# fatchord/WaveRNN

Measured on AMD Instinct MI355X. Metric: audio samples/sec (real-time factor @22.05 kHz), MoL WaveRNN batched generate, higher is better.
Workload: dtype f32

## Files before the change

### include/wavernn_amd.h

```cpp
#ifndef WAVERNN_AMD_H
#define WAVERNN_AMD_H

#include <stddef.h>
#include <stdint.h>

#ifdef __cplusplus
extern "C" {
#endif

#define WRNN_ABI_VERSION 9

enum {
    WRNN_OK = 0,
    WRNN_ERR_ARG = -1,
    WRNN_ERR_NO_DEVICE = -2,
    WRNN_ERR_HIP = -3,
    WRNN_ERR_WORKSPACE = -4,
    WRNN_ERR_KERNEL = -5,
    WRNN_ERR_RESIDENCY = -6
};

enum { WRNN_MODE_RAW = 0, WRNN_MODE_MOL = 1 };

enum {
// ... 111 lines not shown
    int32_t struct_bytes;
    int32_t n_cus;
    int32_t mode, C;
    int32_t generic;
    int32_t gH, gF, gM, gA;
    int32_t sp_nbp;
    int32_t sp_max_blocks;
    int32_t sp_fc;
} wrnn_plan_traits;
int wrnn_debug_plan(const wrnn_plan_traits *traits, int32_t n_segments, int32_t T, int32_t n_frames,
                    const wrnn_options *opt, wrnn_run_info *out, size_t *workspace_bytes);

int wrnn_timer_create(int device, wrnn_timer **out);
void wrnn_timer_destroy(wrnn_timer *t);
float wrnn_timer_ms(wrnn_timer *t);
int wrnn_timer_launches(const wrnn_timer *t);

typedef struct wrnn_pre_weights {
    int32_t feat_dims;
    int32_t compute_dims;
    int32_t res_out_dims;
    int32_t res_blocks;
    int32_t pad;
    int32_t upsample_factors[3];
    const float *conv_in_w;
    const float *bn_in;
    const float *res_w;
    const float *res_bn;
    const float *conv_out_w;
    const float *conv_out_b;
    const float *up_w;
} wrnn_pre_weights;
typedef struct wrnn_pre wrnn_pre;

int wrnn_pre_create(const wrnn_pre_weights *w, int device, wrnn_pre **out);
void wrnn_pre_destroy(wrnn_pre *p);
int wrnn_pre_hop(const wrnn_pre *p);
size_t wrnn_pre_workspace_bytes(const wrnn_pre *p, int32_t n_frames);
int wrnn_pre_upsample(const wrnn_pre *p, const float *mel, int32_t n_frames, float *mels_up, float *aux,
                      void *workspace, size_t workspace_bytes, void *stream);
int wrnn_pre_upsample_rows(const wrnn_pre *p, const float *mel, int32_t n_frames, float *mel_rows, float *aux,
                           void *workspace, size_t workspace_bytes, void *stream);
typedef struct wrnn_pre_utt {
    const float *mel;
    int32_t n_frames;
    int32_t reserved;
    int64_t up_row;
    int64_t aux_row;
} wrnn_pre_utt;
size_t wrnn_pre_workspace_bytes_many(const wrnn_pre *p, const wrnn_pre_utt *utts, int32_t n_utt, int32_t rows_only);
int wrnn_pre_upsample_many(const wrnn_pre *p, const wrnn_pre_utt *utts, int32_t n_utt, int32_t rows_only, float *mels_up, float *aux,
                           void *workspace, size_t workspace_bytes, void *stream);
int wrnn_pre_debug_host_handle(const wrnn_pre_weights *w, wrnn_pre **out);
const char *wrnn_pre_last_error(void);

int wrnn_post_unfold(const float *segments, int32_t T, int32_t n_utt, const int32_t *first, const int32_t *folds,
                     const int64_t *out_off, const double *lut, int32_t n_classes, const double *fade_in,
                     const double *fade_out, int32_t overlap, const double *tail, int32_t tail_len, int32_t batched,
                     double *out, void *stream);
const char *wrnn_post_last_error(void);

typedef struct wrnn_taco_weights {
    uint32_t struct_bytes;
    int32_t n_mels, prenet1, prenet2, decoder_dims, encoder_width, lstm_dims, attn_filters, attn_kernel;
    const float *prenet_fc1_w, *prenet_fc1_b, *prenet_fc2_w, *prenet_fc2_b;
    const float *attn_rnn_w_ih, *attn_rnn_w_hh, *attn_rnn_b_ih, *attn_rnn_b_hh;
    const float *attn_W_w, *attn_W_b, *attn_conv_w, *attn_L_w, *attn_L_b, *attn_v_w;
    const float *rnn_input_w, *rnn_input_b;
    const float *rnn1_w_ih, *rnn1_w_hh, *rnn1_b_ih, *rnn1_b_hh;
    const float *rnn2_w_ih, *rnn2_w_hh, *rnn2_b_ih, *rnn2_b_hh;
    const float *mel_proj_w;
} wrnn_taco_weights;

typedef struct wrnn_taco_call {
    uint32_t struct_bytes;
    int32_t n;
    int32_t r, max_r;
    int32_t max_steps;
    float stop_threshold;
    const float *seq;
    const float *seq_proj;
    float *mel_out;
    float *scores_out;
    int32_t *steps_done;
    void *workspace;
    size_t workspace_bytes;
    void *stream;
    int32_t variant;
} wrnn_taco_call;

size_t wrnn_taco_workspace_bytes(void);
int wrnn_taco_decode(int device, const wrnn_taco_weights *w, const wrnn_taco_call *c);
int wrnn_taco_status(const void *workspace, unsigned *out4, void *stream);
const char *wrnn_taco_last_error(void);

#define WRNN_TACO_BATCH_MAX 8
#define WRNN_TACO_BATCH_NMAX 256
typedef struct wrnn_taco_batch_call {
    uint32_t struct_bytes;
    int32_t n_sent;
    int32_t r, max_r;
    float stop_threshold;
    const int32_t *n;
    const int32_t *max_steps;
    const float *const *seq, *const *seq_proj;
    float *const *mel_out;
// ... 92 lines not shown
```

### wavernn_amd/_lib.py

```python
import ctypes
import os
import subprocess

_HERE = os.path.dirname(os.path.abspath(__file__))
CSRC = os.path.join(_HERE, 'csrc')
SO_PATH = os.path.join(CSRC, 'libwavernn_amd.so')

WRNN_OK = 0
ERR_ARG = -1
ERR_NO_DEVICE = -2
ERR_RESIDENCY = -6
MODE_RAW, MODE_MOL = 0, 1
ABI_VERSION = 9
ALGO_AUTO, ALGO_STREAM, ALGO_LOOP, ALGO_SPARSE, ALGO_DUO, ALGO_CHAIN, ALGO_OCTO = 0, 1, 2, 5, 6, 7, 8
ALGOS = {'auto': ALGO_AUTO, 'stream': ALGO_STREAM, 'loop': ALGO_LOOP, 'sparse': ALGO_SPARSE, 'duo': ALGO_DUO, 'chain': ALGO_CHAIN, 'octo': ALGO_OCTO}

EXPORTS = ['wrnn_last_error', 'wrnn_abi_version', 'wrnn_device_cus', 'wrnn_pack_create', 'wrnn_pack_destroy',
           'wrnn_pack_weight_bytes', 'wrnn_pack_sparse_blocks', 'wrnn_pack_sparse_fc_blocks', 'wrnn_workspace_bytes', 'wrnn_workspace_bytes_segments', 'wrnn_generate',
           'wrnn_generate_segments', 'wrnn_noise_fill', 'wrnn_noise_fill_host', 'wrnn_plan_segments', 'wrnn_status', 'wrnn_timer_create', 'wrnn_timer_destroy', 'wrnn_timer_ms',
           'wrnn_timer_launches', 'wrnn_debug_read_exchange', 'wrnn_debug_plan', 'wrnn_selftest', 'wrnn_selftest_metric', 'wrnn_pre_create',
           'wrnn_pre_destroy', 'wrnn_pre_hop', 'wrnn_pre_workspace_bytes', 'wrnn_pre_upsample', 'wrnn_pre_upsample_rows', 'wrnn_pre_workspace_bytes_many',
           'wrnn_pre_upsample_many', 'wrnn_pre_debug_host_handle', 'wrnn_pre_last_error',
           'wrnn_post_unfold', 'wrnn_post_last_error', 'wrnn_taco_workspace_bytes', 'wrnn_taco_decode', 'wrnn_taco_status',
           'wrnn_taco_last_error', 'wrnn_bigru', 'wrnn_taco_front_create', 'wrnn_taco_front_destroy', 'wrnn_taco_front_workspace_bytes',
           'wrnn_taco_encode', 'wrnn_taco_postnet', 'wrnn_taco_batch_workspace_bytes', 'wrnn_taco_decode_batch',
           'wrnn_bigru_many', 'wrnn_taco_front_workspace_bytes_many', 'wrnn_taco_encode_many', 'wrnn_taco_postnet_many',
           'wrnn_taco_front_debug_host_handle']


class Weights(ctypes.Structure):
    _fields_ = [(n, ctypes.c_int32) for n in ('rnn_dims', 'fc_dims', 'feat_dims', 'aux_dims', 'n_classes', 'mode')] + \
               [(n, ctypes.c_void_p) for n in ('I_w', 'I_b', 'w_ih1', 'w_hh1', 'b_ih1', 'b_hh1', 'w_ih2', 'w_hh2',
                                               'b_ih2', 'b_hh2', 'fc1_w', 'fc1_b', 'fc2_w', 'fc2_b', 'fc3_w', 'fc3_b')]


class PreWeights(ctypes.Structure):
    _fields_ = [(n, ctypes.c_int32) for n in ('feat_dims', 'compute_dims', 'res_out_dims', 'res_blocks', 'pad')] + \
               [('upsample_factors', ctypes.c_int32 * 3)] + \
               [(n, ctypes.c_void_p) for n in ('conv_in_w', 'bn_in', 'res_w', 'res_bn', 'conv_out_w', 'conv_out_b', 'up_w')]


class PreUtt(ctypes.Structure):
    _fields_ = [('mel', ctypes.c_void_p), ('n_frames', ctypes.c_int32), ('reserved', ctypes.c_int32), ('up_row', ctypes.c_int64),
                ('aux_row', ctypes.c_int64)]


TACO_WEIGHT_FIELDS = ('prenet_fc1_w', 'prenet_fc1_b', 'prenet_fc2_w', 'prenet_fc2_b', 'attn_rnn_w_ih', 'attn_rnn_w_hh', 'attn_rnn_b_ih',
                      'attn_rnn_b_hh', 'attn_W_w', 'attn_W_b', 'attn_conv_w', 'attn_L_w', 'attn_L_b', 'attn_v_w', 'rnn_input_w', 'rnn_input_b',
                      'rnn1_w_ih', 'rnn1_w_hh', 'rnn1_b_ih', 'rnn1_b_hh', 'rnn2_w_ih', 'rnn2_w_hh', 'rnn2_b_ih', 'rnn2_b_hh', 'mel_proj_w')


class TacoWeights(ctypes.Structure):
    _fields_ = [('struct_bytes', ctypes.c_uint32)] + \
               [(n, ctypes.c_int32) for n in ('n_mels', 'prenet1', 'prenet2', 'decoder_dims', 'encoder_width', 'lstm_dims', 'attn_filters',
                                              'attn_kernel')] + \
               [(n, ctypes.c_void_p) for n in TACO_WEIGHT_FIELDS]


class TacoCall(ctypes.Structure):
    _fields_ = [('struct_bytes', ctypes.c_uint32), ('n', ctypes.c_int32), ('r', ctypes.c_int32), ('max_r', ctypes.c_int32),
                ('max_steps', ctypes.c_int32), ('stop_threshold', ctypes.c_float), ('seq', ctypes.c_void_p), ('seq_proj', ctypes.c_void_p),
                ('mel_out', ctypes.c_void_p), ('scores_out', ctypes.c_void_p), ('steps_done', ctypes.c_void_p),
                ('workspace', ctypes.c_void_p), ('workspace_bytes', ctypes.c_size_t), ('stream', ctypes.c_void_p), ('variant', ctypes.c_int32)]


TACO_BATCH_MAX = 8
TACO_BATCH_NMAX = 256


class TacoBatchCall(ctypes.Structure):
    _fields_ = [('struct_bytes', ctypes.c_uint32), ('n_sent', ctypes.c_int32), ('r', ctypes.c_int32), ('max_r', ctypes.c_int32),
                ('stop_threshold', ctypes.c_float), ('n', ctypes.POINTER(ctypes.c_int32)), ('max_steps', ctypes.POINTER(ctypes.c_int32)),
                ('seq', ctypes.POINTER(ctypes.c_void_p)), ('seq_proj', ctypes.POINTER(ctypes.c_void_p)),
                ('mel_out', ctypes.POINTER(ctypes.c_void_p)), ('scores_out', ctypes.POINTER(ctypes.c_void_p)),
                ('steps_done', ctypes.c_void_p), ('workspace', ctypes.c_void_p), ('workspace_bytes', ctypes.c_size_t), ('stream', ctypes.c_void_p)]
# ... 99 lines not shown
    import torch
    L = ctypes.CDLL(SO_PATH)
    L.wrnn_last_error.restype = ctypes.c_char_p
    L.wrnn_abi_version.restype = ctypes.c_int
    L.wrnn_device_cus.argtypes = [ctypes.c_int]
    L.wrnn_pack_create.argtypes = [ctypes.POINTER(Weights), ctypes.c_int, ctypes.POINTER(ctypes.c_void_p)]
    L.wrnn_pack_destroy.argtypes = [ctypes.c_void_p]
    L.wrnn_pack_destroy.restype = None
    L.wrnn_pack_weight_bytes.argtypes = [ctypes.c_void_p]
    L.wrnn_pack_weight_bytes.restype = ctypes.c_size_t
    L.wrnn_pack_sparse_blocks.argtypes = [ctypes.c_void_p]
    L.wrnn_pack_sparse_fc_blocks.argtypes = [ctypes.c_void_p]
    L.wrnn_workspace_bytes.argtypes = [ctypes.c_void_p, ctypes.POINTER(Geometry), ctypes.POINTER(Options)]
    L.wrnn_workspace_bytes.restype = ctypes.c_size_t
    L.wrnn_generate.argtypes = [ctypes.c_void_p, ctypes.POINTER(Geometry), ctypes.c_void_p, ctypes.c_void_p,
                                ctypes.c_void_p, ctypes.c_void_p, ctypes.c_void_p, ctypes.c_size_t, ctypes.POINTER(Options),
                                ctypes.c_void_p]
    L.wrnn_workspace_bytes_segments.argtypes = [ctypes.c_void_p, ctypes.c_int32, ctypes.c_int32, ctypes.c_int32,
                                                ctypes.POINTER(Options)]
    L.wrnn_workspace_bytes_segments.restype = ctypes.c_size_t
    L.wrnn_generate_segments.argtypes = [ctypes.c_void_p, ctypes.c_int32, ctypes.c_int32, ctypes.c_void_p, ctypes.c_void_p,
                                         ctypes.c_int32, ctypes.c_int32, ctypes.c_int32, ctypes.c_void_p, ctypes.c_void_p,
                                         ctypes.c_void_p, ctypes.c_void_p, ctypes.c_void_p, ctypes.c_size_t,
                                         ctypes.POINTER(Options), ctypes.c_void_p]
    L.wrnn_noise_fill.argtypes = [ctypes.c_int, ctypes.c_int32, ctypes.c_int32, ctypes.c_int32, ctypes.c_int32, ctypes.c_uint64, ctypes.c_void_p,
                                  ctypes.c_void_p, ctypes.c_int, ctypes.c_void_p]
    L.wrnn_noise_fill_host.argtypes = L.wrnn_noise_fill.argtypes[:8]
    L.wrnn_plan_segments.argtypes = [ctypes.c_void_p, ctypes.c_int32, ctypes.c_int32, ctypes.POINTER(Options), ctypes.POINTER(RunInfo)]
    L.wrnn_timer_create.argtypes = [ctypes.c_int, ctypes.POINTER(ctypes.c_void_p)]
    L.wrnn_timer_destroy.argtypes = [ctypes.c_void_p]
    L.wrnn_timer_destroy.restype = None
    L.wrnn_timer_ms.argtypes = [ctypes.c_void_p]
    L.wrnn_timer_ms.restype = ctypes.c_float
    L.wrnn_timer_launches.argtypes = [ctypes.c_void_p]
    L.wrnn_debug_read_exchange.argtypes = [ctypes.c_void_p, ctypes.c_void_p, ctypes.c_int32, ctypes.c_int32, ctypes.c_int32,
                                           ctypes.POINTER(Options), ctypes.c_int, ctypes.c_int, ctypes.c_int, ctypes.c_int,
                                           ctypes.c_void_p]
    L.wrnn_debug_plan.argtypes = [ctypes.POINTER(PlanTraits), ctypes.c_int32, ctypes.c_int32, ctypes.c_int32, ctypes.POINTER(Options),
                                  ctypes.POINTER(RunInfo), ctypes.POINTER(ctypes.c_size_t)]
    L.wrnn_pre_create.argtypes = [ctypes.POINTER(PreWeights), ctypes.c_int, ctypes.POINTER(ctypes.c_void_p)]
    L.wrnn_pre_destroy.argtypes = [ctypes.c_void_p]
    L.wrnn_pre_destroy.restype = None
    L.wrnn_pre_hop.argtypes = [ctypes.c_void_p]
    L.wrnn_pre_workspace_bytes.argtypes = [ctypes.c_void_p, ctypes.c_int32]
    L.wrnn_pre_workspace_bytes.restype = ctypes.c_size_t
    L.wrnn_pre_upsample.argtypes = [ctypes.c_void_p, ctypes.c_void_p, ctypes.c_int32, ctypes.c_void_p, ctypes.c_void_p,
                                    ctypes.c_void_p, ctypes.c_size_t, ctypes.c_void_p]
    L.wrnn_pre_upsample_rows.argtypes = L.wrnn_pre_upsample.argtypes
    L.wrnn_pre_workspace_bytes_many.argtypes = [ctypes.c_void_p, ctypes.POINTER(PreUtt), ctypes.c_int32, ctypes.c_int32]
    L.wrnn_pre_workspace_bytes_many.restype = ctypes.c_size_t
    L.wrnn_pre_upsample_many.argtypes = [ctypes.c_void_p, ctypes.POINTER(PreUtt), ctypes.c_int32, ctypes.c_int32, ctypes.c_void_p, ctypes.c_void_p,
                                         ctypes.c_void_p, ctypes.c_size_t, ctypes.c_void_p]
    L.wrnn_pre_debug_host_handle.argtypes = [ctypes.POINTER(PreWeights), ctypes.POINTER(ctypes.c_void_p)]
    L.wrnn_pre_last_error.restype = ctypes.c_char_p
    L.wrnn_post_unfold.argtypes = [ctypes.c_void_p, ctypes.c_int32, ctypes.c_int32, ctypes.c_void_p, ctypes.c_void_p, ctypes.c_void_p,
                                   ctypes.c_void_p, ctypes.c_int32, ctypes.c_void_p, ctypes.c_void_p, ctypes.c_int32,
                                   ctypes.c_void_p, ctypes.c_int32, ctypes.c_int32, ctypes.c_void_p, ctypes.c_void_p]
    L.wrnn_post_last_error.restype = ctypes.c_char_p
    L.wrnn_taco_workspace_bytes.restype = ctypes.c_size_t
    L.wrnn_taco_decode.argtypes = [ctypes.c_int, ctypes.POINTER(TacoWeights), ctypes.POINTER(TacoCall)]
    L.wrnn_taco_status.argtypes = [ctypes.c_void_p, ctypes.POINTER(ctypes.c_uint32 * 4), ctypes.c_void_p]
    L.wrnn_taco_last_error.restype = ctypes.c_char_p
    L.wrnn_taco_batch_workspace_bytes.argtypes = [ctypes.c_int32]
    L.wrnn_taco_batch_workspace_bytes.restype = ctypes.c_size_t
    L.wrnn_taco_decode_batch.argtypes = [ctypes.c_int, ctypes.POINTER(TacoWeights), ctypes.POINTER(TacoBatchCall)]
    L.wrnn_bigru.argtypes = [ctypes.c_int, ctypes.POINTER(BigruCall)]
    L.wrnn_taco_front_create.argtypes = [ctypes.POINTER(TacoFrontWeights), ctypes.c_int, ctypes.POINTER(ctypes.c_void_p)]
    L.wrnn_taco_front_destroy.argtypes = [ctypes.c_void_p]
    L.wrnn_taco_front_destroy.restype = None
    L.wrnn_taco_front_workspace_bytes.argtypes = [ctypes.c_void_p, ctypes.c_int32]
    L.wrnn_taco_front_workspace_bytes.restype = ctypes.c_size_t
    L.wrnn_taco_encode.argtypes = [ctypes.c_void_p, ctypes.c_void_p, ctypes.c_int32, ctypes.c_void_p, ctypes.c_void_p, ctypes.c_void_p,
                                   ctypes.c_void_p, ctypes.c_size_t, ctypes.c_void_p]
    L.wrnn_taco_postnet.argtypes = [ctypes.c_void_p, ctypes.c_void_p, ctypes.c_int32, ctypes.c_void_p, ctypes.c_void_p, ctypes.c_void_p,
                                    ctypes.c_size_t, ctypes.c_void_p]
    L.wrnn_bigru_many.argtypes = [ctypes.c_int, ctypes.POINTER(BigruManyCall)]
    L.wrnn_taco_front_workspace_bytes_many.argtypes = [ctypes.c_void_p, ctypes.POINTER(ctypes.c_int32), ctypes.c_int32]
    L.wrnn_taco_front_workspace_bytes_many.restype = ctypes.c_size_t
    L.wrnn_taco_encode_many.argtypes = [ctypes.c_void_p, ctypes.c_void_p, ctypes.POINTER(ctypes.c_int32), ctypes.c_int32, ctypes.c_void_p,
                                        ctypes.c_void_p, ctypes.c_void_p, ctypes.c_void_p, ctypes.c_size_t, ctypes.c_void_p]
    L.wrnn_taco_postnet_many.argtypes = [ctypes.c_void_p, ctypes.POINTER(ctypes.c_void_p), ctypes.POINTER(ctypes.c_int32), ctypes.c_int32,
                                         ctypes.c_void_p, ctypes.c_void_p, ctypes.c_void_p, ctypes.c_size_t, ctypes.c_void_p]
    L.wrnn_taco_front_debug_host_handle.argtypes = [ctypes.POINTER(TacoFrontWeights), ctypes.POINTER(ctypes.c_void_p)]
    L.wrnn_status.argtypes = [ctypes.c_void_p, ctypes.c_void_p]
    L.wrnn_selftest.argtypes = [ctypes.c_int, ctypes.c_int]
    L.wrnn_selftest_metric.restype = ctypes.c_float
    _lib = L
    return L


def check(rc, what):
    if rc != WRNN_OK:
        raise WrnnError(f'{what} failed (rc={rc}): {lib().wrnn_last_error().decode()}')


def noise_fill_host(mode, n_segments, n_classes, t_begin, t_end, seed, seg_id=None):
    import numpy as np
    mol = mode == 'MOL'
    out = np.empty((t_end - t_begin, 11 * n_segments) if mol else (t_end - t_begin, n_segments, n_classes), np.float32)
    ids = None if seg_id is None else np.ascontiguousarray(seg_id, dtype=np.uint64)
    if ids is not None and ids.shape != (n_segments,):
        raise ValueError('seg_id: one 64-bit id per segment')
    check(lib().wrnn_noise_fill_host(MODE_MOL if mol else MODE_RAW, n_segments, n_classes, t_begin, t_end, int(seed) & (2 ** 64 - 1),
                                     None if ids is None else ids.ctypes.data, out.ctypes.data), 'wrnn_noise_fill_host')
    return out
```

### wavernn_amd/batch.py

```python
import time
from dataclasses import dataclass
from typing import List, Optional, Sequence

import numpy as np
import torch

from . import fold as _fold


@dataclass
class Plan:
    target: int
    overlap: int
    T: int
    stride: int
    lengths: List[int]
    offsets: np.ndarray
    folds: np.ndarray
    first: np.ndarray
    seg_pos: np.ndarray
    seg_lim: np.ndarray
    seg_utt: np.ndarray

    @property
# ... 59 lines not shown
            else:
                origin = f'built-in defaults ({f} was measured on other kernel sources)'
        except (OSError, ValueError, KeyError):
            pass
        if path is not None:
            return table, origin
        _STEP_TABLE = (table, origin)
    return _STEP_TABLE


def estimate_step_us(n_segments: int, table: Optional[dict] = None) -> float:
    if n_segments <= 0:
        return 0.0
    table = table or step_table()[0]
    groups = -(-n_segments // 16)
    rounds = -(-groups // 32)
    depth = min(8, max(1, -(-(-(-groups // rounds)) // 4)))
    return rounds * table[depth]


def choose_ranks(n_segments: int, world: int, table: Optional[dict] = None) -> int:
    est = [estimate_step_us(-(-n_segments // r), table) for r in range(1, world + 1)]
    best = min(est)
    return 1 + next(i for i, e in enumerate(est) if e <= best * 1.01)


def pack_noise(mode: str, plan: Plan, per_utt, lo: int = 0, hi: Optional[int] = None, steps: Optional[int] = None):
    hi = plan.n_segments if hi is None else hi
    T = plan.T if steps is None else int(steps)
    n = hi - lo
    utts = [u for u in range(len(plan.lengths)) if plan.first[u] < hi and plan.first[u] + plan.folds[u] > lo]
    sample = per_utt[utts[0]]
    is_torch = isinstance(sample, torch.Tensor)
    cat = (lambda xs, d: torch.cat(xs, dim=d)) if is_torch else (lambda xs, d: np.concatenate(xs, axis=d))
    mix, logi, raw = [], [], []
    for u in utts:
        Bu, f0 = int(plan.folds[u]), int(plan.first[u])
        a, b = max(lo, f0) - f0, min(hi, f0 + Bu) - f0
        z = per_utt[u]
        if mode == 'MOL':
            z = z.reshape(T, 11 * Bu)
            mix.append(z[:, 10 * a:10 * b])
            logi.append(z[:, 10 * Bu + a:10 * Bu + b])
        else:
            raw.append(z.reshape(T, Bu, -1)[:, a:b])
    out = cat(mix + logi, 1) if mode == 'MOL' else cat(raw, 1)
    assert out.shape[0] == T and (out.shape[1] == 11 * n if mode == 'MOL' else out.shape[1] == n)
    return out.contiguous() if is_torch else np.ascontiguousarray(out)


def library_seg_ids(seed, folds, first_fold: int = 0) -> np.ndarray:
    hi = np.uint64((int(seed) & 0xffffffff) << 32)
    return hi | np.arange(first_fold, first_fold + int(folds), dtype=np.uint64)


def chunk_utterances(plan: Plan, lo: int, hi: int, max_segments: int):
    chunks, cur, cur_lo, cur_hi = [], [], None, None
    for u in range(len(plan.lengths)):
        a, b = max(lo, int(plan.first[u])), min(hi, int(plan.first[u] + plan.folds[u]))
        if a >= b:
            continue
        if cur and (b - cur_lo) > max_segments:
            chunks.append((cur, cur_lo, cur_hi))
            cur, cur_lo = [], None
        if cur_lo is None:
            cur_lo = a
        cur.append(u)
        cur_hi = b
    if cur:
        chunks.append((cur, cur_lo, cur_hi))
    return chunks


def generate_corpus(model, mels: Sequence, target: int, overlap: int, mu_law: bool, seeds: Optional[Sequence[int]] = None,
                    group=None, loop_fn=None, return_segments=False, noise_source='cpu', finish='all', check=True,
                    max_segments_per_launch: int = 4096, shard=None, ranks: Optional[int] = None, timings: Optional[dict] = None):
    import torch.distributed as dist
    from .rng import draw_steps
    if noise_source in ('cpu', 'library') and seeds is None:
        raise ValueError(f"noise_source={noise_source!r} needs `seeds` (one per utterance); "
                         "pass noise_source='device' to draw from the device generator instead")
    if noise_source not in ('cpu', 'device', 'library'):
        raise ValueError(f'unknown noise source {noise_source!r}')
    world = dist.get_world_size(group) if group is not None else 1
    rank = dist.get_rank(group) if group is not None else 0
    if shard is not None:
        if group is not None:
            raise ValueError('shard=(rank, world) emulates a rank without a process group')
        rank, world = int(shard[0]), int(shard[1])
        finish = 'own'
    device = next(model.parameters()).device
    mode = model.mode
    mu_law = mu_law if mode == 'RAW' else False
    hop = model.hop_length
    was_training = model.training
    model.eval()
    mels = [torch.as_tensor(m) for m in mels]
    mels = [m.unsqueeze(0) if m.dim() == 2 else m for m in mels]
    frames = [int(m.size(-1)) for m in mels]
    plan = plan_utterances([n * hop for n in frames], target, overlap)
    bounds = shard_bounds(plan.n_segments, world, ranks)
    lo, hi = bounds[rank]
    n_max = max(h - l for l, h in bounds)

    out_local = torch.zeros(n_max, plan.T, dtype=torch.float32, device=device)
    native_pre = loop_fn is None and getattr(model, 'pre_algo', 'torch') == 'native' and device.type == 'cuda'
# ... 48 lines not shown
                    return mels_up, aux
                ups, auxs = zip(*[model.conditioning(mels[u])[:2] for u in utts])
                return torch.cat(ups).contiguous(), torch.cat(auxs).contiguous()
            rows = eng is not None and native_pre and model.mel_rows_ok(eng, n_seg, T)
            mels_up, aux = conditioning(rows)
            rebase = np.array([local_off[int(u)] - int(plan.offsets[int(u)]) for u in plan.seg_utt[clo:chi]], dtype=np.int64)
            seg_pos = (plan.seg_pos[clo:chi].astype(np.int64) + rebase).astype(np.int32)
            seg_lim = (plan.seg_lim[clo:chi].astype(np.int64) + rebase).astype(np.int32)
            out_view = out_local[clo - lo:chi - lo]
            gens, pool = {}, None
            if noise_source == 'cpu':
                if len(utts) > 1 and mode == 'RAW':
                    import os
                    from concurrent.futures import ThreadPoolExecutor
                    pool = ThreadPoolExecutor(max(1, min(len(utts), (os.cpu_count() or 2) // (2 * max(1, int(os.environ.get('LOCAL_WORLD_SIZE', '1')))))))
                from .rng import burn_ctor_draws
                for u in utts:
                    gens[u] = torch.Generator(device='cpu').manual_seed(int(seeds[u]))
                    burn_ctor_draws(model.rnn_dims, model.aux_dims, 'cpu', gens[u])

            lib_ids = None
            if noise_source == 'library':
                lib_ids = np.concatenate([library_seg_ids(seeds[u], min(chi, int(plan.first[u] + plan.folds[u])) - max(clo, int(plan.first[u])),
                                                          max(clo, int(plan.first[u])) - int(plan.first[u])) for u in utts])
                assert lib_ids.shape == (n_seg,)
            lib_kw = dict(noise_seed=int(getattr(model, 'noise_key', 0)), noise_seg_id=lib_ids) if lib_ids is not None else {}

            def draw(steps_):
                if noise_source == 'library':
                    if loop_fn is None:
                        return None
                    from ._lib import noise_fill_host
                    return torch.from_numpy(noise_fill_host(mode, n_seg, model.n_classes, 0, steps_, lib_kw['noise_seed'], lib_ids)).to(device)
                if noise_source != 'cpu':
                    return draw_steps(mode, n_seg, steps_, model.n_classes, device, 'device')
                def one(u):
                    noise[u] = draw_steps(mode, int(plan.folds[u]), steps_, model.n_classes, 'cpu', 'cpu', generator=gens[u])
                if pool is None:
                    for u in utts:
                        one(u)
                else:
                    list(pool.map(one, utts))
                return pack_noise(mode, plan, noise, clo, chi, steps=steps_).to(device)

            if loop_fn is not None:
                out_view[:] = loop_fn(mels_up, aux, seg_pos, seg_lim, T, draw(T), hop)
                if pool is not None:
                    pool.shutdown()
                continue
            from ._lib import ResidencyError
            from .engine import RESUMABLE_KERNELS
            steps = T
            groups = model.loop_sparse_groups(eng, n_seg, T) if hasattr(model, 'loop_sparse_groups') else 0
            if noise_source != 'library' and eng.plan(n_seg, T, algo=model.loop_algo)['kernel'] in RESUMABLE_KERNELS:
                per_step = n_seg * (11 if mode == 'MOL' else model.n_classes) * 4
                steps = max(1, min(T, getattr(model, 'noise_chunk_bytes', 2 << 30) // per_step))
                steps = -(-T // (-(-T // steps)))
            try:
                for t0 in range(0, T, steps):
                    t1 = min(T, t0 + steps)
                    eng.run_segments(mels_up, aux, seg_pos, seg_lim, T, draw(t1 - t0), hop, algo=model.loop_algo, check=check, out=out_view,
                                     t_range=None if (t0 == 0 and t1 == T) else (t0, t1), sparse_groups=groups, tuning=slab_tuning, **lib_kw)
            except ResidencyError as e:
                import warnings
                warnings.warn(f'wavernn_amd: {e}; redoing the chunk unsliced on the next kernel')
                if rows:
                    mels_up, aux = conditioning(False)
                for u in gens:
                    gens[u].manual_seed(int(seeds[u]))
                    burn_ctor_draws(model.rnn_dims, model.aux_dims, 'cpu', gens[u])
                eng.run_segments(mels_up, aux, seg_pos, seg_lim, T, draw(T), hop, algo=model.loop_algo, check=check, out=out_view, sparse_groups=groups, tuning=slab_tuning, **lib_kw)
            finally:
                if pool is not None:
                    pool.shutdown()
    n_utt = len(frames)
    work, gathered = None, None
    if group is not None:
        gathered = [torch.empty_like(out_local) for _ in range(world)]
        work = dist.all_gather(gathered, out_local, group=group, async_op=True)
        if timings is not None:
            timings['gather_bytes'] = timings.get('gather_bytes', 0) + (world - 1) * out_local.numel() * out_local.element_size()
            timings['world_seen'] = dist.get_world_size(group)

    def gathered_segments():
        nonlocal work
        if group is None:
            if shard is not None:
                raise ValueError('an emulated shard has only its own block of segments')
            return out_local[:plan.n_segments]
        if work is not None:
            t_w = time.perf_counter()
            work.wait()
            work = None
            if timings is not None:
                timings['gather_wait_ms'] = timings.get('gather_wait_ms', 0.0) + (time.perf_counter() - t_w) * 1e3
        return torch.cat([gathered[r][:h - l] for r, (l, h) in enumerate(bounds)])

    if was_training:
        model.train()
    if return_segments:
        return gathered_segments().cpu().numpy().astype(np.float64), plan
    outs = [None] * n_utt

    def unfold(segs, first_of, us):
        if not us:
            return
        if native_post:
            from .post import unfold_on_device
            wav, sl = unfold_on_device(segs, *unfold_args(us, first_of), tables=early.get(first_of))
            if getattr(model, 'pinned_output', True):
                host = torch.empty(wav.shape, dtype=wav.dtype, pin_memory=True)
                host.copy_(wav, non_blocking=True)
                torch.cuda.current_stream(wav.device).synchronize()
                wav = host.numpy()
            else:
                wav = wav.cpu().numpy()
            for (a, b), u in zip(sl, us):
                outs[u] = wav[a:b]
            return
        host = segs.cpu().numpy().astype(np.float64)
        for u in us:
            y = host[first_of(u):first_of(u) + int(plan.folds[u])].copy()
            if mu_law:
                y = _fold.decode_mu_law(y, model.n_classes, False)
# ... 18 lines not shown
```

### wavernn_amd/csrc/wrnn_abi.hip

```cpp
#include <hip/hip_runtime.h>
#include <stdarg.h>
#include <stdio.h>
#include <stdlib.h>
#include <string.h>
#include <math.h>
#include <string>
#include <vector>

#include "../../include/wavernn_amd.h"
#include "wrnn_device.h"

namespace wrnn {
hipError_t launch_cond(const CondArgs &a, int n_cus, bool valu, hipStream_t stream);
hipError_t launch_cond_frames(const CondArgs &a, hipStream_t stream);
hipError_t launch_cond_frames_slab(const CondArgs &a, hipStream_t stream);
hipError_t launch_slab_prep(const CondArgs &a, const float *nz_in, float *nz_out, long nz_n, unsigned *xcc, int n_cus, hipStream_t stream);
hipError_t launch_cond_frag(const CondArgs &a, int n_cus, hipStream_t stream);
hipError_t launch_noise_mol(const float *in, float *out, long n, int B, int n_cus, hipStream_t stream);
hipError_t launch_noise_fill(bool mol, int B, int C, int t0, int t1, uint64_t seed, const uint64_t *seg_id, float *out, int n_cus, hipStream_t stream);
void noise_fill_host(bool mol, int B, int C, int t0, int t1, uint64_t seed, const uint64_t *seg_id, float *out);
hipError_t launch_stream(const LoopArgs &args, int mode, hipStream_t stream);
hipError_t launch_loop(const LoopArgs &args, int ncl, int mode, hipStream_t stream);
int loop_max_depth(int mode);
size_t loop_state_floats(int G);
hipError_t launch_generic(const GenArgs &args, int mode, hipStream_t stream);
bool generic_dims_ok(int H, int F, int M, int A, int C, int mode);
hipError_t launch_duo(const LoopArgs &args, int ncl, int mode, hipStream_t stream);
int duo_max_depth();
size_t duo_xbuf_bytes(int G);
size_t duo_xbuf_bytes_max();
hipError_t launch_sparse(const LoopArgs &args, int nbp, int mode, hipStream_t stream);
int sparse_clusters(int n_cus);
int sparse_max_slots();
size_t sparse_state_floats(int slots);
size_t sparse_xbuf_bytes(int slots);
hipError_t launch_put_floats(float *dst, const float *src, int n, hipStream_t stream);
hipError_t launch_chain(const LoopArgs &args, int mode, hipStream_t stream);
hipError_t launch_octo(const LoopArgs &args, int ncl, int mode, hipStream_t stream);
int octo_max_depth();
int chain_clusters(int n_cus);
int chain_max_depth();
size_t chain_state_floats(int G);
size_t chain_xbuf_bytes(int G);
int selftest_mfma(char *msg, size_t n);
int selftest_allgather(int n_cus, char *msg, size_t n, float *us_per_round);
int selftest_tanh(char *msg, size_t n);
int selftest_xor(char *msg, size_t n);
}

using namespace wrnn;

static thread_local char g_err[512] = "";
static void set_err(const char *fmt, ...)
// ... 310 lines not shown
extern "C" float wrnn_timer_ms(wrnn_timer *t)
{
    if (!t || t->used < 2) return -1.f;
    float total = 0.f;
    for (int i = 0; i + 1 < t->used; i += 2) {
        if (hipEventSynchronize(t->ev[i + 1]) != hipSuccess) return -1.f;
        float ms = 0.f;
        if (hipEventElapsedTime(&ms, t->ev[i], t->ev[i + 1]) != hipSuccess) return -1.f;
        total += ms;
    }
    return total;
}

namespace {
int timer_mark(wrnn_timer *t, hipStream_t stream)
{
    if (!t) return WRNN_OK;
    if (t->used == (int)t->ev.size()) {
        hipEvent_t e;
        HIPCHK(hipEventCreate(&e));
        t->ev.push_back(e);
    }
    HIPCHK(hipEventRecord(t->ev[t->used], stream));
    t->used += 1;
    return WRNN_OK;
}

struct ProgressCtx {
    void (*fn)(int32_t, int32_t, int32_t, void *);
    void *user;
    int32_t done, T, n;
};
void progress_trampoline(void *p)
{
    ProgressCtx *c = static_cast<ProgressCtx *>(p);
    c->fn(c->done, c->T, c->n, c->user);
    delete c;
}
int enqueue_progress(const wrnn_options *o, int done, int T, int n, hipStream_t stream)
{
    if (!o->progress) return WRNN_OK;
    ProgressCtx *c = new ProgressCtx{o->progress, o->progress_user, done, T, n};
    hipError_t e = hipLaunchHostFunc(stream, progress_trampoline, c);
    if (e != hipSuccess) {
        delete c;
        set_err("hipLaunchHostFunc failed: %s", hipGetErrorString(e));
        return WRNN_ERR_HIP;
    }
    return WRNN_OK;
}

enum Kind { K_STREAM, K_GENERIC, K_LOOP, K_DUO, K_OCTO, K_CHAIN, K_SPARSE, N_KINDS };
constexpr int DUO_TAB_FPS = 8;
constexpr bool DUO_AUTO = true;
constexpr int CHAIN_AUTO_GROUPS = 8;
constexpr bool OCTO_AUTO = false;

struct KindDesc {
    const char *name;
    int units_per_wg;
    int kind_tag;
    bool persistent;
    bool slabbed;
    bool mel_stage;
    int (*clusters)(int n_cus);
    int (*max_depth)(int mode);
    size_t (*state_floats)(int G);
    size_t (*xbuf_bytes)(int G);
    size_t (*xbuf_fill)(int G);
    hipError_t (*launch)(const LoopArgs &a, int ncl, int nbp, int mode, hipStream_t s);
};
size_t loop_xbuf_bytes(int) { return XBUF_FLOATS * sizeof(float); }
const KindDesc KINDS[N_KINDS] = {
     {"wrnn_stream_kernel", 0, 0, false, false, false},
     {"wrnn_generic_kernel", 16, 0, false, false, false},
     {"wrnn_loop_kernel", 16, 1, true, false, false, clusters_of_64, loop_max_depth, loop_state_floats, loop_xbuf_bytes, loop_xbuf_bytes,
                     [](const LoopArgs &a, int ncl, int, int mode, hipStream_t s) { return launch_loop(a, ncl, mode, s); }},
     {"wrnn_duo_kernel", 16, 2, true, true, true, clusters_of_64, [](int) { return duo_max_depth(); }, loop_state_floats,
                     [](int) { return duo_xbuf_bytes_max(); }, duo_xbuf_bytes,
                     [](const LoopArgs &a, int ncl, int, int mode, hipStream_t s) { return launch_duo(a, ncl, mode, s); }},
     {"wrnn_octo_kernel", 16, 5, true, true, true, clusters_of_64, [](int) { return octo_max_depth(); }, loop_state_floats,
                     [](int) { return duo_xbuf_bytes_max(); }, duo_xbuf_bytes,
                     [](const LoopArgs &a, int ncl, int, int mode, hipStream_t s) { return launch_octo(a, ncl, mode, s); }},
     {"wrnn_chain_kernel", 16, 4, true, true, true, chain_clusters, [](int) { return chain_max_depth(); }, chain_state_floats,
                     chain_xbuf_bytes, chain_xbuf_bytes,
                     [](const LoopArgs &a, int, int, int mode, hipStream_t s) { return launch_chain(a, mode, s); }},
     {"wrnn_sparse_kernel", 64, 3, true, true, true, sparse_clusters, [](int) { return 1; }, sparse_state_floats,
                     sparse_xbuf_bytes, sparse_xbuf_bytes,
                     [](const LoopArgs &a, int, int nbp, int mode, hipStream_t s) { return launch_sparse(a, nbp, mode, s); }},
};

struct Plan {
    Kind kind;
    int ncl, G, rounds, per_round, slab, ngr_max;
    int tab_fps;
    int t0, t1;
};

struct WsLayout {
    size_t status, xcc, segs, melc, c2f, c3f, c4f;
    size_t cI, npre;
    size_t nlib;
    size_t xbuf, state, cIf;
    size_t total;
};
size_t al(size_t x) { return (x + 255) / 256 * 256; }

template <class S> S norm_struct(const S *in)
{
    S s;
    memset(&s, 0, sizeof s);
    if (in) memcpy(&s, in, in->struct_bytes > 0 && (size_t)in->struct_bytes < sizeof s ? (size_t)in->struct_bytes : sizeof s);
    s.struct_bytes = (int32_t)sizeof s;
    return s;
}
wrnn_options whole_call(const wrnn_options *opt)
{
    wrnn_options o = norm_struct(opt);
    o.t_begin = 0; o.t_end = 0;
    return o;
}

void plan_split(Plan *pl, int B, int ncl, int gmax, int depth)
{
    const int groups = (B + SEG - 1) / SEG;
    int g = depth;
    if (g < 1 || g > gmax) {
        const int rounds = (groups + ncl * gmax - 1) / (ncl * gmax);
        g = (groups + ncl * rounds - 1) / (ncl * rounds);
        if (g < 1) g = 1;
        if (g > gmax) g = gmax;
    }
    pl->ncl = ncl; pl->G = g;
    pl->rounds = (groups + ncl * g - 1) / (ncl * g);
    pl->per_round = (B + pl->rounds - 1) / pl->rounds;
    pl->ngr_max = (pl->per_round + SEG - 1) / SEG;
    if (pl->ngr_max > ncl * g) { pl->rounds += 1; pl->per_round = (B + pl->rounds - 1) / pl->rounds; pl->ngr_max = (pl->per_round + SEG - 1) / SEG; }
}

constexpr size_t NOISE_LIB_SLAB_BYTES = (size_t)2 << 30;
int default_slab(const Plan &pl, int mode, int C, bool noise_lib)
{
    const int most = KINDS[pl.kind].slabbed ? 4096 : 1024;
    int slab = most;
    if (!KINDS[pl.kind].slabbed) slab = (int)((96u << 20) / ((size_t)pl.ngr_max * SEG * H * sizeof(float)));
    else if (mode == WRNN_MODE_MOL) slab = (int)((32u << 20) / ((size_t)pl.per_round * 11 * sizeof(float) * pl.rounds));
    else if (noise_lib) {
        const size_t fit = NOISE_LIB_SLAB_BYTES / ((size_t)pl.per_round * pl.rounds * C * sizeof(float));
        slab = fit < (size_t)most ? (int)fit : most;
    }
    return slab < 16 ? 16 : slab > most ? most : slab;
}

int make_plan(const wrnn_plan_traits *p, int B, int T, const wrnn_options *o, Plan *pl)
{
    const bool shape_ok = (p->mode == WRNN_MODE_MOL) || (p->C == H);
    pl->t0 = o->t_begin; pl->t1 = o->t_end;
    if (pl->t0 == 0 && pl->t1 == 0) pl->t1 = T;
    if (pl->t0 < 0 || pl->t1 > T || pl->t0 >= pl->t1) { set_err("bad step range [%d, %d) of T=%d", pl->t0, pl->t1, T); return WRNN_ERR_ARG; }
    const bool partial = pl->t0 != 0 || pl->t1 != T;
    const int algo = o->algo;
    if (algo != WRNN_ALGO_AUTO && algo != WRNN_ALGO_STREAM && algo != WRNN_ALGO_LOOP && algo != WRNN_ALGO_SPARSE && algo != WRNN_ALGO_DUO && algo != WRNN_ALGO_CHAIN &&
        algo != WRNN_ALGO_OCTO) {
        set_err("unknown algo %d", algo);
        return WRNN_ERR_ARG;
    }
    if (o->sparse_groups < 0 || o->sparse_groups > sparse_max_slots()) {
        set_err("wrnn_options.sparse_groups = %d: 0 or 1 (one group per cluster) or 2", o->sparse_groups);
        return WRNN_ERR_ARG;
    }
    if (o->noise_lib != 0 && o->noise_lib != 1) {
        set_err("wrnn_options.noise_lib = %d: 0 (the caller's `noise`) or 1 (the library draws it)", o->noise_lib);
        return WRNN_ERR_ARG;
    }
    const bool two_groups = o->sparse_groups == 2;
    const int groups = (B + SEG - 1) / SEG;
    pl->kind = K_STREAM; pl->ncl = 0; pl->G = 0; pl->rounds = 1; pl->per_round = B; pl->slab = T; pl->ngr_max = groups;
    if (p->generic) {
        if (algo != WRNN_ALGO_AUTO && algo != WRNN_ALGO_STREAM) {
            set_err("this pack has non-shipped dims (rnn %d, fc %d, feat %d, aux %d): only the generic kernel (algo auto / stream) runs it", p->gH, p->gF, p->gM, p->gA);
            return WRNN_ERR_ARG;
        }
        if (partial) { set_err("a partial step range needs a persistent loop kernel"); return WRNN_ERR_ARG; }
        if (two_groups) { set_err("wrnn_options.sparse_groups = 2: only wrnn_sparse_kernel runs two groups per cluster (this call runs on wrnn_generic_kernel)"); return WRNN_ERR_ARG; }
        pl->kind = K_GENERIC;
        return WRNN_OK;
    }
    const int ccl = KINDS[K_CHAIN].clusters(p->n_cus), scl = KINDS[K_SPARSE].clusters(p->n_cus), lcl = KINDS[K_LOOP].clusters(p->n_cus);
    const bool chain_hw = shape_ok && ccl >= 1;
    if (algo == WRNN_ALGO_CHAIN && !chain_hw) {
        set_err("wrnn_chain_kernel needs MOL or RAW with 512 classes, and >= 256 CUs (C = %d, device: %d CUs)", p->C, p->n_cus);
        return !shape_ok ? WRNN_ERR_ARG : WRNN_ERR_RESIDENCY;
    }
    if (algo == WRNN_ALGO_SPARSE && (!p->sp_nbp || scl < 1)) {
        set_err("block-sparse kernel needs MOL or RAW with 512 classes, >= 256 CUs and GRU matrices with <= 64 surviving 16x1 blocks per block row "
                "(this pack: mode %s, %d classes, up to %d blocks; device: %d CUs)", p->mode == WRNN_MODE_MOL ? "MOL" : "RAW", p->C, p->sp_max_blocks, p->n_cus);
        return (!p->sp_nbp) ? WRNN_ERR_ARG : WRNN_ERR_RESIDENCY;
    }
    if (algo == WRNN_ALGO_OCTO && (p->mode != WRNN_MODE_MOL || KINDS[K_OCTO].clusters(p->n_cus) != MAXCL)) {
        set_err("wrnn_octo_kernel needs MOL and >= 256 CUs (mode %d, device has %d CUs)", p->mode, p->n_cus);
        return p->mode != WRNN_MODE_MOL ? WRNN_ERR_ARG : WRNN_ERR_RESIDENCY;
    }
    if (algo == WRNN_ALGO_DUO && (!shape_ok || KINDS[K_DUO].clusters(p->n_cus) < 1)) {
        set_err("the two-workgroups-per-CU loop kernel needs MOL or RAW with 512 classes, and >= 64 CUs (C = %d, device has %d CUs)", p->C, p->n_cus);
        return !shape_ok ? WRNN_ERR_ARG : WRNN_ERR_RESIDENCY;
    }
    if (algo == WRNN_ALGO_LOOP && !(shape_ok && lcl >= 1)) {
        set_err("the loop kernel needs >= 64 CUs and (MOL or RAW with 512 classes); device has %d CUs, C=%d", p->n_cus, p->C);
        return WRNN_ERR_RESIDENCY;
    }
    const bool sparse_auto = p->sp_nbp && p->mode == WRNN_MODE_MOL;
    Kind kind = K_STREAM;
    int ncl = 0;
    if (algo == WRNN_ALGO_CHAIN || (algo == WRNN_ALGO_AUTO && chain_hw && groups <= CHAIN_AUTO_GROUPS && !sparse_auto)) {
        kind = K_CHAIN; ncl = ccl;
    } else if (algo == WRNN_ALGO_SPARSE || (algo == WRNN_ALGO_AUTO && sparse_auto && scl >= 1)) {
        kind = K_SPARSE; ncl = scl;
    } else if (algo != WRNN_ALGO_STREAM && shape_ok && lcl >= 1) {
        ncl = lcl;
        if (o->clusters == 1 || o->clusters == 2 || o->clusters == 4) ncl = o->clusters < ncl ? o->clusters : ncl;
        else if (groups < ncl && !(DUO_AUTO && algo != WRNN_ALGO_LOOP && ncl == MAXCL)) {
            int c2 = 1; while (c2 < groups) c2 *= 2; if (c2 < ncl) ncl = c2;
        }
        kind = K_LOOP;
        if (algo == WRNN_ALGO_DUO || (algo == WRNN_ALGO_AUTO && DUO_AUTO && ncl == MAXCL)) kind = K_DUO;
        if (algo == WRNN_ALGO_OCTO || (kind == K_DUO && algo == WRNN_ALGO_AUTO && OCTO_AUTO && p->mode == WRNN_MODE_MOL && !o->clusters)) kind = K_OCTO;
    }
    const KindDesc &k = KINDS[kind];
    pl->kind = kind;
    if (two_groups) {
        if (kind != K_SPARSE) {
            set_err("wrnn_options.sparse_groups = 2: only wrnn_sparse_kernel runs two groups per cluster (this call runs on %s)", k.name);
            return WRNN_ERR_ARG;
        }
        if (p->mode != WRNN_MODE_MOL) { set_err("wrnn_options.sparse_groups = 2: wrnn_sparse_kernel's 9-bit RAW form is built with one group per cluster only"); return WRNN_ERR_ARG; }
        if (!p->sp_fc || (o->tuning & 2048)) {
            set_err("wrnn_options.sparse_groups = 2: needs a pack whose Linear layers are block-sparse too (wrnn_pack_sparse_fc_blocks() > 0) and their gathered fc "
                    "stages: the dense fc tiles leave no registers for a second group");
            return WRNN_ERR_ARG;
        }
        if (o->phase_clocks && !(o->tuning & 64)) { set_err("wrnn_options.sparse_groups = 2: the phase-clock build of wrnn_sparse_kernel has one group per cluster only"); return WRNN_ERR_ARG; }
    }
    if (k.persistent) {
        if (two_groups) plan_split(pl, B, ncl, sparse_max_slots(), sparse_max_slots());
        else plan_split(pl, B, ncl, k.max_depth(p->mode), o->depth);
        pl->slab = o->slab_steps >= 1 ? o->slab_steps : default_slab(*pl, p->mode, p->C, o->noise_lib != 0);
        if (pl->slab > T) pl->slab = T;
        pl->tab_fps = DUO_TAB_FPS;
    } else if (partial) {
        set_err("a partial step range [%d, %d) needs a persistent loop kernel", pl->t0, pl->t1);
        return WRNN_ERR_ARG;
    }
    if (k.slabbed && ((size_t)B * pl->tab_fps + 1) * 3 * H * sizeof(float) >= 0x7FFFF000ull) {
        set_err("%d segments in one call: the per-slab aux tables exceed a 2 GB buffer resource; split the call (generate_corpus caps a launch at 4096 segments)", B);
        return WRNN_ERR_ARG;
    }
    return WRNN_OK;
}

WsLayout ws_layout(const wrnn_plan_traits *p, const Plan &pl, int B, int T, int n_frames, bool noise_lib)
{
    const size_t noise_row = (size_t)B * (p->mode == WRNN_MODE_MOL ? 11 : p->C) * sizeof(float);
    const KindDesc &k = KINDS[pl.kind];
    WsLayout l;
    memset(&l, 0, sizeof l);
    size_t o = 0;
    l.status = o; o = al(o + STATUS_WORDS * sizeof(unsigned));
    l.xcc = o;    o = al(o + XCC_WORDS * sizeof(unsigned));
    l.segs = o;   o = al(o + (size_t)3 * B * sizeof(int));
    l.melc = o;   o = al(o + (size_t)3 * LAST_SCALE * sizeof(float));
    if (pl.kind == K_GENERIC) {
        l.nlib = o; if (noise_lib) o = al(o + (size_t)T * noise_row);
        l.total = o;
        return l;
    }
    const size_t tab_rows = k.slabbed ? (size_t)B * pl.tab_fps + 1 : (size_t)n_frames + 1;
    l.c2f = o;    o = al(o + tab_rows * 3 * H * sizeof(float));
    l.c3f = o;    o = al(o + tab_rows * H * sizeof(float));
    l.c4f = o;    o = al(o + tab_rows * H * sizeof(float));
    if (k.persistent) {
        l.xbuf = o;  o = al(o + k.xbuf_bytes(pl.G));
        l.state = o; o = al(o + (size_t)pl.rounds * k.state_floats(pl.G) * sizeof(float));
        l.cIf = o;   if (!k.slabbed) o = al(o + (size_t)pl.slab * pl.ngr_max * SEG * H * sizeof(float));
        l.npre = o;  if (p->mode == WRNN_MODE_MOL) o = al(o + (size_t)pl.slab * 11 * B * sizeof(float));
    } else {
        l.cI = o;    o = al(o + (size_t)T * B * H * sizeof(float));
        l.npre = o;
    }
    l.nlib = o;   if (noise_lib) o = al(o + (size_t)(k.persistent ? pl.slab : T) * noise_row);
    l.total = o;
    return l;
}
void hop_magic(int hop, unsigned *magic, int *shift)
{
    *magic = 0u; *shift = 0;
    if (hop < 2) return;
    int s = 0;
    while ((1ll << s) < hop) ++s;
    const unsigned long long m = ((1ull << (31 + s)) + (unsigned long long)hop - 1ull) / (unsigned long long)hop;
    if (m >> 32) return;
    const int sh = s - 1;
    for (long long q = 0; q * hop < (1ll << 31); q += 997) {
        for (long long p = q * hop - 1; p <= q * hop + 1; ++p) {
            if (p < 0 || p >= (1ll << 31)) continue;
            if ((long long)(((unsigned long long)p * m) >> (32 + sh)) != p / hop) return;
        }
    }
    *magic = (unsigned)m; *shift = sh;
}

int check_geometry(const wrnn_geometry *g)
{
    if (!g) { set_err("NULL geometry"); return WRNN_ERR_ARG; }
    if (g->B < 1 || g->T < 1 || g->L < 1 || g->hop < 1 || g->n_frames < 1 || g->stride < 0) {
        set_err("bad geometry B=%d T=%d stride=%d L=%d hop=%d n_frames=%d", g->B, g->T, g->stride, g->L, g->hop, g->n_frames);
        return WRNN_ERR_ARG;
    }
    if ((long)g->n_frames * g->hop < g->L) { set_err("n_frames*hop < L"); return WRNN_ERR_ARG; }
    if ((double)g->B * g->stride + g->T > 2.0e9) { set_err("geometry overflows int32"); return WRNN_ERR_ARG; }
    return WRNN_OK;
}
int check_segments(int B, int T, const int32_t *seg_pos, const int32_t *seg_lim, int L, int hop, int n_frames)
{
    if (B < 1 || T < 1 || L < 1 || hop < 1 || n_frames < 1 || !seg_pos || !seg_lim) {
        set_err("bad segment table B=%d T=%d L=%d hop=%d n_frames=%d", B, T, L, hop, n_frames);
        return WRNN_ERR_ARG;
    }
    if ((long)n_frames * hop < L) { set_err("n_frames*hop < L"); return WRNN_ERR_ARG; }
    for (int b = 0; b < B; ++b) {
        if (seg_pos[b] < 0 || seg_lim[b] < 0 || seg_lim[b] > L || (double)seg_pos[b] + T > 2.0e9) {
            set_err("segment %d: pos=%d lim=%d outside [0,%d]", b, seg_pos[b], seg_lim[b], L);
            return WRNN_ERR_ARG;
        }
    }
    return WRNN_OK;
}
int plan_report(const wrnn_plan_traits *tr, int B, int T, int n_frames, const wrnn_options &o, wrnn_run_info *out, size_t *ws_bytes)
{
    Plan pl;
    const int rc = make_plan(tr, B, T, &o, &pl);
    if (rc != WRNN_OK) return rc;
    if (out) {
        memset(out, 0, sizeof *out);
        out->kernel = KINDS[pl.kind].name; out->units_per_wg = KINDS[pl.kind].units_per_wg;
        out->clusters = pl.ncl; out->depth = pl.G; out->rounds = pl.rounds; out->slab_steps = pl.slab;
    }
    if (ws_bytes) *ws_bytes = ws_layout(tr, pl, B, T, n_frames, o.noise_lib != 0).total;
    return WRNN_OK;
}
}

extern "C" size_t wrnn_workspace_bytes_segments(const wrnn_pack *p, int32_t n_segments, int32_t T, int32_t n_frames,
                                                const wrnn_options *opt)
{
    if (!p || n_segments < 1 || T < 1 || n_frames < 1) return 0;
    size_t bytes = 0;
    (void)plan_report(&p->tr, n_segments, T, n_frames, whole_call(opt), nullptr, &bytes);
    return bytes;
}

extern "C" int wrnn_plan_segments(const wrnn_pack *p, int32_t n_segments, int32_t T, const wrnn_options *opt, wrnn_run_info *out)
{
    if (!p || !out || n_segments < 1 || T < 1) { set_err("bad argument"); return WRNN_ERR_ARG; }
    return plan_report(&p->tr, n_segments, T, 1, whole_call(opt), out, nullptr);
}

extern "C" size_t wrnn_workspace_bytes(const wrnn_pack *p, const wrnn_geometry *g, const wrnn_options *opt)
{
    if (!p || check_geometry(g) != WRNN_OK) return 0;
    return wrnn_workspace_bytes_segments(p, g->B, g->T, g->n_frames, opt);
}

extern "C" int wrnn_generate_segments(const wrnn_pack *p, int32_t B, int32_t T, const int32_t *seg_pos,
                                      const int32_t *seg_lim, int32_t L, int32_t hop, int32_t n_frames,
                                      const float *mels_up, const float *aux, const float *noise, float *out,
                                      void *workspace, size_t workspace_bytes, const wrnn_options *opt, void *stream_)
{
    const wrnn_options opts = norm_struct(opt), *o = &opts;
    const bool lib_noise = o->noise_lib == 1;
    if (lib_noise && noise) {
        set_err("wrnn_options.noise_lib = 1: the library draws the noise itself -- `noise` must be NULL (the tensor passed would not be read)");
        return WRNN_ERR_ARG;
    }
    if (!p || !mels_up || !aux || (!noise && !lib_noise) || !out || !workspace) { set_err("NULL argument"); return WRNN_ERR_ARG; }
    int rc = check_segments(B, T, seg_pos, seg_lim, L, hop, n_frames);
    if (rc != WRNN_OK) return rc;
    Plan pl;
    if ((rc = make_plan(&p->tr, B, T, o, &pl)) != WRNN_OK) return rc;
    const KindDesc &k = KINDS[pl.kind];
    const WsLayout l = ws_layout(&p->tr, pl, B, T, n_frames, lib_noise);
    if (workspace_bytes < l.total) { set_err("workspace %zu < required %zu", workspace_bytes, l.total); return WRNN_ERR_WORKSPACE; }
    if (((uintptr_t)workspace & 255) != 0) { set_err("workspace must be 256-byte aligned"); return WRNN_ERR_ARG; }
    hipStream_t stream = (hipStream_t)stream_;
    DeviceGuard dg(p->device);
    HIPCHK(dg.err);
    char *ws = (char *)workspace;
    const bool mol_mode = p->tr.mode == WRNN_MODE_MOL;
    wrnn_timer *timer = o->timer;
    if (timer && pl.t0 == 0) timer->used = 0;

    if (pl.t0 == 0) HIPCHK(hipMemsetAsync(ws + l.status, 0, STATUS_WORDS * sizeof(unsigned), stream));
    HIPCHK(hipMemcpyAsync(ws + l.segs, seg_pos, (size_t)B * sizeof(int), hipMemcpyHostToDevice, stream));
    HIPCHK(hipMemcpyAsync(ws + l.segs + (size_t)B * sizeof(int), seg_lim, (size_t)B * sizeof(int), hipMemcpyHostToDevice, stream));
    const int *d_pos = (const int *)(ws + l.segs), *d_lim = d_pos + B;
    if (o->mel_stage) {
        if (!k.mel_stage) { set_err("wrnn_options.mel_stage: only wrnn_duo_kernel / wrnn_sparse_kernel / wrnn_chain_kernel form the last up-sampling stage (this call runs on another kernel)"); return WRNN_ERR_ARG; }
        if (o->mel_stage != 1 || o->mel_scale != LAST_SCALE || !o->mel_taps || !o->seg_moff || o->mel_rows < 3) {
            set_err("wrnn_options.mel_stage=%d: needs mel_scale == %d (got %d), mel_taps, seg_moff, mel_rows >= 3", o->mel_stage, LAST_SCALE, o->mel_scale);
            return WRNN_ERR_ARG;
        }
        for (int b = 0; b < B; ++b) {
            const long last = (seg_lim[b] < (long)seg_pos[b] + T ? seg_lim[b] : (long)seg_pos[b] + T) - 1;
            if (last < seg_pos[b]) continue;
            const long j0 = (long)seg_pos[b] + o->seg_moff[b], j1 = last + o->seg_moff[b];
            if (o->seg_moff[b] < 0 || j0 / LAST_SCALE < 1 || j1 / LAST_SCALE + 1 >= o->mel_rows) {
                set_err("segment %d: positions %ld..%ld of the last up-sampling stage reach outside its %d input rows", b, j0, j1, o->mel_rows);
                return WRNN_ERR_ARG;
            }
        }
        float coef[3 * LAST_SCALE];
        for (int ph = 0; ph < LAST_SCALE; ++ph) {
            double c0 = 0, c1 = 0, c2 = 0;
            for (int j = 0; j <= 2 * LAST_SCALE; ++j) {
                const double w = o->mel_taps[j];
                if (j < LAST_SCALE - ph) c0 += w; else if (j < 2 * LAST_SCALE - ph) c1 += w; else c2 += w;
            }
            coef[3 * ph] = (float)c0; coef[3 * ph + 1] = (float)c1; coef[3 * ph + 2] = (float)c2;
        }
        HIPCHK(hipMemcpyAsync(ws + l.segs + (size_t)2 * B * sizeof(int), o->seg_moff, (size_t)B * sizeof(int), hipMemcpyHostToDevice, stream));
        HIPCHK(launch_put_floats((float *)(ws + l.melc), coef, 3 * LAST_SCALE, stream));
    }
    if (pl.kind == K_GENERIC) {
        GenArgs g;
        memset(&g, 0, sizeof g);
        g.I_T = p->g_I_T; g.I_b = p->I_b; g.w_ih1T = p->w_ih1T; g.w_hh1T = p->w_hh1T; g.b_ih1 = p->b_ih1; g.b_hh1 = p->b_hh1;
        g.w_ih2T = p->g_w_ih2T; g.w_hh2T = p->w_hh2T; g.b_ih2 = p->b_ih2; g.b_hh2 = p->b_hh2;
        g.fc1T = p->g_fc1T; g.fc1_b = p->fc1_b; g.fc2T = p->g_fc2T; g.fc2_b = p->fc2_b; g.fc3T = p->fc3T; g.fc3_b = p->fc3_b;
        g.mels_up = mels_up; g.aux = aux; g.noise = noise; g.force_x = o->force_x; g.out = out; g.dbg_logits = o->logits;
        g.seg_pos = d_pos; g.seg_lim = d_lim;
        if (lib_noise) {
            HIPCHK(launch_noise_fill(mol_mode, B, p->tr.C, 0, T, o->noise_seed, o->noise_seg_id, (float *)(ws + l.nlib), p->tr.n_cus, stream));
            g.noise = (const float *)(ws + l.nlib);
        }
        g.H = p->tr.gH; g.F = p->tr.gF; g.M = p->tr.gM; g.A = p->tr.gA; g.C = p->tr.C; g.B = B; g.T = T; g.hop = hop;
        if ((rc = timer_mark(timer, stream)) != WRNN_OK) return rc;
        HIPCHK(launch_generic(g, p->tr.mode, stream));
        if ((rc = timer_mark(timer, stream)) != WRNN_OK) return rc;
        wrnn_run_info gi;
        memset(&gi, 0, sizeof gi);
        gi.kernel = k.name; gi.rounds = 1; gi.slab_steps = T; gi.launches = 1;
        if (o->info) *o->info = gi;
        return enqueue_progress(o, T, T, B, stream);
    }

    CondArgs c;
    memset(&c, 0, sizeof c);
    c.mels_up = mels_up; c.aux = aux; c.I_cT = p->I_cT; c.I_b = p->I_b; c.c2_wT = p->c2_wT; c.b_ih2 = p->b_ih2;
    c.c3_wT = p->c3_wT; c.fc1_b = p->fc1_b; c.c4_wT = p->c4_wT; c.fc2_b = p->fc2_b;
    c.c2f = (float *)(ws + l.c2f); c.c3f = (float *)(ws + l.c3f); c.c4f = (float *)(ws + l.c4f);
    c.seg_pos = d_pos; c.seg_lim = d_lim;
    c.B = B; c.T = T; c.hop = hop; c.NF = n_frames;
    if (k.slabbed) {
        const long eff = (long)(pl.tab_fps - 2) * hop + 1;
        if (pl.slab > eff) pl.slab = (int)eff;
    } else HIPCHK(launch_cond_frames(c, stream));

    LoopArgs a;
    memset(&a, 0, sizeof a);
    a.I_w0 = p->I_w0; a.w_ih1 = p->w_ih1; a.w_hh1 = p->w_hh1; a.b_ih1 = p->b_ih1; a.b_hh1 = p->b_hh1;
    a.w_ih2 = p->w_ih2; a.w_hh2 = p->w_hh2; a.b_hh2 = p->b_hh2; a.fc1_w = p->fc1_w; a.fc2_w = p->fc2_w;
    a.fc3_w = p->fc3_w; a.fc3_b = p->fc3_b; a.fc3f = p->fc3f; a.u1 = p->u1;
    a.w_ih1T = p->w_ih1T; a.w_hh1T = p->w_hh1T; a.w_ih2T = p->w_ih2T; a.w_hh2T = p->w_hh2T;
    a.fc1T = p->fc1T; a.fc2T = p->fc2T; a.fc3T = p->fc3T;
    a.c2f = c.c2f; a.c3f = c.c3f; a.c4f = c.c4f;
    a.noise = noise; a.force_x = o->force_x; a.out = out; a.dbg_logits = o->logits;
    a.status = (unsigned *)(ws + l.status);
    a.prof = (u64 *)o->phase_clocks;
    a.tuning = o->tuning;
    a.seg_pos = d_pos; a.seg_lim = d_lim;
    a.Btot = B; a.T = T; a.hop = hop; a.NF = n_frames; a.C = p->tr.C;
    a.NG = (B + SEG - 1) / SEG;
    a.Nall = B;
    a.xcc_tab = (unsigned *)(ws + l.xcc);
    a.mels_up = mels_up; a.aux_fr = aux; a.I_cT = p->I_cT; a.I_b = p->I_b;
    a.mel_stage = o->mel_stage; a.seg_moff = d_pos + 2 * B; a.mel_coef = (const float *)(ws + l.melc);
    hop_magic(hop, &a.hop_magic, &a.hop_shift);

    wrnn_run_info info;
    memset(&info, 0, sizeof info);
    info.kernel = k.name; info.units_per_wg = k.units_per_wg;
    info.clusters = pl.ncl; info.depth = pl.G; info.rounds = pl.rounds; info.slab_steps = pl.slab;

    if (k.persistent) {
        a.sp_vals = p->sp_vals; a.sp_cols = p->sp_cols;
        a.sp_fc_vals = (o->tuning & 2048) ? nullptr : p->sp_fc_vals; a.sp_fc_cols = p->sp_fc_cols;
        const bool mol = p->tr.mode == WRNN_MODE_MOL;
        a.xbuf = (float *)(ws + l.xbuf);
        a.cIf = (const float *)(ws + l.cIf);
        a.G = pl.G;
        c.cI = (float *)(ws + l.cIf);
        for (int s0 = pl.t0; s0 < pl.t1; s0 += pl.slab) {
            const int s1 = s0 + pl.slab < pl.t1 ? s0 + pl.slab : pl.t1;
            if (lib_noise) HIPCHK(launch_noise_fill(mol, B, p->tr.C, s0, s1, o->noise_seed, o->noise_seg_id, (float *)(ws + l.nlib), p->tr.n_cus, stream));
            const bool prep_fused = k.slabbed && !(o->tuning & 8192);
            const float *mol_rows = nullptr;
            if (mol) {
                const float *const rows = lib_noise ? (const float *)(ws + l.nlib) : noise + (size_t)(s0 - pl.t0) * 11 * B;
                if (prep_fused) mol_rows = rows;
                else HIPCHK(launch_noise_mol(rows, (float *)(ws + l.npre), (long)(s1 - s0) * 11 * B, B, p->tr.n_cus, stream));
                a.noise_pre = (const float *)(ws + l.npre);
                a.noise_t0 = s0;
            } else if (lib_noise) {
                a.noise = (const float *)(ws + l.nlib);
                a.noise_t0 = s0;
            } else {
                a.noise_t0 = pl.t0;
            }
            if (k.slabbed) {
                c.t0 = s0; c.B = B; c.FPS = pl.tab_fps;
                if (prep_fused) HIPCHK(launch_slab_prep(c, mol_rows, (float *)(ws + l.npre), (long)(s1 - s0) * 11 * B, (unsigned *)(ws + l.xcc), p->tr.n_cus, stream));
                else HIPCHK(launch_cond_frames_slab(c, stream));
                a.tab_fps = pl.tab_fps; a.tab_t0 = s0;
            }
            bool xcc_clear = prep_fused;
            for (int r = 0; r < pl.rounds; ++r) {
                const int rb0 = (int)(((long)r * B) / pl.rounds), rb1 = (int)(((long)(r + 1) * B) / pl.rounds);
                const int nr = rb1 - rb0;
                if (nr < 1) continue;
                const int ngr = (nr + SEG - 1) / SEG;
                c.t0 = s0; c.t1 = s1; c.rb0 = rb0; c.B = nr; c.NG = ngr;
                if (!k.slabbed) HIPCHK(launch_cond_frag(c, p->tr.n_cus, stream));
                if (!k.slabbed || s0 == 0 || pl.rounds > 1 || (o->tuning & 4)) HIPCHK(hipMemsetAsync(ws + l.xbuf, 0xFF, k.xbuf_fill(pl.G), stream));
                if (k.slabbed && !xcc_clear) HIPCHK(hipMemsetAsync(ws + l.xcc, 0, XCC_WORDS * sizeof(unsigned), stream));
                xcc_clear = false;
                a.state = (float *)(ws + l.state) + (size_t)r * k.state_floats(pl.G);
                a.t0 = s0; a.t1 = s1; a.cI_t0 = s0; a.rb0 = rb0; a.Btot = nr; a.NG = ngr; a.resume = s0 > 0 ? 1 : 0;
                a.kind_tag = k.kind_tag;
                if ((rc = timer_mark(timer, stream)) != WRNN_OK) return rc;
                hipError_t e = k.launch(a, pl.ncl, p->tr.sp_nbp, p->tr.mode, stream);
                if (e != hipSuccess) {
                    (void)hipGetLastError();
                    set_err("%s cooperative launch failed: %s", info.kernel, hipGetErrorString(e));
                    return e == hipErrorCooperativeLaunchTooLarge ? WRNN_ERR_RESIDENCY : WRNN_ERR_HIP;
                }
                if ((rc = timer_mark(timer, stream)) != WRNN_OK) return rc;
                info.launches += 1;
            }
            if ((rc = enqueue_progress(o, s1, T, B, stream)) != WRNN_OK) return rc;
        }
    } else {
        c.cI = (float *)(ws + l.cI);
        a.cI = c.cI;
        HIPCHK(launch_cond(c, p->tr.n_cus, o->cond_valu != 0, stream));
        if (lib_noise) {
            HIPCHK(launch_noise_fill(mol_mode, B, p->tr.C, 0, T, o->noise_seed, o->noise_seg_id, (float *)(ws + l.nlib), p->tr.n_cus, stream));
            a.noise = (const float *)(ws + l.nlib);
        }
        a.b0 = 0;
        a.nb = B;
        if ((rc = timer_mark(timer, stream)) != WRNN_OK) return rc;
        HIPCHK(launch_stream(a, p->tr.mode, stream));
        if ((rc = timer_mark(timer, stream)) != WRNN_OK) return rc;
        info.launches = 1;
        if ((rc = enqueue_progress(o, T, T, B, stream)) != WRNN_OK) return rc;
    }
    if (o->info) *o->info = info;
    return WRNN_OK;
}

extern "C" int wrnn_generate(const wrnn_pack *p, const wrnn_geometry *g, const float *mels_up, const float *aux,
                             const float *noise, float *out, void *workspace, size_t workspace_bytes, const wrnn_options *opt,
                             void *stream_)
{
    int rc = check_geometry(g);
    if (rc != WRNN_OK) return rc;
// ... 108 lines not shown
```

### wavernn_amd/csrc/wrnn_chain.hip

```cpp
#include <type_traits>

#include "wrnn_ring.h"

namespace wrnn {

constexpr int CHCL = 4;
constexpr int CHWG = 64;
constexpr int CHMAXG = 4;
constexpr int CHPART = 2 * NW * 3 * 256;
constexpr int CHSTATE_SLOT = NT * 4 + SEG;
static_assert(CHCL * CHWG <= XCC_WORDS, "placement table");
static_assert(CHCL * CHMAXG <= LMAXG * MAXCL, "one exchange-buffer region per (slot, cluster)");
static_assert(SEG * LDC <= 2 * XT, "RAW logits fit the fc3 region");

struct ChLds {
    int off_seg, off_geo, off_st, off_part, off_misc, off_prof, off_b3, off_y2t, off_f3, total;
};
__host__ __device__ inline ChLds ch_lds(int G)
{
    ChLds l;
    int o = 0;
    l.off_seg = o;  o += G * 64;
    l.off_geo = o;  o += 2 * CHMAXG;
    l.off_st = o;   o += G * 8 * NT;
    l.off_part = o; o += CHPART;
    l.off_misc = o; o += 64;
    l.off_prof = o; o += 64;
    l.off_b3 = o;   o += 32;
    l.off_y2t = o;  o += 256;
    o = (o + 3) & ~3;
    l.off_f3 = o;   o += 2 * XT;
    l.total = o;
    return l;
}

typedef unsigned ch_u32x2 __attribute__((ext_vector_type(2)));
#define CHX(k)                                                                 \
    do {                                                                       \
        if (PROF && tid == 0) {                                                \
            const u64 now_ = __builtin_amdgcn_s_memtime();                     \
            PROFL[k] += now_ - plast;                                          \
            plast = now_;                                                      \
        }                                                                      \
    } while (0)

template <int MODE, bool LA, bool PROF>
__device__ __forceinline__ void ch_role(const LoopArgs &a, float *smem, const int cl, const int ncl, const int J, const bool loc_a, const bool loc_b)
{
    const int G = a.G;
    const ChLds L = ch_lds(G);
    float *PART = smem + L.off_part, *fc3b = smem + L.off_b3, *F3 = smem + L.off_f3, *ST = smem + L.off_st, *Y2T = smem + L.off_y2t;
    int *SEGT = reinterpret_cast<int *>(smem + L.off_seg), *GEO = reinterpret_cast<int *>(smem + L.off_geo);
    u64 *PROFL = reinterpret_cast<u64 *>(smem + L.off_prof);
    u64 plast = 0;
    const int tid = threadIdx.x, lane = tid & 63, w = __builtin_amdgcn_readfirstlane(tid >> 6);
    const int fi = lane & 15, kq = lane >> 4;
    const int kbase_lane = KCH * w + 4 * kq;
    const int pu = 4 * w + (tid & 3), pj = (tid >> 2) & 15;
    const int prow = LU * J + pu;
    const int T0 = a.t0, T1 = a.t1;
    unsigned *const status = a.status;
    const int hop = a.hop, resume = a.resume, Tall = a.T, Nall = a.Nall, noise_t0 = a.noise_t0, C = a.C;
    const unsigned magic = a.hop_magic;
    const int mshift = a.hop_shift;
    const int zrow = a.Nall * a.tab_fps;
    float *const outp = a.out, *const dbgl = a.dbg_logits;
    const float *const forcex = a.force_x, *const noise_pre = a.noise_pre, *const noise_raw = a.noise;
    const float *const mels_up = a.mels_up, *const aux_fr = a.aux_fr, *const mel_coef = a.mel_coef;
    const int mel_stage = a.mel_stage;
    const int NR = a.Btot, NGR = a.NG;
    constexpr bool HAS_FC1 = !LA;
    constexpr bool MOL = MODE == 1;
    float *const state_wg = a.state + ((size_t)(cl * CHWG + (LA ? 0 : 32) + J) * G) * CHSTATE_SLOT;

    float A_ih[3][AF], A_hh[3][AF], A_fc1[AF], A_fc2[AF];
#pragma unroll
    for (int g = 0; g < 3; ++g) {
        load_afrag(A_ih[g], LA ? a.w_ih1 : a.w_ih2, LA ? H : H + AUX, g * H + LU * J + fi, true, kbase_lane);
        load_afrag(A_hh[g], LA ? a.w_hh1 : a.w_hh2, H, g * H + LU * J + fi, true, kbase_lane);
    }
    if constexpr (HAS_FC1) load_afrag(A_fc1, a.fc1_w, H + AUX, LU * J + fi, true, kbase_lane);
    if constexpr (!LA) load_afrag(A_fc2, a.fc2_w, H + AUX, LU * J + fi, true, kbase_lane);
    float A_f3[AF];
    float A_f3m[2][AF];
    if constexpr (LA && MOL) {
        if (a.tuning & 32) {
#pragma unroll
            for (int q = 0; q < 2; ++q)
#pragma unroll
                for (int k = 0; k < AF; ++k) A_f3m[q][k] = 0.f;
        } else {
#pragma unroll
            for (int q = 0; q < 2; ++q)
#pragma unroll
                for (int r = 0; r < 8; ++r) {
                    const float4 v = *reinterpret_cast<const float4 *>(a.fc3f + q * XT + frag_off(w, 0, lane) + 256 * r);
                    A_f3m[q][4 * r + 0] = v.x; A_f3m[q][4 * r + 1] = v.y; A_f3m[q][4 * r + 2] = v.z; A_f3m[q][4 * r + 3] = v.w;
                }
        }
    }
    bool fold3 = false;
    float A3[2][4];
    if constexpr (!LA && MOL) {
#pragma unroll
        for (int q = 0; q < 2; ++q)
#pragma unroll
            for (int i = 0; i < 4; ++i) A3[q][i] = (16 * q + fi < C) ? a.fc3_w[(size_t)(16 * q + fi) * H + LU * J + 4 * i + kq] : 0.f;
    }
    float b3 = 0.f;
    if constexpr (LA && !MOL) {
        load_afrag(A_f3, a.fc3_w, H, LU * J + fi, true, kbase_lane);
        b3 = a.fc3_b[prow];
    }
    float cb_r = 0.f, cb_z = 0.f, cb_n = 0.f, ux_r = 0.f, ux_z = 0.f, ux_n = 0.f, w0o = 0.f;
    if constexpr (LA) {
        cb_r = a.b_ih1[prow]; cb_z = a.b_ih1[H + prow]; cb_n = a.b_ih1[2 * H + prow];
        ux_r = a.u1[prow]; ux_z = a.u1[H + prow]; ux_n = a.u1[2 * H + prow];
        w0o = a.I_w0[prow];
    }
    const float *bhp = LA ? a.b_hh1 : a.b_hh2;
    const float bh_r = bhp[prow], bh_z = bhp[H + prow], bh_n = bhp[2 * H + prow];
    CondTile ct;
    if constexpr (LA) cond_tile_init(ct, a.I_cT, a.I_b, J, lane);
    for (int q = tid; q < L.off_f3; q += NT) smem[q] = 0.f;
    __syncthreads();
    int nact = 0;
    for (int i = 0; i < G; ++i) {
        const int g = cl + ncl * i;
        if (g >= NGR) break;
        nact = i + 1;
        const int b0 = (int)(((long)g * NR) / NGR), nb = (int)(((long)(g + 1) * NR) / NGR) - b0;
        if (tid == 0) { GEO[2 * i] = a.rb0 + b0; GEO[2 * i + 1] = nb; }
        if (tid < SEG) {
            const int sc = a.rb0 + b0 + (tid < nb ? tid : nb - 1);
            const int pos = a.seg_pos[sc];
            SEGT[i * 64 + tid] = pos;
            SEGT[i * 64 + SEG + tid] = a.seg_lim[sc];
            SEGT[i * 64 + 2 * SEG + tid] = sc * a.tab_fps - (pos + a.tab_t0) / a.hop;
            SEGT[i * 64 + 3 * SEG + tid] = a.mel_stage ? a.seg_moff[sc] : 0;
        }
        float4 sv = make_float4(0.f, bh_r, bh_z, bh_n);
        if (resume) sv = *reinterpret_cast<const float4 *>(state_wg + (size_t)i * CHSTATE_SLOT + tid * 4);
        ST[(i * 8 + 0) * NT + tid] = sv.x; ST[(i * 8 + 1) * NT + tid] = sv.y; ST[(i * 8 + 2) * NT + tid] = sv.z; ST[(i * 8 + 3) * NT + tid] = sv.w;
    }
    fold3 = MOL && nact == 1 && (a.tuning & 16) == 0;
    const bool sampler = LA && J < (MOL ? nact : 4 * nact);
    const bool f3_lds = (a.tuning & 32) != 0;
    if (MOL && sampler) {
        for (int q = tid; q < 2 * XT / 4; q += NT) reinterpret_cast<float4 *>(F3)[q] = reinterpret_cast<const float4 *>(a.fc3f)[q];
        if (tid < 32) fc3b[tid] = tid < 30 ? a.fc3_b[tid] : 0.f;
    }
    float *const LGT = F3;
    __syncthreads();

    const __amdgpu_buffer_rsrc_t xrs = make_rsrc(a.xbuf, (unsigned)(DXBUF_FLOATS * 4));
    const __amdgpu_buffer_rsrc_t crs = make_rsrc(a.c2f, 0x7FFFF000u);
    const __amdgpu_buffer_rsrc_t nrs = make_rsrc(noise_pre, 0x7FFFF000u);
    const __amdgpu_buffer_rsrc_t f1rs = make_rsrc(a.c3f, 0x7FFFF000u), f2rs = make_rsrc(a.c4f, 0x7FFFF000u);
    const int voff_frag = frag_off(w, 0, lane) * 4;
    const int voff_own = (((J * 64) + 16 * w + pj) * 4 + (tid & 3)) * 4;
    const bool loc_x2 = loc_b, loc_y1 = loc_b;

    bool dead = false;
    int pp = 0;
    int t = T0;
    auto cbase_of = [&](int i) { return (i * CHCL + cl) * DSLOTB; };
    auto nb_of = [&](int i) { return GEO[2 * i + 1]; };

    auto stage = [&](auto NTC, auto AGC, const float (&A0)[AF], const float (&A1)[AF], const float (&A2)[AF], int so, int nb, unsigned code, int ts, int px_wait,
                     float &s0, float &s1, float &s2, unsigned &ownw, bool want_own) {
        constexpr int NTL = decltype(NTC)::value;
        constexpr bool AG = decltype(AGC)::value != 0;
        const bool live = fi < nb, plive = pj < nb;
        u32x4 x[8];
#pragma unroll
        for (int r = 0; r < 8; ++r) x[r] = __builtin_amdgcn_raw_buffer_load_b128(xrs, voff_frag + r * 1024, so, 16 );
        if (want_own) ownw = __builtin_amdgcn_raw_buffer_load_b32(xrs, voff_own, so, 16 );
        if (__builtin_expect(!frag_there(x, live), 0))
            wait_for([&] { return frag_there(x, live); },
                     [&] {
#pragma unroll
                         for (int r = 0; r < 8; ++r) x[r] = __builtin_amdgcn_raw_buffer_load_b128(xrs, voff_frag + r * 1024, so, 16 );
                         if (want_own) ownw = __builtin_amdgcn_raw_buffer_load_b32(xrs, voff_own, so, 16 );
                     },
                     status, dead, code, ts);
        if (want_own && __builtin_expect(__any(plive && ownw == SENT), 0))
            wait_for([&] { return !__any(plive && ownw == SENT); }, [&] { ownw = __builtin_amdgcn_raw_buffer_load_b32(xrs, voff_own, so, 16 ); },
                     status, dead, code | 0x80u, ts);
        CHX(px_wait);
        float b[32];
        frag_to_b(x, b);
// ... 454 lines not shown
```

### wavernn_amd/csrc/wrnn_cond.hip

```cpp
#include <stdlib.h>
#include <string.h>

#include "wrnn_device.h"

namespace wrnn {


constexpr int CR = 8;

__global__ __launch_bounds__(H) void wrnn_cond_sample_kernel(const CondArgs a)
{
    __shared__ __attribute__((aligned(16))) float in[CR][KCOND];
    const int r = threadIdx.x;
    float wreg[KCOND];
#pragma unroll
    for (int k = 0; k < KCOND; ++k) wreg[k] = a.I_cT[k * H + r];
    const float bias = a.I_b[r];
    const long rows = (long)a.T * a.B;
    for (long base = (long)blockIdx.x * CR; base < rows; base += (long)gridDim.x * CR) {
        __syncthreads();
        for (int q = r; q < CR * KCOND; q += H) {
            const int rr = q / KCOND, k = q % KCOND;
            const long row = base + rr;
            float val = 0.f;
// ... 185 lines not shown
    }
    if (r < 4 * AUX) ax[r] = (f < a.NF) ? a.aux[(size_t)f * 4 * AUX + r] : 0.f;
    __syncthreads();
    float g0 = 0.f, g1 = 0.f, g2 = 0.f, y3 = 0.f, y4 = 0.f;
#pragma unroll 8
    for (int k = 0; k < AUX; ++k) {
        g0 = fmaf(a.c2_wT[k * 3 * H + r], ax[AUX + k], g0);
        g1 = fmaf(a.c2_wT[k * 3 * H + H + r], ax[AUX + k], g1);
        g2 = fmaf(a.c2_wT[k * 3 * H + 2 * H + r], ax[AUX + k], g2);
        y3 = fmaf(a.c3_wT[k * H + r], ax[2 * AUX + k], y3);
        y4 = fmaf(a.c4_wT[k * H + r], ax[3 * AUX + k], y4);
    }
    a.c2f[(size_t)row * 3 * H + r] = g0 + a.b_ih2[r];
    a.c2f[(size_t)row * 3 * H + H + r] = g1 + a.b_ih2[H + r];
    a.c2f[(size_t)row * 3 * H + 2 * H + r] = g2 + a.b_ih2[2 * H + r];
    a.c3f[(size_t)row * H + r] = y3 + a.fc1_b[r];
    a.c4f[(size_t)row * H + r] = y4 + a.fc2_b[r];
}

__device__ __forceinline__ void noise_mol_body(const float *__restrict__ in, float *__restrict__ out, long n, int B, long i0, long stride)
{
    for (long i = i0; i < n; i += stride) {
        const float u = in[i];
        const int col = (int)(i % (11L * B));
        out[i] = (col < 10 * B) ? logf(-logf(u)) : (logf(u) - logf(1.0f - u));
    }
}
__global__ __launch_bounds__(256) void wrnn_noise_mol_kernel(const float *__restrict__ in, float *__restrict__ out, long n, int B)
{
    noise_mol_body(in, out, n, B, (long)blockIdx.x * blockDim.x + threadIdx.x, (long)gridDim.x * blockDim.x);
}

constexpr int SPR = 8;
struct SlabPrepArgs {
    CondArgs c;
    const float *nz_in;
    float *nz_out;
    long nz_n;
    unsigned *xcc;
    int cond_blocks, nz_blocks;
};
__global__ __launch_bounds__(H) void wrnn_slab_prep_kernel(const SlabPrepArgs s)
{
    const int r = threadIdx.x;
    if ((int)blockIdx.x >= s.cond_blocks) {
        const int nb = (int)blockIdx.x - s.cond_blocks;
        if (nb == 0)
            for (int i = r; i < XCC_WORDS; i += H) s.xcc[i] = 0u;
        noise_mol_body(s.nz_in, s.nz_out, s.nz_n, s.c.B, (long)nb * H + r, (long)s.nz_blocks * H);
        return;
    }
    const CondArgs &a = s.c;
    __shared__ float ax[SPR][4 * AUX];
    const int nrows = a.B * a.FPS + 1, row0 = (int)blockIdx.x * SPR;
    for (int q = r; q < SPR * 4 * AUX; q += H) {
        const int i = q / (4 * AUX), e = q % (4 * AUX), row = row0 + i;
        int f = a.NF;
        if (row < a.B * a.FPS) {
            const int b = row / a.FPS, j = row % a.FPS;
            f = (a.seg_pos[b] + a.t0) / a.hop + j;
        }
        ax[i][e] = (f < a.NF) ? a.aux[(size_t)f * 4 * AUX + e] : 0.f;
    }
    __syncthreads();
    float g0[SPR], g1[SPR], g2[SPR], y3[SPR], y4[SPR];
#pragma unroll
    for (int i = 0; i < SPR; ++i) { g0[i] = 0.f; g1[i] = 0.f; g2[i] = 0.f; y3[i] = 0.f; y4[i] = 0.f; }
#pragma unroll 4
    for (int k = 0; k < AUX; ++k) {
        const float w0 = a.c2_wT[k * 3 * H + r], w1 = a.c2_wT[k * 3 * H + H + r], w2 = a.c2_wT[k * 3 * H + 2 * H + r];
        const float w3 = a.c3_wT[k * H + r], w4 = a.c4_wT[k * H + r];
#pragma unroll
        for (int i = 0; i < SPR; ++i) {
            g0[i] = fmaf(w0, ax[i][AUX + k], g0[i]);
            g1[i] = fmaf(w1, ax[i][AUX + k], g1[i]);
            g2[i] = fmaf(w2, ax[i][AUX + k], g2[i]);
            y3[i] = fmaf(w3, ax[i][2 * AUX + k], y3[i]);
            y4[i] = fmaf(w4, ax[i][3 * AUX + k], y4[i]);
        }
    }
    const float b0 = a.b_ih2[r], b1 = a.b_ih2[H + r], b2 = a.b_ih2[2 * H + r], b3 = a.fc1_b[r], b4 = a.fc2_b[r];
#pragma unroll
    for (int i = 0; i < SPR; ++i) {
        const int row = row0 + i;
        if (row < nrows) {
            a.c2f[(size_t)row * 3 * H + r] = g0[i] + b0;
            a.c2f[(size_t)row * 3 * H + H + r] = g1[i] + b1;
            a.c2f[(size_t)row * 3 * H + 2 * H + r] = g2[i] + b2;
            a.c3f[(size_t)row * H + r] = y3[i] + b3;
            a.c4f[(size_t)row * H + r] = y4[i] + b4;
        }
    }
}

hipError_t launch_slab_prep(const CondArgs &a, const float *nz_in, float *nz_out, long nz_n, unsigned *xcc, int n_cus, hipStream_t stream)
{
    SlabPrepArgs s;
    s.c = a; s.nz_in = nz_in; s.nz_out = nz_out; s.nz_n = nz_in ? nz_n : 0; s.xcc = xcc;
    s.cond_blocks = (a.B * a.FPS + 1 + SPR - 1) / SPR;
    long nb = (s.nz_n + H - 1) / H;
    if (nb > (long)n_cus * 4) nb = (long)n_cus * 4;
    if (nb < 1) nb = 1;
    s.nz_blocks = (int)nb;
    hipLaunchKernelGGL(wrnn_slab_prep_kernel, dim3((unsigned)(s.cond_blocks + s.nz_blocks)), dim3(H), 0, stream, s);
    return hipGetLastError();
}

hipError_t launch_noise_mol(const float *in, float *out, long n, int B, int n_cus, hipStream_t stream)
{
    long blocks = (n + 255) / 256;
    if (blocks > (long)n_cus * 8) blocks = (long)n_cus * 8;
    if (blocks < 1) blocks = 1;
    hipLaunchKernelGGL(wrnn_noise_mol_kernel, dim3((unsigned)blocks), dim3(256), 0, stream, in, out, n, B);
    return hipGetLastError();
}

hipError_t launch_cond_frames(const CondArgs &a, hipStream_t stream)
{
    hipLaunchKernelGGL(wrnn_cond_frame_kernel, dim3(a.NF + 1), dim3(H), 0, stream, a);
    return hipGetLastError();
}

hipError_t launch_cond_frames_slab(const CondArgs &a, hipStream_t stream)
{
    hipLaunchKernelGGL(wrnn_cond_frame_slab_kernel, dim3(a.B * a.FPS + 1), dim3(H), 0, stream, a);
    return hipGetLastError();
}

struct PutFloats { float v[64]; };
__global__ void wrnn_put_floats_kernel(float *dst, PutFloats src, int n)
{
    if ((int)threadIdx.x < n) dst[threadIdx.x] = src.v[threadIdx.x];
}
hipError_t launch_put_floats(float *dst, const float *src, int n, hipStream_t stream)
{
    if (n < 1 || n > 64) return hipErrorInvalidValue;
    PutFloats p;
    for (int i = 0; i < 64; ++i) p.v[i] = i < n ? src[i] : 0.f;
    hipLaunchKernelGGL(wrnn_put_floats_kernel, dim3(1), dim3(64), 0, stream, dst, p, n);
    return hipGetLastError();
}

hipError_t launch_cond_frag(const CondArgs &a, int n_cus, hipStream_t stream)
{
    long blocks = (long)(a.t1 - a.t0) * a.NG;
    if (blocks > n_cus) blocks = n_cus;
    if (blocks < 1) blocks = 1;
    hipLaunchKernelGGL(wrnn_cond_frag_kernel, dim3((unsigned)blocks), dim3(256), 0, stream, a);
    return hipGetLastError();
}

hipError_t launch_cond(const CondArgs &a, int n_cus, bool valu, hipStream_t stream)
// ... 19 lines not shown
```

### wavernn_amd/csrc/wrnn_device.h

```cpp
#pragma once
#include <hip/hip_runtime.h>
#include <stdint.h>

namespace wrnn {

struct DeviceGuard {
    int prev = -1;
    hipError_t err;
    explicit DeviceGuard(int device)
    {
        if (hipGetDevice(&prev) != hipSuccess) prev = -1;
        err = (prev == device) ? hipSuccess : hipSetDevice(device);
    }
    ~DeviceGuard() { if (prev >= 0) (void)hipSetDevice(prev); }
    DeviceGuard(const DeviceGuard &) = delete;
    DeviceGuard &operator=(const DeviceGuard &) = delete;
};

typedef float f32x4 __attribute__((ext_vector_type(4)));
typedef unsigned long long u64;

constexpr int H = 512;
constexpr int MEL = 80;
constexpr int AUX = 32;
// ... 14 lines not shown
{
    int ncl = n_cus / 64;
    if (ncl > MAXCL) ncl = MAXCL;
    while (ncl > 1 && (8 % ncl) != 0) --ncl;
    return ncl;
}

struct LoopArgs {
    const float *I_w0;
    const float *w_ih1, *w_hh1;
    const float *b_ih1, *b_hh1;
    const float *w_ih2;
    const float *w_hh2;
    const float *b_hh2;
    const float *fc1_w, *fc2_w;
    const float *fc3_w, *fc3_b;
    const float *w_ih1T, *w_hh1T, *w_ih2T, *w_hh2T;
    const float *fc1T, *fc2T;
    const float *fc3T;
    const float *cI;
    const float *c2f, *c3f, *c4f;
    const float *noise;
    const float *noise_pre;
    const float *sp_vals;
    const int *sp_cols;
    const float *sp_fc_vals;
    const int *sp_fc_cols;
    const float *force_x;
    float *out;
    float *dbg_logits;
    unsigned *status;
    u64 *prof;
    const int *seg_pos, *seg_lim;
    int Btot, b0, nb, T, hop, NF, C;
    int NG;
    float *xbuf;
    float *state;
    const float *cIf;
    int t0, t1, cI_t0, noise_t0;
    int tuning;
    int rb0, Nall, G, resume;
    const float *fc3f;
    const float *u1;
    unsigned hop_magic;
    int hop_shift;
    const float *mels_up, *aux_fr;
    const float *I_cT, *I_b;
    int mel_stage;
    const int *seg_moff;
    const float *mel_coef;
    int tab_fps, tab_t0;
    unsigned *xcc_tab;
    int kind_tag;
};

__device__ __forceinline__ void check_kind(const LoopArgs &a)
{
    if (blockIdx.x == 0 && threadIdx.x == 0) {
        if (!a.resume) a.status[8] = (unsigned)a.kind_tag;
        else if (a.status[8] != (unsigned)a.kind_tag) {
            if (atomicCAS(a.status + 1, 0u, 0x7F0u | (unsigned)a.kind_tag) == 0u) { a.status[2] = a.status[8]; a.status[3] = (unsigned)a.t0; a.status[4] = 0u; }
            __hip_atomic_store(a.status, 1u, __ATOMIC_RELAXED, __HIP_MEMORY_SCOPE_AGENT);
        }
    }
}


struct GenArgs {
    const float *I_T, *I_b;
    const float *w_ih1T, *w_hh1T, *b_ih1, *b_hh1;
    const float *w_ih2T, *w_hh2T, *b_ih2, *b_hh2;
    const float *fc1T, *fc1_b;
    const float *fc2T, *fc2_b;
    const float *fc3T, *fc3_b;
    const float *mels_up, *aux;
    const float *noise;
    const float *force_x;
    float *out, *dbg_logits;
    const int *seg_pos, *seg_lim;
    int H, F, M, A, C, B, T, hop;
};

struct CondArgs {
    const float *mels_up;
    const float *aux;
    const float *I_cT;
    const float *I_b;
    const float *c2_wT;
    const float *b_ih2;
    const float *c3_wT, *fc1_b;
    const float *c4_wT, *fc2_b;
    float *cI, *c2f, *c3f, *c4f;
    const int *seg_pos, *seg_lim;
    int B, T, hop, NF;
    int t0, t1, rb0, NG;
    int FPS;
};

__device__ __forceinline__ float sigmoid_f(float x) { return 1.0f / (1.0f + expf(-x)); }

__device__ __forceinline__ float gru_update(float gi_r, float gi_z, float gi_n, float gh_r, float gh_z,
                                            float gh_n, float h)
{
    const float r = sigmoid_f(gh_r + gi_r);
    const float z = sigmoid_f(gh_z + gi_z);
    const float n = tanhf(gi_n + gh_n * r);
// ... 241 lines not shown
```

### wavernn_amd/csrc/wrnn_duo.hip

```cpp
#include <type_traits>

#include "wrnn_ring.h"

namespace wrnn {

#ifndef DUO_XR_FIRST
#define DUO_XR_FIRST 1
#endif

#ifndef DUO_ABLATE
#define DUO_ABLATE 0
#endif
#ifndef DUO_EI_DEPTH
#define DUO_EI_DEPTH 4
#endif

constexpr int DNWGC = 4 * LNJ;
#ifndef DUO_GH_SHIFT
#define DUO_GH_SHIFT 1
#endif
constexpr int DLOGS = 36;
constexpr int DPART = 2 * NW * 3 * 256;
static_assert(O_HOWN == 768 && O_XS == 1024 && O_SP == 1040, "saved state layout");

// ... 25 lines not shown
            PROFL[k] += now_ - plast;                                          \
            plast = now_;                                                      \
            if (trp && t >= tr_t0 && t < tr_t0 + 3 && ntr < 510)               \
                trp[1 + ntr++] = (now_ << 16) | (u64)(((tri & 15) << 8) | ((k) & 255));   \
        }                                                                      \
    } while (0)
#define TRACE_DECL                                                                                                   \
    u64 *const trp = (PROF && (a.tuning & 16384) && a.prof) ? a.prof + 256 * 32 + (size_t)blockIdx.x * 512 : nullptr; \
    int ntr = 0, tri = 0;                                                                                            \
    const int tr_t0 = a.t0 + (a.t1 - a.t0) / 2;

typedef __attribute__((address_space(3))) void lds_void;
__device__ __forceinline__ void prefetch8(__amdgpu_buffer_rsrc_t rs, float *dst, int voff, int soff)
{
    lds_void *d0 = (lds_void *)dst, *d1 = (lds_void *)(dst + 1024);
    __builtin_amdgcn_raw_ptr_buffer_load_lds(rs, d0, 16, voff, soff, 0, 16 );
    __builtin_amdgcn_raw_ptr_buffer_load_lds(rs, d0, 16, voff, soff, 1024, 16);
    __builtin_amdgcn_raw_ptr_buffer_load_lds(rs, d0, 16, voff, soff, 2048, 16);
    __builtin_amdgcn_raw_ptr_buffer_load_lds(rs, d0, 16, voff, soff, 3072, 16);
    __builtin_amdgcn_raw_ptr_buffer_load_lds(rs, d1, 16, voff + 4096, soff, 0, 16);
    __builtin_amdgcn_raw_ptr_buffer_load_lds(rs, d1, 16, voff + 4096, soff, 1024, 16);
    __builtin_amdgcn_raw_ptr_buffer_load_lds(rs, d1, 16, voff + 4096, soff, 2048, 16);
    __builtin_amdgcn_raw_ptr_buffer_load_lds(rs, d1, 16, voff + 4096, soff, 3072, 16);
}

struct DuoGeo {
    int nact;
    u64 nbpack;
};

template <int MODE, bool LA, bool LP, bool EI, bool PROF>
__device__ __forceinline__ void duo_ih(const LoopArgs &a, float *smem, const int cl, const int J, const int ncl, const bool loc_h, const bool loc_y)
{
    const int G = a.G;
    const DuoLds L = duo_lds(G);
    float *HS = smem + L.off_h, *XS = smem + L.off_xs, *PART = smem + L.off_part;
    int *SEGT = reinterpret_cast<int *>(smem + L.off_seg);
    int *GEO = reinterpret_cast<int *>(smem + L.off_misc);
    u64 *PROFL = reinterpret_cast<u64 *>(smem + L.off_prof);
    u64 plast = 0;
    TRACE_DECL
    const int tid = threadIdx.x, lane = tid & 63, w = __builtin_amdgcn_readfirstlane(tid >> 6);
    const int fi = lane & 15, kq = lane >> 4;
    const int kbase_lane = KCH * w + 4 * kq;
    const int pu = 4 * w + (tid & 3), pj = (tid >> 2) & 15;
    const int prow = LU * J + pu;
    const int T0 = a.t0, T1 = a.t1;
    const int NR = a.Btot, NGR = a.NG;
    unsigned *const status = a.status;
    float *const state = a.state;
    u64 *const profp = a.prof;
    const float *const bhhp = LA ? a.b_hh1 : a.b_hh2;
    const int resume = a.resume, hop = a.hop;
    const int zrow = a.Nall * a.tab_fps;
    constexpr int L_H = LA ? 0 : 1, L_XR = LA ? 5 : 6, L_Y = LA ? 2 : 3, L_GH = LA ? 8 : 12;
    constexpr int L_P0 = LA ? 4 : 5, L_P2 = LA ? 6 : 2;

    float A_ih[3][AF], A_fc[AF];
#pragma unroll
    for (int g = 0; g < 3; ++g) load_afrag(A_ih[g], LA ? a.w_ih1 : a.w_ih2, LA ? H : H + AUX, g * H + LU * J + fi, true, kbase_lane);
    load_afrag(A_fc, LA ? a.fc1_w : a.fc2_w, H + AUX, LU * J + fi, true, kbase_lane);
    float cb_r = 0.f, cb_z = 0.f, cb_n = 0.f, ux_r = 0.f, ux_z = 0.f, ux_n = 0.f, w0o = 0.f;
    if constexpr (LA) {
        cb_r = a.b_ih1[prow]; cb_z = a.b_ih1[H + prow]; cb_n = a.b_ih1[2 * H + prow];
        ux_r = a.u1[prow]; ux_z = a.u1[H + prow]; ux_n = a.u1[2 * H + prow];
        w0o = a.I_w0[prow];
    }

    for (int q = tid; q < L.total; q += NT) smem[q] = 0.f;
    __syncthreads();
    DuoGeo geo;
    geo.nact = 0; geo.nbpack = 0;
    const size_t state_wg = ((size_t)(cl * LNWGC + 2 * J + (LA ? 0 : 1)) * G) * LGRP;
    for (int i = 0; i < G; ++i) {
        const int g = cl + ncl * i;
        if (g >= NGR) break;
        geo.nact = i + 1;
        const int b0 = (int)(((long)g * NR) / NGR), nb = (int)(((long)(g + 1) * NR) / NGR) - b0;
        if (tid == 0) { GEO[2 * i] = a.rb0 + b0; GEO[2 * i + 1] = nb; }
        geo.nbpack |= (u64)(unsigned)nb << (8 * i);
        if (a.resume) {
            const float *sg = a.state + state_wg + (size_t)i * LGRP;
            HS[i * 256 + tid] = sg[O_HOWN + tid];
            if (tid < SEG) XS[i * 16 + tid] = sg[O_XS + tid];
            if (tid < 2 * SEG) SEGT[i * 48 + tid] = reinterpret_cast<const int *>(sg + O_SP)[tid];
        } else if (tid < SEG) {
            const int sc = a.rb0 + b0 + (tid < nb ? tid : nb - 1);
            SEGT[i * 48 + tid] = a.seg_pos[sc];
            SEGT[i * 48 + SEG + tid] = a.seg_lim[sc];
        }
    }
    __syncthreads();
    for (int i = 0; i < geo.nact; ++i) {
        if (tid < SEG) {
            const int nb = (int)((geo.nbpack >> (8 * i)) & 255u);
            const int sc = GEO[2 * i] + (tid < nb ? tid : nb - 1);
            SEGT[i * 48 + 2 * SEG + tid] = sc * a.tab_fps - (SEGT[i * 48 + tid] + a.tab_t0) / a.hop;
        }
    }
    __syncthreads();
    const int nact = geo.nact;
    const u64 nbpack = geo.nbpack;

    const __amdgpu_buffer_rsrc_t xrs = make_rsrc(a.xbuf, (unsigned)(DXBUF_FLOATS * 4));
    const __amdgpu_buffer_rsrc_t crs = make_rsrc(a.c2f, 0x7FFFF000u);
    const __amdgpu_buffer_rsrc_t frs = make_rsrc(LA ? a.c3f : a.c4f, 0x7FFFF000u);
    const int voff_frag = frag_off(w, 0, lane) * 4;
    const int voff_own = (((J * 64) + 16 * w + pj) * 4 + (tid & 3)) * 4;
    const int voff_gh = (256 * (J & 7) + tid) * 16;
    const int cbase = cl * DSLOTB;
    const unsigned magic = a.hop_magic;
    const int mshift = a.hop_shift;

    const int locbits = (loc_h ? 1 : 0) | (loc_y ? 2 : 0);
    const bool late_xo = (a.tuning & 128) == 0, reprobe = (a.tuning & 8) == 0;
    const bool full_chk = !PROF && (a.tuning & 4096) != 0;
    bool dead = false;
    int pp = 0;
    int t = T0;
    int cur = 0;

    struct Carry {
        float c0, c1, c2;
        u32x4 gw;
        unsigned xo, xt;
        int i, pp, t;
    };
    Carry cy;
    cy.c0 = cy.c1 = cy.c2 = 0.f; cy.gw = u32x4{0u, 0u, 0u, 0u}; cy.xo = cy.xt = 0u; cy.i = 0; cy.pp = 0; cy.t = T0;

    auto slot_nb = [&](int i) -> int { return (int)((nbpack >> (8 * i)) & 255u); };

    auto back_gates = [&](const Carry &c) {
        const int bi = c.i, bt = c.t;
        const float *PB = DPARTOF(c.pp);
        const int nb = slot_nb(bi);
        const int sb = cbase + bi * (MAXCL * DSLOTB) + (bt & (DRING - 1)) * XTB;
        const bool live = pj < nb;
        lds_barrier();
        PHX(cur + 1);
        const float pr = get_partial<3>(PB, 0, pu, pj), pz = get_partial<3>(PB, 1, pu, pj), pn = get_partial<3>(PB, 2, pu, pj);
        const float hprev = HS[bi * 256 + tid];
        float ghr, ghz, ghn;
        u32x4 g = c.gw;
        if (bt > T0) {
            const unsigned tag = (unsigned)bt + 1u;
            if (__builtin_expect(__any(live && g.w != tag), 0))
                wait_for([&] { return !__any(live && g.w != tag); },
                         [&] { g = __builtin_amdgcn_raw_buffer_load_b128(xrs, voff_gh, cbase + bi * (MAXCL * DSLOTB) + (L_GH + (J >> 3)) * DLAYERB + (bt & (DGHRING - 1)) * XTB, 16 ); },
                         status, dead, 0x500u | (LA ? 0u : 8u) | 6u, bt);
// ... 793 lines not shown
```

### wavernn_amd/csrc/wrnn_octo.hip

```cpp
#include <type_traits>

#include "wrnn_ring.h"

namespace wrnn {

constexpr int ONT = 512;
constexpr int ONPX = 3;
constexpr int OLOGS = 36;
constexpr int OPXB = NW * 3 * 256 + 256;
constexpr int OXO = NW * 3 * 256;

struct OctoLds {
    int off_op, off_px, off_fcw, off_h, off_gh, off_cv, off_seg, off_xs, off_py, off_log, off_misc, off_cnt, off_prof, total;
};
__host__ __device__ constexpr OctoLds octo_lds(int G)
{
    OctoLds l{};
    int o = 0;
    l.off_op = o;   o += NW * 2048;
    l.off_px = o;   o += ONPX * OPXB;
    l.off_fcw = o;  o += XT;
    l.off_h = o;    o += G * 256;
    l.off_gh = o;   o += G * 768;
    l.off_cv = o;   o += G * 5 * 256;
// ... 180 lines not shown
            else mfma3s(A_hh[0], A_hh[1], A_hh[2], b, o0, o1, o2);
            put_partial<3>(P, w, 0, lane, o0);
            put_partial<3>(P, w, 1, lane, o1);
            put_partial<3>(P, w, 2, lane, o2);
        }
        ocnt_set(CNT + w, kblk + 1u, lane);
        if (PROF) { asm volatile("s_waitcnt lgkmcnt(0)" ::: "memory"); if (lane == 0 && w == 0) pacc[5] += 1; }
        OPHM(kind == 2 ? 4 : 3);
        ++kblk;
        pxi = (pxi + 1 == ONPX) ? 0 : pxi + 1;
    };
    using K0 = std::integral_constant<int, 0>;
    using K1 = std::integral_constant<int, 1>;
    using K2 = std::integral_constant<int, 2>;
    for (; t < T1; ++t) {
#pragma unroll 1
        for (int i = 0; i < nact; ++i) block(K0{}, i);
#pragma unroll 1
        for (int i = 0; i < nact; ++i) {
            block(K1{}, i);
            block(K2{}, i);
        }
    }
    if (PROF && w == 0 && lane == 0 && a.prof)
        for (int k = 0; k < 7; ++k) a.prof[(size_t)(blockIdx.x & 255) * 32 + k] += pacc[k];
}

template <bool LA, bool PROF>
__device__ __forceinline__ void octo_service(const LoopArgs &a, float *smem, const int cl, const int J, const int ncl, const int w, const int lane,
                                             const bool loc_h)
{
    const int G = a.G;
    const OctoLds L = octo_lds(G);
    float *const PX = smem + L.off_px, *const HS = smem + L.off_h, *const GH = smem + L.off_gh, *const XS = smem + L.off_xs;
    float *const PY = smem + L.off_py, *const LOG = smem + L.off_log;
    int *const SEGT = reinterpret_cast<int *>(smem + L.off_seg);
    int *const GEO = reinterpret_cast<int *>(smem + L.off_misc);
    unsigned *const CNT = reinterpret_cast<unsigned *>(smem + L.off_cnt);
    const int tid = w * 64 + lane;
    const int fi = lane & 15, kq = lane >> 4;
    const int kbase_lane = KCH * w + 4 * kq;
    const int pu = 4 * w + (tid & 3), pj = (tid >> 2) & 15;
    const int prow = LU * J + pu;
    const int T0 = a.t0, T1 = a.t1, C = a.C;
    const int NR = a.Btot, Nall = a.Nall, NGR = a.NG;
    unsigned *const status = a.status;
    float *const state = a.state;
    float *const outp = a.out, *const dbgl = a.dbg_logits;
    const float *const forcex = a.force_x, *const noise_pre = a.noise_pre;
    const int Tall = a.T, noise_t0 = a.noise_t0;
    const float *const mels_up = a.mels_up, *const aux_fr = a.aux_fr, *const mel_coef = a.mel_coef;
    const int mel_stage = a.mel_stage;
    const int resume = a.resume, hop = a.hop;
    const int zrow = a.Nall * a.tab_fps;
    const unsigned magic = a.hop_magic;
    const int mshift = a.hop_shift;
    const int tun = a.tuning;
    constexpr int L_H = LA ? 0 : 1, L_XR = LA ? 5 : 6, L_Y = LA ? 2 : 3, L_IN = LA ? 4 : 5;

    const float *bhh = LA ? a.b_hh1 : a.b_hh2;
    const float bh_r = bhh[prow], bh_z = bhh[H + prow], bh_n = bhh[2 * H + prow];
    float cb_r = 0.f, cb_z = 0.f, cb_n = 0.f, ux_r = 0.f, ux_z = 0.f, ux_n = 0.f, w0o = 0.f;
    CondTile ct;
    if constexpr (LA) {
        cb_r = a.b_ih1[prow]; cb_z = a.b_ih1[H + prow]; cb_n = a.b_ih1[2 * H + prow];
        ux_r = a.u1[prow]; ux_z = a.u1[H + prow]; ux_n = a.u1[2 * H + prow];
        w0o = a.I_w0[prow];
        cond_tile_init(ct, a.I_cT, a.I_b, J, lane);
    }

    int nact = 0;
    u64 nbpack = 0;
    for (int i = 0; i < G; ++i) {
        const int g = cl + ncl * i;
        if (g >= NGR) break;
        nact = i + 1;
        const int b0 = (int)(((long)g * NR) / NGR), nb = (int)(((long)(g + 1) * NR) / NGR) - b0;
        nbpack |= (u64)(unsigned)nb << (8 * i);
    }
    auto slot_nb = [&](int i) -> int { return (int)((nbpack >> (8 * i)) & 255u); };
    const size_t state_wg = ((size_t)(cl * LNWGC + 2 * J + (LA ? 0 : 1)) * G) * LGRP;

    const bool sampler = !LA && J < nact;
    float A3[2][AF];
    float b3a = 0.f, b3b = 0.f;
    if constexpr (!LA) {
        load_afrag(A3[0], a.fc3_w, H, fi, sampler, kbase_lane);
        load_afrag(A3[1], a.fc3_w, H, 16 + fi, sampler && 16 + fi < 30, kbase_lane);
        if (sampler) {
            b3a = a.fc3_b[pu];
            b3b = (16 + pu < 30) ? a.fc3_b[16 + pu] : 0.f;
        }
    }

    const __amdgpu_buffer_rsrc_t xrs = make_rsrc(a.xbuf, (unsigned)(DXBUF_FLOATS * 4));
    const __amdgpu_buffer_rsrc_t crs = make_rsrc(a.c2f, 0x7FFFF000u);
    const __amdgpu_buffer_rsrc_t frs = make_rsrc(LA ? a.c3f : a.c4f, 0x7FFFF000u);
    const int voff_frag = frag_off(w, 0, lane) * 4;
    const int voff_own = (((J * 64) + 16 * w + pj) * 4 + (tid & 3)) * 4;
    const int cbase = cl * DSLOTB;

    bool dead = false;
    u64 *const pacc = reinterpret_cast<u64 *>(smem + L.off_prof) + 8;
    u64 plast = PROF ? __builtin_amdgcn_s_memtime() : 0;
    unsigned kblk = 0, ksync = 0;
    int pxi = 0;
    int t = T0;
// ... 322 lines not shown
        const int ok_a = (tid < LNJ) ? (v != 0u && (int)v == TAB[0]) : 1;
        const int ok_b = (tid >= LNJ && tid < LNWGC) ? (v != 0u && (int)v == TAB[LNJ]) : 1;
        loc_a = __syncthreads_and(ok_a) != 0;
        loc_b = __syncthreads_and(ok_b) != 0;
        if (a.tuning & 256) { loc_a = false; loc_b = false; }
        __syncthreads();
    }
    for (int q = tid; q < L.total; q += ONT) smem[q] = 0.f;
    __syncthreads();
    {
        const float *Wfc = layer == 0 ? a.fc1_w : a.fc2_w;
        float *FCW = smem + L.off_fcw;
        for (int q = tid; q < XT / 4; q += ONT) {
            const int lq = q & 63, r = (q >> 6) & 7, wq = q >> 9;
            reinterpret_cast<float4 *>(FCW)[q] = *reinterpret_cast<const float4 *>(Wfc + (size_t)(LU * J + (lq & 15)) * (H + AUX) + KCH * wq + 16 * r + 4 * (lq >> 4));
        }
        float *HS = smem + L.off_h, *GH = smem + L.off_gh, *XS = smem + L.off_xs;
        int *SEGT = reinterpret_cast<int *>(smem + L.off_seg);
        int *GEO = reinterpret_cast<int *>(smem + L.off_misc);
        const size_t state_wg = ((size_t)(cl * LNWGC + 2 * J + layer) * G) * LGRP;
        const float *bhh = layer == 0 ? a.b_hh1 : a.b_hh2;
        const int NR = a.Btot, NGR = a.NG;
        for (int i = 0; i < G; ++i) {
            const int g = cl + ncl * i;
            if (g >= NGR) break;
            const int b0 = (int)(((long)g * NR) / NGR), nb = (int)(((long)(g + 1) * NR) / NGR) - b0;
            if (tid == 0) { GEO[2 * i] = a.rb0 + b0; GEO[2 * i + 1] = nb; }
            if (tid < 256) {
                const int pu = 4 * (tid >> 6) + (tid & 3);
                const int prow = LU * J + pu;
                if (a.resume) {
                    const float *sg = a.state + state_wg + (size_t)i * LGRP;
                    HS[i * 256 + tid] = sg[O_HOWN + tid];
                    GH[i * 768 + tid] = sg[tid]; GH[i * 768 + 256 + tid] = sg[256 + tid]; GH[i * 768 + 512 + tid] = sg[512 + tid];
                    if (tid < SEG) XS[i * 16 + tid] = sg[O_XS + tid];
                    if (tid < 2 * SEG) SEGT[i * 64 + tid] = reinterpret_cast<const int *>(sg + O_SP)[tid];
                } else {
                    GH[i * 768 + tid] = bhh[prow]; GH[i * 768 + 256 + tid] = bhh[H + prow]; GH[i * 768 + 512 + tid] = bhh[2 * H + prow];
                    if (tid < SEG) {
                        const int sc = a.rb0 + b0 + (tid < nb ? tid : nb - 1);
                        SEGT[i * 64 + tid] = a.seg_pos[sc];
                        SEGT[i * 64 + SEG + tid] = a.seg_lim[sc];
                    }
                }
            }
        }
        __syncthreads();
        for (int i = 0; i < G; ++i) {
            const int g = cl + ncl * i;
            if (g >= NGR) break;
            const int b0 = (int)(((long)g * NR) / NGR), nb = (int)(((long)(g + 1) * NR) / NGR) - b0;
            if (tid < SEG) {
                const int sc = a.rb0 + b0 + (tid < nb ? tid : nb - 1);
                SEGT[i * 64 + 2 * SEG + tid] = sc * a.tab_fps - (SEGT[i * 64 + tid] + a.tab_t0) / a.hop;
                SEGT[i * 64 + 3 * SEG + tid] = a.mel_stage ? a.seg_moff[sc] : 0;
            }
        }
        __syncthreads();
    }
#ifndef OCTO_ROLES
#define OCTO_ROLES 15
#endif
    const int w = w8 & 3;
    if (w8 < 4) {
        if (layer == 0) { if constexpr ((OCTO_ROLES & 1) != 0) octo_matrix<true, PROF>(a, smem, cl, J, ncl, w, lane); }
        else { if constexpr ((OCTO_ROLES & 2) != 0) octo_matrix<false, PROF>(a, smem, cl, J, ncl, w, lane); }
    } else {
        if (layer == 0) { if constexpr ((OCTO_ROLES & 4) != 0) octo_service<true, PROF>(a, smem, cl, J, ncl, w, lane, loc_a); }
        else { if constexpr ((OCTO_ROLES & 8) != 0) octo_service<false, PROF>(a, smem, cl, J, ncl, w, lane, loc_b); }
    }
}

size_t octo_lds_bytes(int G) { return (size_t)octo_lds(G).total * sizeof(float); }
constexpr int OMAXG = 4;
static_assert(sizeof(float) * (size_t)octo_lds(OMAXG).total <= 160 * 1024, "LDS carve");
int octo_max_depth() { return OMAXG; }

hipError_t launch_octo(const LoopArgs &args, int ncl, int mode, hipStream_t stream)
{
    if (ncl < 1 || args.G < 1 || args.G > OMAXG || mode != 1 || !args.u1 || !args.xcc_tab) return hipErrorInvalidValue;
    const size_t lds = octo_lds_bytes(args.G);
    const void *fn = args.prof ? (const void *)wrnn_octo_kernel<true> : (const void *)wrnn_octo_kernel<false>;
    hipError_t e = hipFuncSetAttribute(fn, hipFuncAttributeMaxDynamicSharedMemorySize, (int)lds);
    if (e != hipSuccess) return e;
    LoopArgs a = args;
    void *params[] = {(void *)&a};
    return hipLaunchCooperativeKernel(fn, dim3(ncl * LNWGC), dim3(ONT), params, (unsigned)lds, stream);
}

}
```

### wavernn_amd/csrc/wrnn_pre.hip

```cpp
#include <math.h>
#include <stdio.h>
#include <string.h>
#include <vector>

#include "wrnn_device.h"
#include "../../include/wavernn_amd.h"

namespace wrnn {

constexpr int PC = 128;
constexpr int PFEAT = MEL;
constexpr int PK = 5;
constexpr int PPAD = 2;
constexpr int PKIN = PFEAT * PK;
constexpr int PLDI = 516;
constexpr int PLDX = 132;
constexpr int PNF = 16;

struct PreArgs {
    const float *mel;
    const float *conv_in_w;
    const float *bn_in;
    const float *res_w;
    const float *res_bn;
// ... 177 lines not shown
        float acc = 0.f;
        for (int k = 0; k < C; ++k) acc = fmaf(a.conv_out_w[(size_t)r * C + k], XA[j * C + k], acc);
        if (j0 + j < N) a.aux[(size_t)(j0 + j) * R + r] = acc + a.conv_out_b[r];
    }
}

template <bool FIRST, bool LAST, int S, int F>
__device__ __forceinline__ void upstage_body(const float *__restrict__ in, float *__restrict__ out, const float *__restrict__ taps, int n_in, int s_rt,
                                             int pad, int indent, int feat_rt, long blk, long nblk)
{
    const int s = S > 0 ? S : s_rt;
    const int feat = F > 0 ? F : feat_rt;
    const long n_out = (long)n_in * s;
    const long total = LAST ? (n_out - 2L * indent) * feat : n_out * feat;
    const int ld_in = FIRST ? n_in - 2 * pad : n_in;
    for (long idx = blk * blockDim.x + threadIdx.x; idx < total; idx += nblk * blockDim.x) {
        int c;
        long q;
        if (LAST) { c = (int)(idx % feat); q = idx / feat + indent; }
        else { c = (int)(idx / n_out); q = idx % n_out; }
        float acc = 0.f;
#pragma unroll
        for (int j = 0; j <= 2 * s; ++j) {
            const long u = q + j - s;
            float v = 0.f;
            if (u >= 0 && u < n_out) {
                int f = (int)(u / s);
                if (FIRST) { f -= pad; v = (f >= 0 && f < ld_in) ? in[(size_t)c * ld_in + f] : 0.f; }
                else v = in[(size_t)c * ld_in + f];
            }
            acc = fmaf(taps[j], v, acc);
        }
        if (LAST) out[(size_t)(q - indent) * feat + c] = acc;
        else out[(size_t)c * n_out + q] = acc;
    }
}
template <bool FIRST, bool LAST, int S, int F = PFEAT>
__global__ __launch_bounds__(256) void wrnn_upstage_kernel(const float *__restrict__ in, float *__restrict__ out,
                                                           const float *__restrict__ taps, int n_in, int s_rt, int pad, int indent, int feat_rt = PFEAT)
{
    upstage_body<FIRST, LAST, S, F>(in, out, taps, n_in, s_rt, pad, indent, feat_rt, blockIdx.x, gridDim.x);
}
template <bool FIRST, bool LAST, int S>
__global__ __launch_bounds__(256) void wrnn_upstage_many_kernel(const PreUttDev *__restrict__ utt, int n_utt, const float *__restrict__ taps)
{
    constexpr int stage = FIRST ? 1 : 2;
    const int u = pre_find_utt(utt, n_utt, stage, blockIdx.x);
    const int nf = utt[u].n + 2 * PPAD, n_in = FIRST ? nf : nf * 5;
    const float *in = FIRST ? utt[u].mel : utt[u].s1;
    float *out = FIRST ? utt[u].s1 : (LAST ? utt[u].up : utt[u].s2);
    upstage_body<FIRST, LAST, S, PFEAT>(in, out, taps, n_in, S, PPAD, 0, PFEAT, blockIdx.x - utt[u].blk[stage], utt[u + 1].blk[stage] - utt[u].blk[stage]);
}

template <int S>
__device__ __forceinline__ void upstage_last_body(const float *__restrict__ in, float *__restrict__ out, const float *__restrict__ taps, int n_in, int s_rt,
                                                  int indent, long blk, long nblk)
{
    constexpr int TQ = 64;
    __shared__ float tile[TQ][PFEAT + 1];
    const int s = S > 0 ? S : s_rt;
    const long n_out = (long)n_in * s, nq = n_out - 2L * indent;
    for (long q0 = blk * TQ; q0 < nq; q0 += nblk * TQ) {
        for (int e = threadIdx.x; e < TQ * PFEAT; e += 256) {
            const int c = e / TQ, ql = e % TQ;
            const long q = q0 + ql + indent;
            float acc = 0.f;
            if (q0 + ql < nq) {
#pragma unroll
                for (int j = 0; j <= 2 * s; ++j) {
                    const long u = q + j - s;
                    float v = 0.f;
                    if (u >= 0 && u < n_out) v = in[(size_t)c * n_in + (int)(u / s)];
                    acc = fmaf(taps[j], v, acc);
                }
            }
            tile[ql][c] = acc;
        }
        __syncthreads();
        for (int e = threadIdx.x; e < TQ * PFEAT; e += 256) {
            const int ql = e / PFEAT, c = e % PFEAT;
            if (q0 + ql < nq) out[(size_t)(q0 + ql) * PFEAT + c] = tile[ql][c];
        }
        __syncthreads();
    }
}
template <int S>
__global__ __launch_bounds__(256) void wrnn_upstage_last_kernel(const float *__restrict__ in, float *__restrict__ out,
                                                                const float *__restrict__ taps, int n_in, int s_rt, int indent)
{
    upstage_last_body<S>(in, out, taps, n_in, s_rt, indent, blockIdx.x, gridDim.x);
}
template <int S>
__global__ __launch_bounds__(256) void wrnn_upstage_last_many_kernel(const PreUttDev *__restrict__ utt, int n_utt, const float *__restrict__ taps, int indent)
{
    const int u = pre_find_utt(utt, n_utt, 3, blockIdx.x);
    upstage_last_body<S>(utt[u].s2, utt[u].up, taps, (utt[u].n + 2 * PPAD) * 25, S, indent, blockIdx.x - utt[u].blk[3], utt[u + 1].blk[3] - utt[u].blk[3]);
}

}

using namespace wrnn;

static thread_local char g_pre_err[384] = "";
extern "C" const char *wrnn_pre_last_error(void) { return g_pre_err; }
#define PRE_FAIL(code, ...)                                  \
    do {                                                     \
        snprintf(g_pre_err, sizeof g_pre_err, __VA_ARGS__);  \
        return code;                                         \
    } while (0)
#define PRE_HIP(expr)                                                                                   \
    do {                                                                                                \
        hipError_t e_ = (expr);                                                                         \
        if (e_ != hipSuccess) PRE_FAIL(WRNN_ERR_HIP, "%s failed: %s", #expr, hipGetErrorString(e_));    \
    } while (0)

struct wrnn_pre {
    int device, blocks, scales[3], total_scale;
    int feat, C, R, pad;
    int gf;
    float *dev;
    const float *conv_in_w, *bn_in, *res_w, *res_bn, *conv_out_w, *conv_out_b, *taps[3];
};

static size_t generic_lds_bytes(int feat, int C, int pad, int gf) { return ((size_t)feat * (gf + 2 * pad) + 2 * (size_t)gf * C) * sizeof(float); }

static int pre_check_dims(const wrnn_pre_weights *w, int *gf_out)
{
    if (w->feat_dims < 1 || w->feat_dims > 4096 || w->compute_dims < 1 || w->compute_dims > 4096 || w->res_out_dims < 1 || w->res_out_dims > 4096 ||
        w->pad < 0 || w->pad > 64 || w->res_blocks < 0 || w->res_blocks > 64)
        PRE_FAIL(WRNN_ERR_ARG, "bad UpsampleNetwork dims: feat_dims %d, compute_dims %d, res_out_dims %d, pad %d, res_blocks %d", w->feat_dims,
                 w->compute_dims, w->res_out_dims, w->pad, w->res_blocks);
    for (int i = 0; i < 3; ++i)
        if (w->upsample_factors[i] < 1 || w->upsample_factors[i] > 64) PRE_FAIL(WRNN_ERR_ARG, "bad upsample factor %d", w->upsample_factors[i]);
    const int FE = w->feat_dims, C = w->compute_dims, R = w->res_out_dims, PD = w->pad;
    const bool shipped_dims = FE == PFEAT && C == PC && R == PC && PD == PPAD;
    int gf = 0;
    if (!shipped_dims) {
        for (gf = 16; gf >= 1 && generic_lds_bytes(FE, C, PD, gf) > 65536; gf >>= 1) {}
        if (gf < 1) PRE_FAIL(WRNN_ERR_ARG, "UpsampleNetwork too wide for the pre-loop kernel (feat_dims %d, compute_dims %d, pad %d)", FE, C, PD);
    }
    *gf_out = gf;
    return WRNN_OK;
}

static void pre_set_dims(wrnn_pre *p, const wrnn_pre_weights *w, int device, int gf)
{
    p->device = device; p->blocks = w->res_blocks; p->total_scale = 1;
    p->feat = w->feat_dims; p->C = w->compute_dims; p->R = w->res_out_dims; p->pad = w->pad; p->gf = gf;
    for (int i = 0; i < 3; ++i) { p->scales[i] = w->upsample_factors[i]; p->total_scale *= w->upsample_factors[i]; }
}

extern "C" int wrnn_pre_debug_host_handle(const wrnn_pre_weights *w, wrnn_pre **out)
{
    if (!w || !out) PRE_FAIL(WRNN_ERR_ARG, "NULL argument");
    int gf = 0;
    const int rc = pre_check_dims(w, &gf);
    if (rc != WRNN_OK) return rc;
    wrnn_pre *p = new wrnn_pre();
    pre_set_dims(p, w, -1, gf);
    *out = p;
    return WRNN_OK;
}

extern "C" int wrnn_pre_create(const wrnn_pre_weights *w, int device, wrnn_pre **out)
{
    if (!w || !out) PRE_FAIL(WRNN_ERR_ARG, "NULL argument");
    int gf = 0;
    const int rc_dims = pre_check_dims(w, &gf);
    if (rc_dims != WRNN_OK) return rc_dims;
    if (!w->conv_in_w || !w->bn_in || (w->res_blocks && (!w->res_w || !w->res_bn)) || !w->conv_out_w || !w->conv_out_b || !w->up_w)
        PRE_FAIL(WRNN_ERR_ARG, "NULL weight pointer");
    const int FE = w->feat_dims, C = w->compute_dims, R = w->res_out_dims, PD = w->pad, KT = 2 * PD + 1;
    int n = 0;
    if (hipGetDeviceCount(&n) != hipSuccess || n <= 0 || device >= n) PRE_FAIL(WRNN_ERR_NO_DEVICE, "no HIP device %d (count %d)", device, n);
    DeviceGuard dg(device);
    PRE_HIP(dg.err);
    const int B = w->res_blocks;
    const double eps = 1e-5;
    std::vector<float> h;
    auto put = [&](const float *src, size_t cnt) { size_t o = (h.size() + 63) / 64 * 64; h.resize(o + cnt); if (src) memcpy(h.data() + o, src, cnt * 4); return o; };
    auto fold = [&](const float *bn, size_t o) {
        for (int c = 0; c < C; ++c) {
            const float s = bn[c] / sqrtf(bn[3 * C + c] + (float)eps);
            h[o + c] = s;
            h[o + C + c] = bn[C + c] - bn[2 * C + c] * s;
        }
    };
    const size_t o_cin = put(w->conv_in_w, (size_t)C * FE * KT);
    const size_t o_bnin = put(nullptr, 2 * (size_t)C);
    fold(w->bn_in, o_bnin);
    const size_t o_resw = put(w->res_w, (size_t)B * 2 * C * C);
    const size_t o_resbn = put(nullptr, (size_t)B * 2 * 2 * C);
    for (int i = 0; i < 2 * B; ++i) fold(w->res_bn + (size_t)i * 4 * C, o_resbn + (size_t)i * 2 * C);
    const size_t o_cow = put(w->conv_out_w, (size_t)R * C), o_cob = put(w->conv_out_b, R);
    size_t o_t[3], toff = 0;
    for (int i = 0; i < 3; ++i) { o_t[i] = put(w->up_w + toff, 2 * w->upsample_factors[i] + 1); toff += 2 * w->upsample_factors[i] + 1; }
    put(nullptr, 64);
    wrnn_pre *p = new wrnn_pre();
    pre_set_dims(p, w, device, gf);
    hipError_t e = hipMalloc((void **)&p->dev, h.size() * 4);
    if (e != hipSuccess) { delete p; PRE_FAIL(WRNN_ERR_HIP, "hipMalloc failed: %s", hipGetErrorString(e)); }
    e = hipMemcpy(p->dev, h.data(), h.size() * 4, hipMemcpyHostToDevice);
    if (e != hipSuccess) { (void)hipFree(p->dev); delete p; PRE_FAIL(WRNN_ERR_HIP, "hipMemcpy failed: %s", hipGetErrorString(e)); }
    p->conv_in_w = p->dev + o_cin; p->bn_in = p->dev + o_bnin; p->res_w = p->dev + o_resw; p->res_bn = p->dev + o_resbn;
    p->conv_out_w = p->dev + o_cow; p->conv_out_b = p->dev + o_cob;
    for (int i = 0; i < 3; ++i) p->taps[i] = p->dev + o_t[i];
    *out = p;
    return WRNN_OK;
}

extern "C" void wrnn_pre_destroy(wrnn_pre *p)
{
    if (!p) return;
    if (p->dev) (void)hipFree(p->dev);
    delete p;
}

extern "C" int wrnn_pre_hop(const wrnn_pre *p) { return p ? p->total_scale : 0; }

extern "C" size_t wrnn_pre_workspace_bytes(const wrnn_pre *p, int32_t n_frames)
{
    if (!p || n_frames < 1) return 0;
    const size_t nf = (size_t)n_frames + 2 * p->pad;
    return (nf * p->scales[0] + nf * p->scales[0] * p->scales[1]) * p->feat * sizeof(float) + 512;
}

static int pre_run(const wrnn_pre *p, const float *mel, int32_t n_frames, float *mels_up, float *aux,
                   void *workspace, size_t workspace_bytes, void *stream_, bool rows_only)
{
    if (!p || !mel || !mels_up || !aux || !workspace) PRE_FAIL(WRNN_ERR_ARG, "NULL argument");
    if (n_frames < 1 || (double)n_frames * p->total_scale > 2.0e9) PRE_FAIL(WRNN_ERR_ARG, "bad n_frames %d", n_frames);
    if (workspace_bytes < wrnn_pre_workspace_bytes(p, n_frames)) PRE_FAIL(WRNN_ERR_WORKSPACE, "workspace too small");
    if (((uintptr_t)workspace & 255) != 0) PRE_FAIL(WRNN_ERR_ARG, "workspace must be 256-byte aligned");
    if (p->device < 0) PRE_FAIL(WRNN_ERR_NO_DEVICE, "a dims-only handle (wrnn_pre_debug_host_handle) launches nothing");
    hipStream_t stream = (hipStream_t)stream_;
    DeviceGuard dg(p->device);
    PRE_HIP(dg.err);
    PreArgs a;
    a.mel = mel; a.conv_in_w = p->conv_in_w; a.bn_in = p->bn_in; a.res_w = p->res_w; a.res_bn = p->res_bn;
    a.conv_out_w = p->conv_out_w; a.conv_out_b = p->conv_out_b; a.aux = aux; a.N = n_frames; a.blocks = p->blocks;
    const int FE = p->feat, PD = p->pad;
    if (p->gf == 0) hipLaunchKernelGGL(wrnn_resnet_kernel, dim3((n_frames + PNF - 1) / PNF), dim3(256), 0, stream, a);
    else {
        GenPreArgs g;
        g.p = a; g.feat = FE; g.C = p->C; g.R = p->R; g.pad = PD; g.gf = p->gf;
        hipLaunchKernelGGL(wrnn_resnet_generic_kernel, dim3((n_frames + p->gf - 1) / p->gf), dim3(256), generic_lds_bytes(FE, p->C, PD, p->gf), stream, g);
    }
    const int nf = n_frames + 2 * PD;
    float *s1 = (float *)workspace;
    float *s2 = s1 + (size_t)nf * p->scales[0] * FE;
    auto grid = [](long total) { long b = (total + 255) / 256; return (unsigned)(b > 65535 ? 65535 : (b < 1 ? 1 : b)); };
    const bool feat80 = FE == PFEAT;
    const bool shipped = feat80 && PD == PPAD && p->scales[0] == 5 && p->scales[1] == 5 && p->scales[2] == 11;
    const unsigned g1 = grid((long)nf * p->scales[0] * FE), g2 = grid((long)nf * p->scales[0] * p->scales[1] * FE);
    const unsigned g3 = grid((long)n_frames * p->total_scale * 4);
    const int n2 = nf * p->scales[0], n3 = n2 * p->scales[1], indent = PD * p->total_scale;
    if (rows_only) {
        if (shipped) {
            hipLaunchKernelGGL((wrnn_upstage_kernel<true, false, 5>), dim3(g1), dim3(256), 0, stream, mel, s1, p->taps[0], nf, 5, PD, 0, PFEAT);
            hipLaunchKernelGGL((wrnn_upstage_kernel<false, true, 5>), dim3(g2), dim3(256), 0, stream, s1, mels_up, p->taps[1], n2, 5, 0, 0, PFEAT);
        } else {
            hipLaunchKernelGGL((wrnn_upstage_kernel<true, false, 0, 0>), dim3(g1), dim3(256), 0, stream, mel, s1, p->taps[0], nf, p->scales[0], PD, 0, FE);
            hipLaunchKernelGGL((wrnn_upstage_kernel<false, true, 0, 0>), dim3(g2), dim3(256), 0, stream, s1, mels_up, p->taps[1], n2, p->scales[1], 0, 0, FE);
        }
    } else if (shipped) {
        hipLaunchKernelGGL((wrnn_upstage_kernel<true, false, 5>), dim3(g1), dim3(256), 0, stream, mel, s1, p->taps[0], nf, 5, PD, 0, PFEAT);
        hipLaunchKernelGGL((wrnn_upstage_kernel<false, false, 5>), dim3(g2), dim3(256), 0, stream, s1, s2, p->taps[1], n2, 5, 0, 0, PFEAT);
        hipLaunchKernelGGL((wrnn_upstage_last_kernel<11>), dim3(g3), dim3(256), 0, stream, s2, mels_up, p->taps[2], n3, 11, indent);
    } else {
        hipLaunchKernelGGL((wrnn_upstage_kernel<true, false, 0, 0>), dim3(g1), dim3(256), 0, stream, mel, s1, p->taps[0], nf, p->scales[0], PD, 0, FE);
        hipLaunchKernelGGL((wrnn_upstage_kernel<false, false, 0, 0>), dim3(g2), dim3(256), 0, stream, s1, s2, p->taps[1], n2, p->scales[1], 0, 0, FE);
        if (feat80) hipLaunchKernelGGL((wrnn_upstage_last_kernel<0>), dim3(g3), dim3(256), 0, stream, s2, mels_up, p->taps[2], n3, p->scales[2], indent);
        else hipLaunchKernelGGL((wrnn_upstage_kernel<false, true, 0, 0>), dim3(grid((long)n_frames * p->total_scale * FE)), dim3(256), 0, stream, s2, mels_up, p->taps[2], n3, p->scales[2], 0, indent, FE);
    }
    PRE_HIP(hipGetLastError());
    return WRNN_OK;
}

extern "C" int wrnn_pre_upsample(const wrnn_pre *p, const float *mel, int32_t n_frames, float *mels_up, float *aux,
                                 void *workspace, size_t workspace_bytes, void *stream)
{
    return pre_run(p, mel, n_frames, mels_up, aux, workspace, workspace_bytes, stream, false);
}

extern "C" int wrnn_pre_upsample_rows(const wrnn_pre *p, const float *mel, int32_t n_frames, float *mel_rows, float *aux,
                                      void *workspace, size_t workspace_bytes, void *stream)
{
    return pre_run(p, mel, n_frames, mel_rows, aux, workspace, workspace_bytes, stream, true);
}

static size_t al256(size_t x) { return (x + 255) & ~(size_t)255; }
static bool pre_many_batched(const wrnn_pre *p) { return p->gf == 0 && p->scales[0] == 5 && p->scales[1] == 5 && p->scales[2] == 11; }
static size_t pre_many_slice(const wrnn_pre *p, int32_t n_frames, bool rows_only, size_t *s2_off)
{
    if (!pre_many_batched(p)) return al256(wrnn_pre_workspace_bytes(p, n_frames));
    const size_t nf = (size_t)n_frames + 2 * p->pad, s1 = al256(nf * p->scales[0] * p->feat * sizeof(float));
    if (s2_off) *s2_off = s1;
    return s1 + (rows_only ? 0 : al256(nf * p->scales[0] * p->scales[1] * p->feat * sizeof(float)));
}

extern "C" size_t wrnn_pre_workspace_bytes_many(const wrnn_pre *p, const wrnn_pre_utt *utts, int32_t n_utt, int32_t rows_only)
{
    if (!p || !utts || n_utt < 1) return 0;
    size_t total = al256((size_t)(n_utt + 1) * sizeof(PreUttDev));
    for (int u = 0; u < n_utt; ++u) {
        if (utts[u].n_frames < 1) return 0;
        total += pre_many_slice(p, utts[u].n_frames, rows_only != 0, nullptr);
    }
    return total;
}

extern "C" int wrnn_pre_upsample_many(const wrnn_pre *p, const wrnn_pre_utt *utts, int32_t n_utt, int32_t rows_only, float *mels_up, float *aux,
                                      void *workspace, size_t workspace_bytes, void *stream_)
{
    if (!p || !mels_up || !aux || !workspace) PRE_FAIL(WRNN_ERR_ARG, "NULL argument");
    if (!utts) PRE_FAIL(WRNN_ERR_ARG, "NULL utterance table");
    if (n_utt < 1 || n_utt > 65536) PRE_FAIL(WRNN_ERR_ARG, "bad utterance count %d (1 .. 65536 per call)", n_utt);
    for (int u = 0; u < n_utt; ++u) {
        if (utts[u].n_frames < 1 || (double)utts[u].n_frames * p->total_scale > 2.0e9) PRE_FAIL(WRNN_ERR_ARG, "utterance %d: bad n_frames %d", u, utts[u].n_frames);
        if (!utts[u].mel || utts[u].up_row < 0 || utts[u].aux_row < 0) PRE_FAIL(WRNN_ERR_ARG, "utterance %d: NULL mel or negative output offset", u);
    }
    const size_t need = wrnn_pre_workspace_bytes_many(p, utts, n_utt, rows_only);
    if (workspace_bytes < need) PRE_FAIL(WRNN_ERR_ARG, "workspace too small: %zu bytes, wrnn_pre_workspace_bytes_many says %zu", workspace_bytes, need);
    if (((uintptr_t)workspace & 255) != 0) PRE_FAIL(WRNN_ERR_ARG, "workspace must be 256-byte aligned");
    if (p->device < 0) PRE_FAIL(WRNN_ERR_NO_DEVICE, "a dims-only handle (wrnn_pre_debug_host_handle) launches nothing");
    const bool rows = rows_only != 0;
    char *ws = (char *)workspace;
    size_t off = al256((size_t)(n_utt + 1) * sizeof(PreUttDev));
    if (!pre_many_batched(p)) {
        for (int u = 0; u < n_utt; ++u) {
            const size_t slice = pre_many_slice(p, utts[u].n_frames, rows, nullptr);
            const int rc = pre_run(p, utts[u].mel, utts[u].n_frames, mels_up + (size_t)utts[u].up_row * p->feat, aux + (size_t)utts[u].aux_row * p->R,
                                   ws + off, slice, stream_, rows);
            if (rc != WRNN_OK) return rc;
            off += slice;
        }
        return WRNN_OK;
    }
    hipStream_t stream = (hipStream_t)stream_;
    DeviceGuard dg(p->device);
    PRE_HIP(dg.err);
    auto grid = [](long total) { long b = (total + 255) / 256; return (long)(b > 65535 ? 65535 : (b < 1 ? 1 : b)); };
    std::vector<PreUttDev> tab((size_t)n_utt + 1);
    long blk[4] = {0, 0, 0, 0};
    for (int u = 0; u < n_utt; ++u) {
        const int n = utts[u].n_frames;
        const long nf = (long)n + 2 * PPAD;
        size_t s2_off = 0;
        const size_t slice = pre_many_slice(p, n, rows, &s2_off);
        PreUttDev &d = tab[u];
        d.mel = utts[u].mel; d.up = mels_up + (size_t)utts[u].up_row * PFEAT; d.aux = aux + (size_t)utts[u].aux_row * PC;
        d.s1 = (float *)(ws + off); d.s2 = rows ? nullptr : (float *)(ws + off + s2_off);
        d.n = n; d.pad_ = 0;
        for (int s = 0; s < 4; ++s) d.blk[s] = (int)blk[s];
        blk[0] += (n + PNF - 1) / PNF;
        blk[1] += grid(nf * 5 * PFEAT);
        blk[2] += grid(nf * 25 * PFEAT);
        blk[3] += rows ? 0 : grid((long)n * p->total_scale * 4);
        for (int s = 0; s < 4; ++s)
            if (blk[s] > 0x7fffffffL) PRE_FAIL(WRNN_ERR_ARG, "too many frames for one call (stage grid of %ld workgroups); split the table", blk[s]);
        off += slice;
    }
    memset(&tab[n_utt], 0, sizeof(PreUttDev));
    for (int s = 0; s < 4; ++s) tab[n_utt].blk[s] = (int)blk[s];
    PreUttDev *d_tab = (PreUttDev *)ws;
    PRE_HIP(hipMemcpyAsync(d_tab, tab.data(), tab.size() * sizeof(PreUttDev), hipMemcpyHostToDevice, stream));
    PreManyArgs m;
    memset(&m, 0, sizeof m);
    m.w.conv_in_w = p->conv_in_w; m.w.bn_in = p->bn_in; m.w.res_w = p->res_w; m.w.res_bn = p->res_bn;
    m.w.conv_out_w = p->conv_out_w; m.w.conv_out_b = p->conv_out_b; m.w.blocks = p->blocks;
    m.utt = d_tab; m.n_utt = n_utt;
    hipLaunchKernelGGL(wrnn_resnet_many_kernel, dim3((unsigned)blk[0]), dim3(256), 0, stream, m);
    hipLaunchKernelGGL((wrnn_upstage_many_kernel<true, false, 5>), dim3((unsigned)blk[1]), dim3(256), 0, stream, d_tab, n_utt, p->taps[0]);
    if (rows) {
        hipLaunchKernelGGL((wrnn_upstage_many_kernel<false, true, 5>), dim3((unsigned)blk[2]), dim3(256), 0, stream, d_tab, n_utt, p->taps[1]);
    } else {
        hipLaunchKernelGGL((wrnn_upstage_many_kernel<false, false, 5>), dim3((unsigned)blk[2]), dim3(256), 0, stream, d_tab, n_utt, p->taps[1]);
        hipLaunchKernelGGL((wrnn_upstage_last_many_kernel<11>), dim3((unsigned)blk[3]), dim3(256), 0, stream, d_tab, n_utt, p->taps[2], PPAD * p->total_scale);
    }
    PRE_HIP(hipGetLastError());
    return WRNN_OK;
}
```

### wavernn_amd/csrc/wrnn_sparse.hip

```cpp
#include <type_traits>

#include "wrnn_ring.h"
#include "wrnn_raw.h"

namespace wrnn {

constexpr int SPCLUSTERS = 16;
constexpr int SPWG = 16;
constexpr int SPPART = 2 * NW * 2 * 256;
constexpr int SPSTATE_WG = NT * 16 + SEG;
constexpr int SPSTATE_CL = SPWG * SPSTATE_WG;
static_assert(SPCLUSTERS <= LMAXG * MAXCL, "one exchange-buffer region per cluster");
static_assert(SPCLUSTERS * SPWG <= XCC_WORDS, "placement table");

struct SpLds {
    int off_seg, off_part, off_log, off_misc, off_prof, off_ct1, off_f3, off_lgt, off_seg1, total;
};
__host__ __device__ inline SpLds sp_lds(bool raw = false, int slots = 1)
{
    SpLds l;
    int o = 0;
    l.off_seg = o;  o += 64;
    l.off_part = o; o += SPPART;
    l.off_log = o;  o += 32;
// ... 96 lines not shown

__device__ __forceinline__ unsigned max4(const u32x4 &q) { return max(max(q.x, q.y), max(q.z, q.w)); }
typedef unsigned u32x2 __attribute__((ext_vector_type(2)));
#define SPX(k)                                                                 \
    do {                                                                       \
        if (PROF && tid == 0) {                                                \
            const u64 now_ = __builtin_amdgcn_s_memtime();                     \
            PROFL[k] += now_ - plast;                                          \
            plast = now_;                                                      \
        }                                                                      \
    } while (0)

__device__ __forceinline__ void mfma2(const float (&a0)[AF], const float (&a1)[AF], const float (&b)[32], f32x4 &o0, f32x4 &o1)
{
    f32x4 c00 = mfma_ag0(a0[0], b[0]), c10 = mfma_ag0(a1[0], b[0]), c01 = mfma_ag0(a0[4], b[4]), c11 = mfma_ag0(a1[4], b[4]);
#pragma unroll
    for (int r = 0; r < 8; r += 2) {
#pragma unroll
        for (int e = 0; e < 4; ++e) {
            if (r + e > 0) {
                mfma_ag(c00, a0[4 * r + e], b[4 * r + e]);
                mfma_ag(c10, a1[4 * r + e], b[4 * r + e]);
                mfma_ag(c01, a0[4 * r + 4 + e], b[4 * r + 4 + e]);
                mfma_ag(c11, a1[4 * r + 4 + e], b[4 * r + 4 + e]);
            }
        }
    }
    asm volatile("s_nop 15\n\ts_nop 7" : "+v"(c00), "+v"(c10), "+v"(c01), "+v"(c11));
    o0 = c00 + c01;
    o1 = c10 + c11;
}

template <int NBP, bool FCS, int MODE, bool LA, bool PROF, int NS>
__device__ __forceinline__ void sp_role(const LoopArgs &a, float *smem, const int rg, const int gid, const int ub, const int wgi, const bool loc)
{
    constexpr int MPW = NBP / 4;
    constexpr bool MOL = MODE == 1;
    static_assert(NS == 1 || (NS == 2 && MOL && FCS && !PROF), "two groups per cluster: MOL with gathered fc stages");
    const SpLds L = sp_lds(!MOL, NS);
    float *PART = smem + L.off_part, *fc3b = smem + L.off_log, *F3 = smem + L.off_f3, *LGT = smem + L.off_lgt;
    u64 *PROFL = reinterpret_cast<u64 *>(smem + L.off_prof);
    u64 plast = 0;
    const int tid = threadIdx.x, lane = tid & 63, w = __builtin_amdgcn_readfirstlane(tid >> 6);
    const int fi = lane & 15, kq = lane >> 4;
    const int rb = 4 * ub + w;
    const int u0 = LU * rb + 4 * kq;
    const int kbase_lane = KCH * w + 4 * kq;
    const int pu = 4 * w + (tid & 3), pj = (tid >> 2) & 15;
    const int T0 = a.t0, T1 = a.t1;
    unsigned *const status = a.status;
    const int hop = a.hop, resume = a.resume, Tall = a.T, Nall = a.Nall, noise_t0 = a.noise_t0, C = a.C;
    const unsigned magic = a.hop_magic;
    const int mshift = a.hop_shift;
    const int zrow = a.Nall * a.tab_fps;
    float *const outp = a.out, *const dbgl = a.dbg_logits;
    const float *const forcex = a.force_x, *const noise_pre = a.noise_pre, *const noise_raw = a.noise;
    const float *const mels_up = a.mels_up, *const aux_fr = a.aux_fr, *const mel_coef = a.mel_coef;
    const int mel_stage = a.mel_stage;
    const int NR = a.Btot, NGR = a.NG;
    constexpr int L_H = LA ? 0 : 1, L_XR = LA ? 5 : 6, L_IN = LA ? 4 : 5;
    SpSlot sl[NS];
#pragma unroll
    for (int s = 0; s < NS; ++s) {
        const int g = gid + SPCLUSTERS * s;
        const bool there = NS == 1 || g < NGR;
        const int b0 = there ? (int)(((long)g * NR) / NGR) : 0;
        sl[s].nb = there ? (int)(((long)(g + 1) * NR) / NGR) - b0 : 0;
        sl[s].b0g = a.rb0 + b0;
        sl[s].cbase = (rg + SPCLUSTERS * s) * DSLOTB;
        sl[s].state_wg = a.state + (size_t)g * SPSTATE_CL + (size_t)wgi * SPSTATE_WG;
        sl[s].SEGT = reinterpret_cast<int *>(smem + (s == 0 ? L.off_seg : L.off_seg1));
    }
    const bool sampler = !LA && (ub == 0 || (!MOL && ub >= 5));
    const int sidx = ub == 0 ? 0 : ub - 4;

    GateTiles<MPW> gi, gh;
    gate_tiles_init(gi, a.sp_vals, a.sp_cols, LA ? 0 : 2, rb, lane);
    gate_tiles_init(gh, a.sp_vals, a.sp_cols, LA ? 1 : 3, rb, lane);
    float A_fc1[2][AF], A_fc2[2][AF];
    FcTile<MPW> ft;
    if constexpr (FCS) fc_tile_init(ft, a.sp_fc_vals, a.sp_fc_cols, w >> 1, 2 * wgi + (w & 1), lane);
    else {
#pragma unroll
        for (int q = 0; q < 2; ++q) {
            load_afrag(A_fc1[q], a.fc1_w, H + AUX, 2 * LU * wgi + LU * q + fi, true, kbase_lane);
            load_afrag(A_fc2[q], a.fc2_w, H + AUX, 2 * LU * wgi + LU * q + fi, true, kbase_lane);
        }
    }
    const bool fold3 = MOL && FCS && (a.tuning & 16) == 0;
    float A3[2][4];
    if constexpr (FCS && MOL) {
#pragma unroll
        for (int q = 0; q < 2; ++q)
#pragma unroll
            for (int e = 0; e < 4; ++e) A3[q][e] = (16 * q + fi < C) ? a.fc3_w[(size_t)(16 * q + fi) * H + LU * (2 * wgi + (w & 1)) + 4 * kq + e] : 0.f;
    }
    for (int q = tid; q < L.off_f3; q += NT) smem[q] = 0.f;
    if constexpr (MOL) {
        if (sampler) {
            for (int q = tid; q < 2 * XT / 4; q += NT) reinterpret_cast<float4 *>(F3)[q] = reinterpret_cast<const float4 *>(a.fc3f)[q];
        }
    } else {
        for (int q = tid; q < 2 * XT / 4; q += NT) {
            const int l6 = q & 63, r = (q >> 6) & 7, wv = (q >> 9) & 3, tile = q >> 11;
            const float *src = a.fc3_w + (size_t)(32 * wgi + 16 * tile + (l6 & 15)) * H + 128 * wv + 16 * r + 4 * (l6 >> 4);
            reinterpret_cast<float4 *>(F3)[q] = make_float4(src[0], src[1], src[2], src[3]);
        }
    }
    float b3r[2] = {0.f, 0.f};
    if constexpr (!MOL) { b3r[0] = a.fc3_b[32 * wgi + pu]; b3r[1] = a.fc3_b[32 * wgi + 16 + pu]; }
    float cb[3][4], ux[3][4], w0o[4], bh[3][4];
#pragma unroll
    for (int g = 0; g < 3; ++g)
#pragma unroll
        for (int e = 0; e < 4; ++e) {
            cb[g][e] = LA ? a.b_ih1[g * H + u0 + e] : 0.f;
            ux[g][e] = LA ? a.u1[g * H + u0 + e] : 0.f;
            bh[g][e] = (LA ? a.b_hh1 : a.b_hh2)[g * H + u0 + e];
        }
#pragma unroll
    for (int e = 0; e < 4; ++e) w0o[e] = LA ? a.I_w0[u0 + e] : 0.f;
    const float b3a = sampler ? a.fc3_b[pu] : 0.f, b3b = (sampler && 16 + pu < 30) ? a.fc3_b[16 + pu] : 0.f;
    const bool cond_wg = !LA && ub >= 1;
    const bool cond2 = cond_wg && ub <= 4 && w == 0;
    const int cblk0 = cond_wg ? 4 * (ub - 1) + w : 0, cblk1 = cond2 ? 27 + ub : 0;
    float *CT0 = smem + L.off_ct1 + w * 64 * (CK + 4), *CT1 = smem + L.off_ct1 + 4 * 64 * (CK + 4);
    __syncthreads();
    if (MOL && sampler && tid >= 32 && tid < 64) fc3b[tid - 32] = tid - 32 < 30 ? a.fc3_b[tid - 32] : 0.f;
    if (cond_wg) {
        CondTile c1;
        cond_tile_init(c1, a.I_cT, a.I_b, cblk0, lane);
#pragma unroll
        for (int kk = 0; kk < CK; ++kk) CT0[kk * 64 + lane] = c1.w[kk];
#pragma unroll
        for (int i = 0; i < 4; ++i) CT0[(CK + i) * 64 + lane] = c1.bias[i];
        if (cond2) {
            cond_tile_init(c1, a.I_cT, a.I_b, cblk1, lane);
#pragma unroll
            for (int kk = 0; kk < CK; ++kk) CT1[kk * 64 + lane] = c1.w[kk];
#pragma unroll
            for (int i = 0; i < 4; ++i) CT1[(CK + i) * 64 + lane] = c1.bias[i];
        }
    }
#pragma unroll
    for (int s = 0; s < NS; ++s) {
        SP_SLOT(sl[s]);
        if (tid < SEG && (NS == 1 || nb > 0)) {
            const int sc = b0g + (tid < nb ? tid : nb - 1);
            const int pos = a.seg_pos[sc];
            SEGT[tid] = pos;
            SEGT[SEG + tid] = a.seg_lim[sc];
            SEGT[2 * SEG + tid] = sc * a.tab_fps - (pos + a.tab_t0) / a.hop;
            SEGT[3 * SEG + tid] = a.mel_stage ? a.seg_moff[sc] : 0;
        }
    }
    __syncthreads();

    const __amdgpu_buffer_rsrc_t xrs = make_rsrc(a.xbuf, (unsigned)(DXBUF_FLOATS * 4));
    const __amdgpu_buffer_rsrc_t crs = make_rsrc(a.c2f, 0x7FFFF000u);
    const __amdgpu_buffer_rsrc_t f1rs = make_rsrc(a.c3f, 0x7FFFF000u), f2rs = make_rsrc(a.c4f, 0x7FFFF000u);
    const int voff_frag = frag_off(w, 0, lane) * 4;
    const int voff_blk = rb * 1024 + lane * 16;
    const int voff_own = u0 * 64 + fi * 4;

    bool dead = false;
    int pp = 0;
    int t = T0;
#pragma unroll
    for (int s = 0; s < NS; ++s) {
    sl[s].live = fi < sl[s].nb;
    SP_SLOT(sl[s]);
    own = u32x4{0u, 0u, 0u, 0u};
#pragma unroll
    for (int e = 0; e < 4; ++e) h[e] = 0.f;
    gacc[0] = gacc[1] = gacc[2] = f32x4{0.f, 0.f, 0.f, 0.f};
    if (resume && (NS == 1 || nb > 0)) {
        const float4 hv = *reinterpret_cast<const float4 *>(state_wg + tid * 16), r4 = *reinterpret_cast<const float4 *>(state_wg + tid * 16 + 4),
                     z4 = *reinterpret_cast<const float4 *>(state_wg + tid * 16 + 8), n4 = *reinterpret_cast<const float4 *>(state_wg + tid * 16 + 12);
        h[0] = hv.x; h[1] = hv.y; h[2] = hv.z; h[3] = hv.w;
        ghr[0] = r4.x; ghr[1] = r4.y; ghr[2] = r4.z; ghr[3] = r4.w; ghz[0] = z4.x; ghz[1] = z4.y; ghz[2] = z4.z; ghz[3] = z4.w;
        ghn[0] = n4.x; ghn[1] = n4.y; ghn[2] = n4.z; ghn[3] = n4.w;
    } else {
#pragma unroll
        for (int e = 0; e < 4; ++e) { ghr[e] = bh[0][e]; ghz[e] = bh[1][e]; ghn[e] = bh[2][e]; }
    }
    }

    auto store4 = [&](const u32x4 &q, int voff_layer, int soff) {
#pragma unroll
        for (int e = 0; e < 4; ++e) {
            if (loc) __builtin_amdgcn_raw_buffer_store_b32(q[e], xrs, voff_layer + voff_own + 64 * e, soff, 0);
            else __builtin_amdgcn_raw_buffer_store_b32(q[e], xrs, voff_layer + voff_own + 64 * e, soff, 16 );
        }
    };
    auto load_own = [&](int soff) {
        u32x4 q;
#pragma unroll
        for (int e = 0; e < 4; ++e) q[e] = __builtin_amdgcn_raw_buffer_load_b32(xrs, voff_own + 64 * e, soff, 16 );
        return q;
    };
    auto store16 = [&](const u32x4 &q, int voff, int soff) {
        if (loc) __builtin_amdgcn_raw_buffer_store_b128(q, xrs, voff, soff, 0);
        else __builtin_amdgcn_raw_buffer_store_b128(q, xrs, voff, soff, 16 );
    };
    auto rearm = [&](SpSlot &S) {
// ... 533 lines not shown
```

### wavernn_amd/engine.py

```python
import ctypes
import numpy as np
import torch

from . import _lib

LOOP_KEYS = dict(I_w='I.weight', I_b='I.bias', w_ih1='rnn1.weight_ih_l0', w_hh1='rnn1.weight_hh_l0',
                 b_ih1='rnn1.bias_ih_l0', b_hh1='rnn1.bias_hh_l0', w_ih2='rnn2.weight_ih_l0', w_hh2='rnn2.weight_hh_l0',
                 b_ih2='rnn2.bias_ih_l0', b_hh2='rnn2.bias_hh_l0', fc1_w='fc1.weight', fc1_b='fc1.bias',
                 fc2_w='fc2.weight', fc2_b='fc2.bias', fc3_w='fc3.weight', fc3_b='fc3.bias')


RESUMABLE_KERNELS = ('wrnn_loop_kernel', 'wrnn_duo_kernel', 'wrnn_sparse_kernel', 'wrnn_chain_kernel')
MEL_STAGE_KERNELS = ('wrnn_duo_kernel', 'wrnn_sparse_kernel', 'wrnn_chain_kernel')
KERNEL_ALGOS = {'wrnn_sparse_kernel': ('sparse', 'duo'), 'wrnn_chain_kernel': ('chain', 'duo'), 'wrnn_octo_kernel': ('octo', 'duo'),
                'wrnn_duo_kernel': ('duo', 'loop'), 'wrnn_loop_kernel': ('loop', None)}
FALLBACK_ALGO = {k: nxt for k, (_, nxt) in KERNEL_ALGOS.items() if nxt}


class MelRows:

    def __init__(self, rows, L, scale, taps, seg_off):
        self.rows, self.L, self.scale = rows, int(L), int(scale)
        self.taps = np.ascontiguousarray(taps, dtype=np.float32).reshape(-1)
        self.seg_off = seg_off
        if self.taps.shape[0] != 2 * self.scale + 1:
            raise ValueError('the last stage has 2 * scale + 1 taps')

    @property
    def shape(self):
        return self.rows.shape


def _as_host_f32(v):
    if isinstance(v, torch.Tensor):
        v = v.detach().to('cpu', torch.float32).numpy()
    return np.ascontiguousarray(v, dtype=np.float32)


class LoopEngine:

    def __init__(self, state_dict, mode, device=None):
        if not torch.cuda.is_available():
            raise _lib.WrnnError('wavernn_amd needs a HIP device (torch.cuda.is_available() is False); '
                                 'there is no CPU fallback')
        self.lib = _lib.lib()
        self.device = torch.device('cuda', torch.cuda.current_device()) if device is None else torch.device(device)
        self._dev_index = self.device.index if self.device.index is not None else torch.cuda.current_device()
        self.mode = mode
        host = {k: _as_host_f32(state_dict[v]) for k, v in LOOP_KEYS.items()}
        w = _lib.Weights()
        w.rnn_dims = host['w_hh1'].shape[1]
        w.fc_dims = host['fc1_w'].shape[0]
        w.aux_dims = host['w_ih2'].shape[1] - w.rnn_dims
        w.feat_dims = host['I_w'].shape[1] - 1 - w.aux_dims
        w.n_classes = host['fc3_w'].shape[0]
        if mode not in ('RAW', 'MOL'):
            raise RuntimeError("Unknown model mode value - ", mode)
        w.mode = _lib.MODE_MOL if mode == 'MOL' else _lib.MODE_RAW
        for k, a in host.items():
            setattr(w, k, a.ctypes.data)
        self.n_classes = int(w.n_classes)
        self.feat_dims, self.aux_dims = int(w.feat_dims), int(w.aux_dims)
        pack = ctypes.c_void_p()
        _lib.check(self.lib.wrnn_pack_create(ctypes.byref(w), self._dev_index, ctypes.byref(pack)), 'wrnn_pack_create')
        self._pack = pack
        self._ws = None
        self.n_cus = self.lib.wrnn_device_cus(self._dev_index)
        if mode == 'RAW' and min(float(np.count_nonzero(host[k])) / host[k].size for k in ('w_ih1', 'w_hh1', 'w_ih2', 'w_hh2')) < 0.5:
            import warnings
# ... 88 lines not shown
        n_frames = int(aux.shape[0])
        o = self.options(algo, depth, clusters, slab_steps, cond_valu, t_range, tuning, sparse_groups, lib_noise)
        if lib_noise:
            o.noise_seed = int(noise_seed) & (2 ** 64 - 1)
            if noise_seg_id is not None:
                noise_seg_id = np.ascontiguousarray(noise_seg_id, dtype=np.uint64)
                if noise_seg_id.shape != (B,):
                    raise ValueError('noise_seg_id: one 64-bit id per segment')
                o.noise_seg_id = noise_seg_id.ctypes.data
        nbytes = int(self.lib.wrnn_workspace_bytes_segments(self._pack, B, T, n_frames, ctypes.byref(o)))
        if nbytes == 0:
            raise _lib.WrnnError('bad geometry / options: ' + self.lib.wrnn_last_error().decode())
        if self._ws is None or self._ws.numel() < nbytes:
            if t0 > 0:
                raise _lib.WrnnError('continuing a call needs the workspace of the call it continues')
            self._ws = None
            self._ws = torch.empty(nbytes, dtype=torch.uint8, device=self.device)
        if out is None:
            out = torch.empty(B, T, dtype=torch.float32, device=self.device)
        if force_x is not None:
            force_x = force_x.to(self.device, torch.float32).contiguous()
            assert force_x.shape == (B, T)
            o.force_x = force_x.data_ptr()
        if want_logits:
            if logits is None:
                logits = torch.empty(T, B, self.n_classes, dtype=torch.float32, device=self.device)
            o.logits = logits.data_ptr()
        if phase_clocks is not None:
            o.phase_clocks = phase_clocks.data_ptr()
        if progress is not None:
            thunk = _lib.PROGRESS_FN(lambda done, T_, n_, user: progress(int(done), int(T_), int(n_)))
            self._progress_keep.append(thunk)
            o.progress = ctypes.cast(thunk, ctypes.c_void_p)
        o.timer = self._timer
        o.info = ctypes.pointer(self._info)
        if rows_in is not None:
            seg_moff = np.ascontiguousarray(np.broadcast_to(np.asarray(rows_in.seg_off, dtype=np.int32), (B,)))
            o.mel_stage, o.mel_rows, o.mel_scale = 1, int(mels_up.shape[0]), rows_in.scale
            o.mel_taps, o.seg_moff = rows_in.taps.ctypes.data, seg_moff.ctypes.data
        stream = torch.cuda.current_stream(self.device).cuda_stream
        rc = self.lib.wrnn_generate_segments(self._pack, B, T, seg_pos.ctypes.data, seg_lim.ctypes.data, L, hop, n_frames,
                                             mels_up.data_ptr(), aux.data_ptr(), None if lib_noise else noise.data_ptr(), out.data_ptr(),
                                             self._ws.data_ptr(), self._ws.numel(), ctypes.byref(o), stream)
        if rc == _lib.ERR_RESIDENCY and t0 == 0 and (algo == 'auto' or _fallback):
            import warnings
            why = self.lib.wrnn_last_error().decode()
            planned = _lib.RunInfo()
            self.lib.wrnn_plan_segments(self._pack, B, T, ctypes.byref(o), ctypes.byref(planned))
            nxt = FALLBACK_ALGO.get((planned.kernel or b'').decode())
            if rows_in is not None and nxt != 'duo':
                raise _lib.ResidencyError('cooperative launch refused (' + why + ')')
            if rows_in is not None:
                mels_up = rows_in
            if nxt is not None:
                warnings.warn('wavernn_amd: cooperative launch refused (' + why + '); trying algo = ' + nxt)
                self._ws = None
                if progress is not None:
                    self._progress_keep.pop()
                res = self.run_segments(mels_up, aux, seg_pos, seg_lim, T, noise, hop, algo=nxt, depth=depth, clusters=clusters, force_x=force_x,
                                        want_logits=want_logits, check=check, slab_steps=slab_steps, cond_valu=cond_valu, t_range=t_range, out=out,
                                        logits=logits, phase_clocks=phase_clocks, tuning=tuning, progress=progress, noise_seed=noise_seed, noise_seg_id=noise_seg_id, _fallback=True)
                if algo == 'auto':
                    self._auto_floor = self._auto_floor or nxt
                return res
            if t1 == T:
                warnings.warn('wavernn_amd: cooperative launch refused (' + why + '); using the stream kernel')
                if progress is not None:
                    self._progress_keep.pop()
                if algo == 'auto':
                    self._auto_floor = 'stream'
                return self.run_segments(mels_up, aux, seg_pos, seg_lim, T, noise, hop, algo='stream', force_x=force_x,
                                         want_logits=want_logits, check=check, slab_steps=slab_steps, cond_valu=cond_valu, out=out, logits=logits,
                                         phase_clocks=phase_clocks, tuning=tuning, progress=progress, noise_seed=noise_seed, noise_seg_id=noise_seg_id)
            raise _lib.ResidencyError('cooperative launch refused (' + why + ')')
        _lib.check(rc, 'wrnn_generate_segments')
        self._launches = (self._launches if t0 > 0 else 0) + int(self._info.launches)
        if t0 == 0:
            self._slice_algo = KERNEL_ALGOS.get((self._info.kernel or b'').decode(), (None, None))[0]
        self._last_opts = (B, T, n_frames, self.options(algo, depth, clusters, slab_steps, cond_valu, None, 0, sparse_groups, lib_noise))
        if check:
            rc = self.lib.wrnn_status(self._ws.data_ptr(), stream)
            del self._progress_keep[:]
            _lib.check(rc, 'loop kernel')
        return (out, logits) if want_logits else out

    def status(self):
        stream = torch.cuda.current_stream(self.device).cuda_stream
        rc = self.lib.wrnn_status(self._ws.data_ptr(), stream)
        del self._progress_keep[:]
        _lib.check(rc, 'loop kernel')

    def read_exchange(self, cluster, slot, layer, ring):
        B, T, n_frames, o = self._last_opts
        host = np.zeros((16, 512), np.float32)
        _lib.check(self.lib.wrnn_debug_read_exchange(self._pack, self._ws.data_ptr(), B, T, n_frames, ctypes.byref(o), cluster,
                                                     slot, layer, ring, host.ctypes.data), 'wrnn_debug_read_exchange')
        return host

    def last_loop_split(self):
        i = self._info
        return int(i.units_per_wg), int(i.clusters), int(i.depth)

    def last_run_info(self):
        i = self._info
        return dict(kernel=(i.kernel or b'').decode(), units_per_wg=int(i.units_per_wg), clusters=int(i.clusters), depth=int(i.depth),
                    rounds=int(i.rounds), slab_steps=int(i.slab_steps), launches=int(self._launches))
# ... 7 lines not shown
```

### wavernn_amd/model.py

```python
import sys
import time
from pathlib import Path
from typing import Union

import numpy as np
import torch
import torch.nn as nn
import torch.nn.functional as F

from . import _lib
from . import fold as _fold
from .dsp import save_wav
from .engine import LoopEngine, LOOP_KEYS, RESUMABLE_KERNELS, MEL_STAGE_KERNELS
from .rng import burn_ctor_draws, draw_steps


class ResBlock(nn.Module):

    def __init__(self, dims):
        super().__init__()
        self.conv1 = nn.Conv1d(dims, dims, kernel_size=1, bias=False)
        self.conv2 = nn.Conv1d(dims, dims, kernel_size=1, bias=False)
        self.batch_norm1 = nn.BatchNorm1d(dims)
        self.batch_norm2 = nn.BatchNorm1d(dims)
# ... 46 lines not shown

    def aux_frames(self, m):
        return self.resnet(m)

    def upsample_mel(self, m):
        m = m.unsqueeze(1)
        for f in self.up_layers:
            m = f(m)
        return m.squeeze(1)[:, :, self.indent:-self.indent].transpose(1, 2)

    def forward(self, m):
        aux = self.resnet_stretch(self.aux_frames(m).unsqueeze(1)).squeeze(1)
        return self.upsample_mel(m), aux.transpose(1, 2)


class WaveRNN(nn.Module):
    def __init__(self, rnn_dims, fc_dims, bits, pad, upsample_factors, feat_dims, compute_dims, res_out_dims,
                 res_blocks, hop_length, sample_rate, mode='RAW'):
        super().__init__()
        self.mode = mode
        self.pad = pad
        if self.mode == 'RAW':
            self.n_classes = 2 ** bits
        elif self.mode == 'MOL':
            self.n_classes = 30
        else:
            RuntimeError("Unknown model mode value - ", self.mode)
        self.rnn_dims = rnn_dims
        self.aux_dims = res_out_dims // 4
        self.hop_length = hop_length
        self.sample_rate = sample_rate

        self.upsample = UpsampleNetwork(feat_dims, upsample_factors, compute_dims, res_blocks, res_out_dims, pad)
        self.I = nn.Linear(feat_dims + self.aux_dims + 1, rnn_dims)
        self.rnn1 = nn.GRU(rnn_dims, rnn_dims, batch_first=True)
        self.rnn2 = nn.GRU(rnn_dims + self.aux_dims, rnn_dims, batch_first=True)
        self.fc1 = nn.Linear(rnn_dims + self.aux_dims, fc_dims)
        self.fc2 = nn.Linear(fc_dims + self.aux_dims, fc_dims)
        self.fc3 = nn.Linear(fc_dims, self.n_classes)
        self.register_buffer('step', torch.zeros(1, dtype=torch.long))
        self.num_params()

        self.noise_source = 'cpu'
        self.noise_seed = 0
        self.noise_key = 0
        self.loop_algo = 'auto'
        self.sparse_groups = None
        self.pre_algo = 'native'
        self.pre_batched = True
        self.pre_streams = 8
        self.pinned_output = True
        self.post_tables_early = True
        self.slab_prep_split = False
        self.mel_in_loop = None
        self.post_algo = 'native'
        self.noise_chunk_bytes = 2 << 30
        self.progress_callback = None
        self._engine = None
        self._engine_key = None
        self._pre = None
        self._pre_key = None
        self.last_loop_ms = None
        self.last_loop_kernel = None

    def forward(self, x, mels):
        self.step += 1
        bsize = x.size(0)
        device = x.device
        h1 = torch.zeros(1, bsize, self.rnn_dims, device=device)
        h2 = torch.zeros(1, bsize, self.rnn_dims, device=device)
        mels, aux = self.upsample(mels)
        d = self.aux_dims
        a1, a2, a3, a4 = (aux[:, :, d * i:d * (i + 1)] for i in range(4))
        x = self.I(torch.cat([x.unsqueeze(-1), mels, a1], dim=2))
        res = x
        x, _ = self.rnn1(x, h1)
        x = x + res
        res = x
        x, _ = self.rnn2(torch.cat([x, a2], dim=2), h2)
        x = x + res
        x = F.relu(self.fc1(torch.cat([x, a3], dim=2)))
        x = F.relu(self.fc2(torch.cat([x, a4], dim=2)))
        return self.fc3(x)

    def invalidate_engines(self):
        self._engine = self._pre = self._engine_key = self._pre_key = None

    @staticmethod
    def _weights_key(sd):
        return tuple((k, v.data_ptr(), str(v.device), tuple(v.shape), str(v.dtype), int(v._version)) for k, v in sorted(sd.items()))

    def _loop_engine(self):
        sd = {k: v for k, v in self.state_dict().items() if k in LOOP_KEYS.values()}
        key = self._weights_key(sd)
        if self._engine is None or key != self._engine_key:
            dev = next(self.parameters()).device
            self._engine = LoopEngine(sd, self.mode, device=dev)
            self._engine_key = key
        return self._engine

    def _pre_engine(self):
        from .pre import PreEngine
        sd = {k: v for k, v in self.state_dict().items() if k.startswith('upsample.')}
        key = self._weights_key(sd)
        if self._pre is None or key != self._pre_key:
            self._pre = PreEngine(sd, device=next(self.parameters()).device)
# ... 77 lines not shown
            burn_ctor_draws(self.rnn_dims, self.aux_dims, self.noise_source)
            per_step = B * (11 if self.mode == 'MOL' else self.n_classes) * 4
            resumable = eng.plan(B, T, algo=self.loop_algo)['kernel'] in RESUMABLE_KERNELS
            chunk = max(1, min(T, self.noise_chunk_bytes // per_step)) if (resumable and self.noise_source != 'library') else T
            chunk = -(-T // (-(-T // chunk)))
            rng_state = torch.get_rng_state() if (self.noise_source == 'cpu' and (chunk < T or rows)) else None
            algo = self.loop_algo
            groups = self.loop_sparse_groups(eng, B, T)
            import warnings
            try:
                out = self._run_sliced(eng, mels_up, aux, B, T, stride, chunk, algo, device, groups)
            except _lib.ResidencyError as e:
                if rng_state is not None:
                    torch.set_rng_state(rng_state)
                if rows:
                    warnings.warn(f'wavernn_amd: {e}; up-sampling the mel in full for the other loop kernels')
                    mels_up, aux, _ = self.conditioning(mels)
                    try:
                        out = self._run_sliced(eng, mels_up, aux, B, T, stride, chunk, algo, device, groups)
                        e = None
                    except _lib.ResidencyError as e2:
                        e = e2
                        if rng_state is not None:
                            torch.set_rng_state(rng_state)
                if e is not None:
                    warnings.warn(f'wavernn_amd: {e}; using the stream kernel')
                    out = self._run_sliced(eng, mels_up, aux, B, T, stride, T, 'stream', device)
            self.last_loop_ms = eng.last_loop_ms()
            self.last_loop_kernel = eng.last_loop_kernel()

        if self.post_algo == 'native':
            from .post import unfold_on_device
            wav, _ = unfold_on_device(out, [0], [B], [wave_len], overlap, self.hop_length, self.n_classes, mu_law, batched)
            output = wav.cpu().numpy()
        else:
            output = out.cpu().numpy().astype(np.float64)
            if mu_law:
                output = _fold.decode_mu_law(output, self.n_classes, False)
            if batched:
                output = _fold.xfade_and_unfold(output, target, overlap)
            else:
                output = output[0]
            output = _fold.finish_waveform(output, wave_len, self.hop_length)
        save_wav(output, save_path, self.sample_rate)
        self.train()
        return output

    def _run_sliced(self, eng, mels_up, aux, B, T, stride, chunk, algo, device, sparse_groups=0):
        out = None
        prog = None
        if self.progress_callback is not None:
            t_start, cb = time.perf_counter(), self.progress_callback
            prog = lambda done, T_, n_: cb(done, T_, n_, time.perf_counter() - t_start)
        if self.noise_source == 'library':
            from .batch import library_seg_ids
            return eng.run(mels_up, aux, B, T, stride, None, self.hop_length, algo=algo, progress=prog, sparse_groups=sparse_groups,
                           noise_seed=self.noise_key, noise_seg_id=library_seg_ids(self.noise_seed, B))
        for t0 in range(0, T, chunk):
            t1 = min(T, t0 + chunk)
            noise = draw_steps(self.mode, B, t1 - t0, self.n_classes, device, self.noise_source)
            out = eng.run(mels_up, aux, B, T, stride, noise, self.hop_length, algo=algo, out=out,
                          t_range=None if (t0 == 0 and t1 == T) else (t0, t1), progress=prog, sparse_groups=sparse_groups)
        return out

    def gen_display(self, i, seq_len, b_size, gen_rate):
        bar_len = 16
        done = (i * bar_len) // max(1, seq_len)
        pbar = ''.join(chr(0x2588) if k < done else chr(0x2591) for k in range(bar_len))
        msg = f'| {pbar} {i * b_size}/{seq_len * b_size} | Batch Size: {b_size} | Gen Rate: {gen_rate:.1f}kHz | '
        sys.stdout.write(f'\r{msg}')

    def pad_tensor(self, x, pad, side='both'):
        return _fold.pad_tensor(x, pad, side)

    def fold_with_overlap(self, x, target, overlap):
        return _fold.fold_with_overlap(x, target, overlap)

    def xfade_and_unfold(self, y, target, overlap):
        return _fold.xfade_and_unfold(y, target, overlap)

    def get_step(self):
        return self.step.data.item()

    def log(self, path, msg):
        with open(path, 'a') as f:
            print(msg, file=f)

    def load(self, path: Union[str, Path]):
        device = next(self.parameters()).device
        self.load_state_dict(torch.load(path, map_location=device), strict=False)

    def save(self, path: Union[str, Path]):
        torch.save(self.state_dict(), path)

    def num_params(self, print_out=True):
        n = sum(int(np.prod(p.size())) for p in self.parameters() if p.requires_grad) / 1_000_000
        if print_out:
            print('Trainable Parameters: %.3fM' % n)
        return n
```

Measured before the change: 11.24 million.

## Add opt-in whole-call aux tables and vectorized last upsample stage

Adds a tuning bit that builds the per-frame aux conditioning tables once for the whole call, instead of rebuilding per-segment tables for every slab. Slabs can then be larger, and per-slab conditioning launches are skipped after the first. It also adds a non-reference variant of the last upsample stage with a different grid, used when the output is 16-byte aligned. The whole-call path is off by default (whole_call_tables=False), while the new upsample variant is on by default.

```diff
diff --git a/include/wavernn_amd.h b/include/wavernn_amd.h
--- a/include/wavernn_amd.h
+++ b/include/wavernn_amd.h
@@ -187,6 +187,7 @@
 int wrnn_pre_upsample_many(const wrnn_pre *p, const wrnn_pre_utt *utts, int32_t n_utt, int32_t rows_only, float *mels_up, float *aux,
                            void *workspace, size_t workspace_bytes, void *stream);
 int wrnn_pre_debug_host_handle(const wrnn_pre_weights *w, wrnn_pre **out);
+int wrnn_pre_debug_last_stage(wrnn_pre *p, int32_t old_body);
 const char *wrnn_pre_last_error(void);
 
 int wrnn_post_unfold(const float *segments, int32_t T, int32_t n_utt, const int32_t *first, const int32_t *folds,
diff --git a/wavernn_amd/_lib.py b/wavernn_amd/_lib.py
--- a/wavernn_amd/_lib.py
+++ b/wavernn_amd/_lib.py
@@ -20,7 +20,7 @@
            'wrnn_generate_segments', 'wrnn_noise_fill', 'wrnn_noise_fill_host', 'wrnn_plan_segments', 'wrnn_status', 'wrnn_timer_create', 'wrnn_timer_destroy', 'wrnn_timer_ms',
            'wrnn_timer_launches', 'wrnn_debug_read_exchange', 'wrnn_debug_plan', 'wrnn_selftest', 'wrnn_selftest_metric', 'wrnn_pre_create',
            'wrnn_pre_destroy', 'wrnn_pre_hop', 'wrnn_pre_workspace_bytes', 'wrnn_pre_upsample', 'wrnn_pre_upsample_rows', 'wrnn_pre_workspace_bytes_many',
-           'wrnn_pre_upsample_many', 'wrnn_pre_debug_host_handle', 'wrnn_pre_last_error',
+           'wrnn_pre_upsample_many', 'wrnn_pre_debug_host_handle', 'wrnn_pre_debug_last_stage', 'wrnn_pre_last_error',
            'wrnn_post_unfold', 'wrnn_post_last_error', 'wrnn_taco_workspace_bytes', 'wrnn_taco_decode', 'wrnn_taco_status',
            'wrnn_taco_last_error', 'wrnn_bigru', 'wrnn_taco_front_create', 'wrnn_taco_front_destroy', 'wrnn_taco_front_workspace_bytes',
            'wrnn_taco_encode', 'wrnn_taco_postnet', 'wrnn_taco_batch_workspace_bytes', 'wrnn_taco_decode_batch',
@@ -226,6 +226,7 @@
     L.wrnn_pre_upsample_many.argtypes = [ctypes.c_void_p, ctypes.POINTER(PreUtt), ctypes.c_int32, ctypes.c_int32, ctypes.c_void_p, ctypes.c_void_p,
                                          ctypes.c_void_p, ctypes.c_size_t, ctypes.c_void_p]
     L.wrnn_pre_debug_host_handle.argtypes = [ctypes.POINTER(PreWeights), ctypes.POINTER(ctypes.c_void_p)]
+    L.wrnn_pre_debug_last_stage.argtypes = [ctypes.c_void_p, ctypes.c_int32]
     L.wrnn_pre_last_error.restype = ctypes.c_char_p
     L.wrnn_post_unfold.argtypes = [ctypes.c_void_p, ctypes.c_int32, ctypes.c_int32, ctypes.c_void_p, ctypes.c_void_p, ctypes.c_void_p,
                                    ctypes.c_void_p, ctypes.c_int32, ctypes.c_void_p, ctypes.c_void_p, ctypes.c_int32,
diff --git a/wavernn_amd/batch.py b/wavernn_amd/batch.py
--- a/wavernn_amd/batch.py
+++ b/wavernn_amd/batch.py
@@ -135,6 +135,22 @@
 def library_seg_ids(seed, folds, first_fold: int = 0) -> np.ndarray:
     hi = np.uint64((int(seed) & 0xffffffff) << 32)
     return hi | np.arange(first_fold, first_fold + int(folds), dtype=np.uint64)
+
+
+WHOLE_CALL_SLAB_BYTES = 256 << 20
+
+
+def whole_call_options(model, eng, n_segments: int, T: int, algo, library_noise: bool, kernel: Optional[str] = None) -> dict:
+    from .engine import SLABBED_KERNELS, TUNING_WHOLE_TABLES
+    want = getattr(model, 'whole_call_tables', False)
+    if want is False or (want is None and model.mode != 'MOL') or getattr(model, 'progress_callback', None) is not None:
+        return {}
+    if (kernel or eng.plan(n_segments, T, algo=algo)['kernel']) not in SLABBED_KERNELS:
+        return {}
+    per_step = n_segments * 4 * ((11 if model.mode == 'MOL' else 0) + (0 if not library_noise else 11 if model.mode == 'MOL' else model.n_classes))
+    slab = T if per_step == 0 else max(16, min(T, WHOLE_CALL_SLAB_BYTES // per_step))
+    slab = -(-T // (-(-T // slab)))
+    return dict(slab_steps=int(slab), tuning=TUNING_WHOLE_TABLES)
 
 
 def chunk_utterances(plan: Plan, lo: int, hi: int, max_segments: int):
@@ -289,7 +305,10 @@
             from .engine import RESUMABLE_KERNELS
             steps = T
             groups = model.loop_sparse_groups(eng, n_seg, T) if hasattr(model, 'loop_sparse_groups') else 0
-            if noise_source != 'library' and eng.plan(n_seg, T, algo=model.loop_algo)['kernel'] in RESUMABLE_KERNELS:
+            planned = eng.plan(n_seg, T, algo=model.loop_algo)['kernel']
+            whole = whole_call_options(model, eng, n_seg, T, model.loop_algo, noise_source == 'library', kernel=planned)
+            run_kw = dict(sparse_groups=groups, tuning=slab_tuning | whole.get('tuning', 0), slab_steps=whole.get('slab_steps', 0), **lib_kw)
+            if noise_source != 'library' and planned in RESUMABLE_KERNELS:
                 per_step = n_seg * (11 if mode == 'MOL' else model.n_classes) * 4
                 steps = max(1, min(T, getattr(model, 'noise_chunk_bytes', 2 << 30) // per_step))
                 steps = -(-T // (-(-T // steps)))
@@ -297,7 +316,7 @@
                 for t0 in range(0, T, steps):
                     t1 = min(T, t0 + steps)
                     eng.run_segments(mels_up, aux, seg_pos, seg_lim, T, draw(t1 - t0), hop, algo=model.loop_algo, check=check, out=out_view,
-                                     t_range=None if (t0 == 0 and t1 == T) else (t0, t1), sparse_groups=groups, tuning=slab_tuning, **lib_kw)
+                                     t_range=None if (t0 == 0 and t1 == T) else (t0, t1), **run_kw)
             except ResidencyError as e:
                 import warnings
                 warnings.warn(f'wavernn_amd: {e}; redoing the chunk unsliced on the next kernel')
@@ -306,7 +325,7 @@
                 for u in gens:
                     gens[u].manual_seed(int(seeds[u]))
                     burn_ctor_draws(model.rnn_dims, model.aux_dims, 'cpu', gens[u])
-                eng.run_segments(mels_up, aux, seg_pos, seg_lim, T, draw(T), hop, algo=model.loop_algo, check=check, out=out_view, sparse_groups=groups, tuning=slab_tuning, **lib_kw)
+                eng.run_segments(mels_up, aux, seg_pos, seg_lim, T, draw(T), hop, algo=model.loop_algo, check=check, out=out_view, **run_kw)
             finally:
                 if pool is not None:
                     pool.shutdown()
diff --git a/wavernn_amd/csrc/wrnn_abi.hip b/wavernn_amd/csrc/wrnn_abi.hip
--- a/wavernn_amd/csrc/wrnn_abi.hip
+++ b/wavernn_amd/csrc/wrnn_abi.hip
@@ -1,4 +1,5 @@
 #include <hip/hip_runtime.h>
+#include <limits.h>
 #include <stdarg.h>
 #include <stdio.h>
 #include <stdlib.h>
@@ -415,6 +416,7 @@
 
 enum Kind { K_STREAM, K_GENERIC, K_LOOP, K_DUO, K_OCTO, K_CHAIN, K_SPARSE, N_KINDS };
 constexpr int DUO_TAB_FPS = 8;
+constexpr int TUNING_WHOLE_TABLES = 1 << 15;
 constexpr bool DUO_AUTO = true;
 constexpr int CHAIN_AUTO_GROUPS = 8;
 constexpr bool OCTO_AUTO = false;
@@ -457,6 +459,7 @@
     Kind kind;
     int ncl, G, rounds, per_round, slab, ngr_max;
     int tab_fps;
+    bool whole;
     int t0, t1;
 };
 
@@ -539,6 +542,7 @@
     const bool two_groups = o->sparse_groups == 2;
     const int groups = (B + SEG - 1) / SEG;
     pl->kind = K_STREAM; pl->ncl = 0; pl->G = 0; pl->rounds = 1; pl->per_round = B; pl->slab = T; pl->ngr_max = groups;
+    pl->tab_fps = 0; pl->whole = false;
     if (p->generic) {
         if (algo != WRNN_ALGO_AUTO && algo != WRNN_ALGO_STREAM) {
             set_err("this pack has non-shipped dims (rnn %d, fc %d, feat %d, aux %d): only the generic kernel (algo auto / stream) runs it", p->gH, p->gF, p->gM, p->gA);
@@ -609,13 +613,29 @@
         else plan_split(pl, B, ncl, k.max_depth(p->mode), o->depth);
         pl->slab = o->slab_steps >= 1 ? o->slab_steps : default_slab(*pl, p->mode, p->C, o->noise_lib != 0);
         if (pl->slab > T) pl->slab = T;
-        pl->tab_fps = DUO_TAB_FPS;
+        pl->whole = k.slabbed && (o->tuning & TUNING_WHOLE_TABLES) != 0;
+        pl->tab_fps = pl->whole ? 0 : DUO_TAB_FPS;
+        if (pl->whole && p->mode == WRNN_MODE_MOL) {
+            const size_t most = (size_t)0x7FFFF000u / ((size_t)B * 11 * sizeof(float));
+            if (most < 1) { set_err("%d segments in one call: one step of derived noise exceeds a 2 GB buffer resource; split the call", B); return WRNN_ERR_ARG; }
+            if ((size_t)pl->slab > most) pl->slab = (int)most;
+        }
     } else if (partial) {
         set_err("a partial step range [%d, %d) needs a persistent loop kernel", pl->t0, pl->t1);
         return WRNN_ERR_ARG;
     }
-    if (k.slabbed && ((size_t)B * pl->tab_fps + 1) * 3 * H * sizeof(float) >= 0x7FFFF000ull) {
+    if (k.slabbed && !pl->whole && ((size_t)B * pl->tab_fps + 1) * 3 * H * sizeof(float) >= 0x7FFFF000ull) {
         set_err("%d segments in one call: the per-slab aux tables exceed a 2 GB buffer resource; split the call (generate_corpus caps a launch at 4096 segments)", B);
+        return WRNN_ERR_ARG;
+    }
+    return WRNN_OK;
+}
+
+int check_whole_tables(const Plan &pl, int n_frames)
+{
+    if (pl.whole && ((size_t)n_frames + 1) * 3 * H * sizeof(float) >= 0x7FFFF000ull) {
+        set_err("%d frames of conditioning in one call: the whole-call aux tables (wrnn_options.tuning bit 15) exceed a 2 GB buffer resource "
+                "(%zu frames at most); split the call or clear the bit", n_frames, (size_t)0x7FFFF000ull / ((size_t)3 * H * sizeof(float)) - 1);
         return WRNN_ERR_ARG;
     }
     return WRNN_OK;
@@ -637,7 +657,7 @@
         l.total = o;
         return l;
     }
-    const size_t tab_rows = k.slabbed ? (size_t)B * pl.tab_fps + 1 : (size_t)n_frames + 1;
+    const size_t tab_rows = k.slabbed && !pl.whole ? (size_t)B * pl.tab_fps + 1 : (size_t)n_frames + 1;
     l.c2f = o;    o = al(o + tab_rows * 3 * H * sizeof(float));
     l.c3f = o;    o = al(o + tab_rows * H * sizeof(float));
     l.c4f = o;    o = al(o + tab_rows * H * sizeof(float));
@@ -701,8 +721,9 @@
 int plan_report(const wrnn_plan_traits *tr, int B, int T, int n_frames, const wrnn_options &o, wrnn_run_info *out, size_t *ws_bytes)
 {
     Plan pl;
-    const int rc = make_plan(tr, B, T, &o, &pl);
+    int rc = make_plan(tr, B, T, &o, &pl);
     if (rc != WRNN_OK) return rc;
+    if ((rc = check_whole_tables(pl, n_frames)) != WRNN_OK) return rc;
     if (out) {
         memset(out, 0, sizeof *out);
         out->kernel = KINDS[pl.kind].name; out->units_per_wg = KINDS[pl.kind].units_per_wg;
@@ -750,6 +771,7 @@
     if (rc != WRNN_OK) return rc;
     Plan pl;
     if ((rc = make_plan(&p->tr, B, T, o, &pl)) != WRNN_OK) return rc;
+    if ((rc = check_whole_tables(pl, n_frames)) != WRNN_OK) return rc;
     const KindDesc &k = KINDS[pl.kind];
     const WsLayout l = ws_layout(&p->tr, pl, B, T, n_frames, lib_noise);
     if (workspace_bytes < l.total) { set_err("workspace %zu < required %zu", workspace_bytes, l.total); return WRNN_ERR_WORKSPACE; }
@@ -823,10 +845,10 @@
     c.c2f = (float *)(ws + l.c2f); c.c3f = (float *)(ws + l.c3f); c.c4f = (float *)(ws + l.c4f);
     c.seg_pos = d_pos; c.seg_lim = d_lim;
     c.B = B; c.T = T; c.hop = hop; c.NF = n_frames;
-    if (k.slabbed) {
+    if (k.slabbed && !pl.whole) {
         const long eff = (long)(pl.tab_fps - 2) * hop + 1;
         if (pl.slab > eff) pl.slab = (int)eff;
-    } else HIPCHK(launch_cond_frames(c, stream));
+    } else if (!k.slabbed) HIPCHK(launch_cond_frames(c, stream));
 
     LoopArgs a;
     memset(&a, 0, sizeof a);
@@ -880,10 +902,12 @@
                 a.noise_t0 = pl.t0;
             }
             if (k.slabbed) {
-                c.t0 = s0; c.B = B; c.FPS = pl.tab_fps;
+                c.t0 = s0; c.B = B; c.FPS = !pl.whole ? pl.tab_fps : s0 == pl.t0 ? 0 : -1;
                 if (prep_fused) HIPCHK(launch_slab_prep(c, mol_rows, (float *)(ws + l.npre), (long)(s1 - s0) * 11 * B, (unsigned *)(ws + l.xcc), p->tr.n_cus, stream));
-                else HIPCHK(launch_cond_frames_slab(c, stream));
-                a.tab_fps = pl.tab_fps; a.tab_t0 = s0;
+                else if (!pl.whole) HIPCHK(launch_cond_frames_slab(c, stream));
+                else if (c.FPS == 0) HIPCHK(launch_cond_frames(c, stream));
+                a.tab_fps = pl.tab_fps; a.tab_t0 = pl.whole ? 0 : s0;
+                a.tab_zrow = pl.whole ? n_frames : B * pl.tab_fps; a.tab_hop = pl.whole ? INT_MAX : hop;
             }
             bool xcc_clear = prep_fused;
             for (int r = 0; r < pl.rounds; ++r) {
diff --git a/wavernn_amd/csrc/wrnn_chain.hip b/wavernn_amd/csrc/wrnn_chain.hip
--- a/wavernn_amd/csrc/wrnn_chain.hip
+++ b/wavernn_amd/csrc/wrnn_chain.hip
@@ -63,7 +63,7 @@
     const int hop = a.hop, resume = a.resume, Tall = a.T, Nall = a.Nall, noise_t0 = a.noise_t0, C = a.C;
     const unsigned magic = a.hop_magic;
     const int mshift = a.hop_shift;
-    const int zrow = a.Nall * a.tab_fps;
+    const int zrow = a.tab_zrow;
     float *const outp = a.out, *const dbgl = a.dbg_logits;
     const float *const forcex = a.force_x, *const noise_pre = a.noise_pre, *const noise_raw = a.noise;
     const float *const mels_up = a.mels_up, *const aux_fr = a.aux_fr, *const mel_coef = a.mel_coef;
@@ -136,7 +136,7 @@
             const int pos = a.seg_pos[sc];
             SEGT[i * 64 + tid] = pos;
             SEGT[i * 64 + SEG + tid] = a.seg_lim[sc];
-            SEGT[i * 64 + 2 * SEG + tid] = sc * a.tab_fps - (pos + a.tab_t0) / a.hop;
+            SEGT[i * 64 + 2 * SEG + tid] = sc * a.tab_fps - (pos + a.tab_t0) / a.tab_hop;
             SEGT[i * 64 + 3 * SEG + tid] = a.mel_stage ? a.seg_moff[sc] : 0;
         }
         float4 sv = make_float4(0.f, bh_r, bh_z, bh_n);
diff --git a/wavernn_amd/csrc/wrnn_cond.hip b/wavernn_amd/csrc/wrnn_cond.hip
--- a/wavernn_amd/csrc/wrnn_cond.hip
+++ b/wavernn_amd/csrc/wrnn_cond.hip
@@ -261,13 +261,16 @@
     }
     const CondArgs &a = s.c;
     __shared__ float ax[SPR][4 * AUX];
-    const int nrows = a.B * a.FPS + 1, row0 = (int)blockIdx.x * SPR;
+    const int ntab = a.FPS > 0 ? a.B * a.FPS : a.NF;
+    const int nrows = ntab + 1, row0 = (int)blockIdx.x * SPR;
     for (int q = r; q < SPR * 4 * AUX; q += H) {
         const int i = q / (4 * AUX), e = q % (4 * AUX), row = row0 + i;
         int f = a.NF;
-        if (row < a.B * a.FPS) {
-            const int b = row / a.FPS, j = row % a.FPS;
-            f = (a.seg_pos[b] + a.t0) / a.hop + j;
+        if (row < ntab) {
+            if (a.FPS > 0) {
+                const int b = row / a.FPS, j = row % a.FPS;
+                f = (a.seg_pos[b] + a.t0) / a.hop + j;
+            } else f = row;
         }
         ax[i][e] = (f < a.NF) ? a.aux[(size_t)f * 4 * AUX + e] : 0.f;
     }
@@ -306,7 +309,7 @@
 {
     SlabPrepArgs s;
     s.c = a; s.nz_in = nz_in; s.nz_out = nz_out; s.nz_n = nz_in ? nz_n : 0; s.xcc = xcc;
-    s.cond_blocks = (a.B * a.FPS + 1 + SPR - 1) / SPR;
+    s.cond_blocks = a.FPS < 0 ? 0 : ((a.FPS > 0 ? a.B * a.FPS : a.NF) + 1 + SPR - 1) / SPR;
     long nb = (s.nz_n + H - 1) / H;
     if (nb > (long)n_cus * 4) nb = (long)n_cus * 4;
     if (nb < 1) nb = 1;
diff --git a/wavernn_amd/csrc/wrnn_device.h b/wavernn_amd/csrc/wrnn_device.h
--- a/wavernn_amd/csrc/wrnn_device.h
+++ b/wavernn_amd/csrc/wrnn_device.h
@@ -90,6 +90,7 @@
     int tab_fps, tab_t0;
     unsigned *xcc_tab;
     int kind_tag;
+    int tab_zrow, tab_hop;
 };
 
 __device__ __forceinline__ void check_kind(const LoopArgs &a)
diff --git a/wavernn_amd/csrc/wrnn_duo.hip b/wavernn_amd/csrc/wrnn_duo.hip
--- a/wavernn_amd/csrc/wrnn_duo.hip
+++ b/wavernn_amd/csrc/wrnn_duo.hip
@@ -101,7 +101,7 @@
     u64 *const profp = a.prof;
     const float *const bhhp = LA ? a.b_hh1 : a.b_hh2;
     const int resume = a.resume, hop = a.hop;
-    const int zrow = a.Nall * a.tab_fps;
+    const int zrow = a.tab_zrow;
     constexpr int L_H = LA ? 0 : 1, L_XR = LA ? 5 : 6, L_Y = LA ? 2 : 3, L_GH = LA ? 8 : 12;
     constexpr int L_P0 = LA ? 4 : 5, L_P2 = LA ? 6 : 2;
 
@@ -144,7 +144,7 @@
         if (tid < SEG) {
             const int nb = (int)((geo.nbpack >> (8 * i)) & 255u);
             const int sc = GEO[2 * i] + (tid < nb ? tid : nb - 1);
-            SEGT[i * 48 + 2 * SEG + tid] = sc * a.tab_fps - (SEGT[i * 48 + tid] + a.tab_t0) / a.hop;
+            SEGT[i * 48 + 2 * SEG + tid] = sc * a.tab_fps - (SEGT[i * 48 + tid] + a.tab_t0) / a.tab_hop;
         }
     }
     __syncthreads();
diff --git a/wavernn_amd/csrc/wrnn_octo.hip b/wavernn_amd/csrc/wrnn_octo.hip
--- a/wavernn_amd/csrc/wrnn_octo.hip
+++ b/wavernn_amd/csrc/wrnn_octo.hip
@@ -256,7 +256,7 @@
     const float *const mels_up = a.mels_up, *const aux_fr = a.aux_fr, *const mel_coef = a.mel_coef;
     const int mel_stage = a.mel_stage;
     const int resume = a.resume, hop = a.hop;
-    const int zrow = a.Nall * a.tab_fps;
+    const int zrow = a.tab_zrow;
     const unsigned magic = a.hop_magic;
     const int mshift = a.hop_shift;
     const int tun = a.tuning;
@@ -685,7 +685,7 @@
             const int b0 = (int)(((long)g * NR) / NGR), nb = (int)(((long)(g + 1) * NR) / NGR) - b0;
             if (tid < SEG) {
                 const int sc = a.rb0 + b0 + (tid < nb ? tid : nb - 1);
-                SEGT[i * 64 + 2 * SEG + tid] = sc * a.tab_fps - (SEGT[i * 64 + tid] + a.tab_t0) / a.hop;
+                SEGT[i * 64 + 2 * SEG + tid] = sc * a.tab_fps - (SEGT[i * 64 + tid] + a.tab_t0) / a.tab_hop;
                 SEGT[i * 64 + 3 * SEG + tid] = a.mel_stage ? a.seg_moff[sc] : 0;
             }
         }
diff --git a/wavernn_amd/csrc/wrnn_pre.hip b/wavernn_amd/csrc/wrnn_pre.hip
--- a/wavernn_amd/csrc/wrnn_pre.hip
+++ b/wavernn_amd/csrc/wrnn_pre.hip
@@ -253,8 +253,9 @@
     upstage_body<FIRST, LAST, S, PFEAT>(in, out, taps, n_in, S, PPAD, 0, PFEAT, blockIdx.x - utt[u].blk[stage], utt[u + 1].blk[stage] - utt[u].blk[stage]);
 }
 
+constexpr int UPLAST_LA = 8;
 template <int S>
-__device__ __forceinline__ void upstage_last_body(const float *__restrict__ in, float *__restrict__ out, const float *__restrict__ taps, int n_in, int s_rt,
+__device__ __forceinline__ void upstage_last_body_ref(const float *__restrict__ in, float *__restrict__ out, const float *__restrict__ taps, int n_in, int s_rt,
                                                   int indent, long blk, long nblk)
 {
     constexpr int TQ = 64;
@@ -286,16 +287,54 @@
     }
 }
 template <int S>
+__device__ __forceinline__ void upstage_last_body(const float *__restrict__ in, float *__restrict__ out, const float *__restrict__ taps, int n_in, int indent,
+                                                  long blk, long nblk)
+{
+    static_assert(S > 0, "compile-time stretch factor");
+    constexpr int LA = UPLAST_LA, ROW = S * PFEAT, TILE = LA * ROW;
+    static_assert(LA % 4 == 0 && PFEAT % 16 == 0 && TILE % 4 == 0, "lane mapping: 4 positions x 16 channels per wave");
+    __shared__ __attribute__((aligned(16))) float tile[TILE];
+    float w[2 * S + 1];
+#pragma unroll
+    for (int j = 0; j <= 2 * S; ++j) w[j] = taps[j];
+    const int a_lo = indent / S, na = n_in - 2 * a_lo;
+    for (long a0 = blk * LA; a0 < na; a0 += nblk * LA) {
+        const int valid = na - a0 < LA ? (int)(na - a0) : LA;
+        for (int e = threadIdx.x; e < LA * PFEAT; e += 256) {
+            const int al = (e >> 4) % LA, c = ((e >> 4) / LA) * 16 + (e & 15);
+            if (al < valid) {
+                const float *src = in + (size_t)c * n_in + (a_lo + a0 + al);
+                const float v0 = src[-1], v1 = src[0], v2 = src[1];
+#pragma unroll
+                for (int ph = 0; ph < S; ++ph) {
+                    float acc = 0.f;
+#pragma unroll
+                    for (int j = 0; j <= 2 * S; ++j) acc = fmaf(w[j], j <= S - 1 - ph ? v0 : (j >= 2 * S - ph ? v2 : v1), acc);
+                    tile[(al * S + ph) * PFEAT + c] = acc;
+                }
+            }
+        }
+        __syncthreads();
+        float4 *dst = reinterpret_cast<float4 *>(out + (size_t)a0 * ROW);
+        const float4 *src4 = reinterpret_cast<const float4 *>(tile);
+        for (int k = threadIdx.x; k < valid * (ROW / 4); k += 256) dst[k] = src4[k];
+        __syncthreads();
+    }
+}
+template <int S, bool REF>
 __global__ __launch_bounds__(256) void wrnn_upstage_last_kernel(const float *__restrict__ in, float *__restrict__ out,
                                                                 const float *__restrict__ taps, int n_in, int s_rt, int indent)
 {
-    upstage_last_body<S>(in, out, taps, n_in, s_rt, indent, blockIdx.x, gridDim.x);
-}
-template <int S>
+    if constexpr (REF) upstage_last_body_ref<S>(in, out, taps, n_in, s_rt, indent, blockIdx.x, gridDim.x);
+    else upstage_last_body<S>(in, out, taps, n_in, indent, blockIdx.x, gridDim.x);
+}
+template <int S, bool REF>
 __global__ __launch_bounds__(256) void wrnn_upstage_last_many_kernel(const PreUttDev *__restrict__ utt, int n_utt, const float *__restrict__ taps, int indent)
 {
     const int u = pre_find_utt(utt, n_utt, 3, blockIdx.x);
-    upstage_last_body<S>(utt[u].s2, utt[u].up, taps, (utt[u].n + 2 * PPAD) * 25, S, indent, blockIdx.x - utt[u].blk[3], utt[u + 1].blk[3] - utt[u].blk[3]);
+    const long blk = blockIdx.x - utt[u].blk[3], nblk = utt[u + 1].blk[3] - utt[u].blk[3];
+    if constexpr (REF) upstage_last_body_ref<S>(utt[u].s2, utt[u].up, taps, (utt[u].n + 2 * PPAD) * 25, S, indent, blk, nblk);
+    else upstage_last_body<S>(utt[u].s2, utt[u].up, taps, (utt[u].n + 2 * PPAD) * 25, indent, blk, nblk);
 }
 
 }
@@ -319,6 +358,7 @@
     int device, blocks, scales[3], total_scale;
     int feat, C, R, pad;
     int gf;
+    int last_ref;
     float *dev;
     const float *conv_in_w, *bn_in, *res_w, *res_bn, *conv_out_w, *conv_out_b, *taps[3];
 };
@@ -361,6 +401,19 @@
     pre_set_dims(p, w, -1, gf);
     *out = p;
     return WRNN_OK;
+}
+
+extern "C" int wrnn_pre_debug_last_stage(wrnn_pre *p, int32_t old_body)
+{
+    if (!p) PRE_FAIL(WRNN_ERR_ARG, "NULL argument");
+    p->last_ref = old_body != 0;
+    return WRNN_OK;
+}
+
+static long last_stage_blocks(const wrnn_pre *p, long n_frames, bool ref)
+{
+    const long b = ref ? (n_frames * p->total_scale * 4 + 255) / 256 : (n_frames * p->scales[0] * p->scales[1] + UPLAST_LA - 1) / UPLAST_LA;
+    return b > 65535 ? 65535 : (b < 1 ? 1 : b);
 }
 
 extern "C" int wrnn_pre_create(const wrnn_pre_weights *w, int device, wrnn_pre **out)
@@ -455,6 +508,7 @@
     const bool shipped = feat80 && PD == PPAD && p->scales[0] == 5 && p->scales[1] == 5 && p->scales[2] == 11;
     const unsigned g1 = grid((long)nf * p->scales[0] * FE), g2 = grid((long)nf * p->scales[0] * p->scales[1] * FE);
     const unsigned g3 = grid((long)n_frames * p->total_scale * 4);
+    const bool last_ref = p->last_ref || ((uintptr_t)mels_up & 15) != 0 || PD < 1;
     const int n2 = nf * p->scales[0], n3 = n2 * p->scales[1], indent = PD * p->total_scale;
     if (rows_only) {
         if (shipped) {
@@ -467,11 +521,12 @@
     } else if (shipped) {
         hipLaunchKernelGGL((wrnn_upstage_kernel<true, false, 5>), dim3(g1), dim3(256), 0, stream, mel, s1, p->taps[0], nf, 5, PD, 0, PFEAT);
         hipLaunchKernelGGL((wrnn_upstage_kernel<false, false, 5>), dim3(g2), dim3(256), 0, stream, s1, s2, p->taps[1], n2, 5, 0, 0, PFEAT);
-        hipLaunchKernelGGL((wrnn_upstage_last_kernel<11>), dim3(g3), dim3(256), 0, stream, s2, mels_up, p->taps[2], n3, 11, indent);
+        if (last_ref) hipLaunchKernelGGL((wrnn_upstage_last_kernel<11, true>), dim3(g3), dim3(256), 0, stream, s2, mels_up, p->taps[2], n3, 11, indent);
+        else hipLaunchKernelGGL((wrnn_upstage_last_kernel<11, false>), dim3((unsigned)last_stage_blocks(p, n_frames, false)), dim3(256), 0, stream, s2, mels_up, p->taps[2], n3, 11, indent);
     } else {
         hipLaunchKernelGGL((wrnn_upstage_kernel<true, false, 0, 0>), dim3(g1), dim3(256), 0, stream, mel, s1, p->taps[0], nf, p->scales[0], PD, 0, FE);
         hipLaunchKernelGGL((wrnn_upstage_kernel<false, false, 0, 0>), dim3(g2), dim3(256), 0, stream, s1, s2, p->taps[1], n2, p->scales[1], 0, 0, FE);
-        if (feat80) hipLaunchKernelGGL((wrnn_upstage_last_kernel<0>), dim3(g3), dim3(256), 0, stream, s2, mels_up, p->taps[2], n3, p->scales[2], indent);
+        if (feat80) hipLaunchKernelGGL((wrnn_upstage_last_kernel<0, true>), dim3(g3), dim3(256), 0, stream, s2, mels_up, p->taps[2], n3, p->scales[2], indent);
         else hipLaunchKernelGGL((wrnn_upstage_kernel<false, true, 0, 0>), dim3(grid((long)n_frames * p->total_scale * FE)), dim3(256), 0, stream, s2, mels_up, p->taps[2], n3, p->scales[2], 0, indent, FE);
     }
     PRE_HIP(hipGetLastError());
@@ -543,6 +598,7 @@
     PRE_HIP(dg.err);
     auto grid = [](long total) { long b = (total + 255) / 256; return (long)(b > 65535 ? 65535 : (b < 1 ? 1 : b)); };
     std::vector<PreUttDev> tab((size_t)n_utt + 1);
+    bool last_ref = p->last_ref || ((uintptr_t)mels_up & 15) != 0;
     long blk[4] = {0, 0, 0, 0};
     for (int u = 0; u < n_utt; ++u) {
         const int n = utts[u].n_frames;
@@ -557,7 +613,7 @@
         blk[0] += (n + PNF - 1) / PNF;
         blk[1] += grid(nf * 5 * PFEAT);
         blk[2] += grid(nf * 25 * PFEAT);
-        blk[3] += rows ? 0 : grid((long)n * p->total_scale * 4);
+        blk[3] += rows ? 0 : last_stage_blocks(p, n, last_ref);
         for (int s = 0; s < 4; ++s)
             if (blk[s] > 0x7fffffffL) PRE_FAIL(WRNN_ERR_ARG, "too many frames for one call (stage grid of %ld workgroups); split the table", blk[s]);
         off += slice;
@@ -577,7 +633,8 @@
         hipLaunchKernelGGL((wrnn_upstage_many_kernel<false, true, 5>), dim3((unsigned)blk[2]), dim3(256), 0, stream, d_tab, n_utt, p->taps[1]);
     } else {
         hipLaunchKernelGGL((wrnn_upstage_many_kernel<false, false, 5>), dim3((unsigned)blk[2]), dim3(256), 0, stream, d_tab, n_utt, p->taps[1]);
-        hipLaunchKernelGGL((wrnn_upstage_last_many_kernel<11>), dim3((unsigned)blk[3]), dim3(256), 0, stream, d_tab, n_utt, p->taps[2], PPAD * p->total_scale);
+        if (last_ref) hipLaunchKernelGGL((wrnn_upstage_last_many_kernel<11, true>), dim3((unsigned)blk[3]), dim3(256), 0, stream, d_tab, n_utt, p->taps[2], PPAD * p->total_scale);
+        else hipLaunchKernelGGL((wrnn_upstage_last_many_kernel<11, false>), dim3((unsigned)blk[3]), dim3(256), 0, stream, d_tab, n_utt, p->taps[2], PPAD * p->total_scale);
     }
     PRE_HIP(hipGetLastError());
     return WRNN_OK;
diff --git a/wavernn_amd/csrc/wrnn_sparse.hip b/wavernn_amd/csrc/wrnn_sparse.hip
--- a/wavernn_amd/csrc/wrnn_sparse.hip
+++ b/wavernn_amd/csrc/wrnn_sparse.hip
@@ -172,7 +172,7 @@
     const int hop = a.hop, resume = a.resume, Tall = a.T, Nall = a.Nall, noise_t0 = a.noise_t0, C = a.C;
     const unsigned magic = a.hop_magic;
     const int mshift = a.hop_shift;
-    const int zrow = a.Nall * a.tab_fps;
+    const int zrow = a.tab_zrow;
     float *const outp = a.out, *const dbgl = a.dbg_logits;
     const float *const forcex = a.force_x, *const noise_pre = a.noise_pre, *const noise_raw = a.noise;
     const float *const mels_up = a.mels_up, *const aux_fr = a.aux_fr, *const mel_coef = a.mel_coef;
@@ -270,7 +270,7 @@
             const int pos = a.seg_pos[sc];
             SEGT[tid] = pos;
             SEGT[SEG + tid] = a.seg_lim[sc];
-            SEGT[2 * SEG + tid] = sc * a.tab_fps - (pos + a.tab_t0) / a.hop;
+            SEGT[2 * SEG + tid] = sc * a.tab_fps - (pos + a.tab_t0) / a.tab_hop;
             SEGT[3 * SEG + tid] = a.mel_stage ? a.seg_moff[sc] : 0;
         }
     }
diff --git a/wavernn_amd/engine.py b/wavernn_amd/engine.py
--- a/wavernn_amd/engine.py
+++ b/wavernn_amd/engine.py
@@ -15,6 +15,8 @@
 KERNEL_ALGOS = {'wrnn_sparse_kernel': ('sparse', 'duo'), 'wrnn_chain_kernel': ('chain', 'duo'), 'wrnn_octo_kernel': ('octo', 'duo'),
                 'wrnn_duo_kernel': ('duo', 'loop'), 'wrnn_loop_kernel': ('loop', None)}
 FALLBACK_ALGO = {k: nxt for k, (_, nxt) in KERNEL_ALGOS.items() if nxt}
+SLABBED_KERNELS = ('wrnn_duo_kernel', 'wrnn_sparse_kernel', 'wrnn_chain_kernel', 'wrnn_octo_kernel')
+TUNING_WHOLE_TABLES = 1 << 15
 
 
 class MelRows:
@@ -209,6 +211,8 @@
                 raise _lib.ResidencyError('cooperative launch refused (' + why + ')')
             if rows_in is not None:
                 mels_up = rows_in
+            if (tuning & TUNING_WHOLE_TABLES) and f'wrnn_{nxt}_kernel' not in SLABBED_KERNELS:
+                tuning, slab_steps = tuning & ~TUNING_WHOLE_TABLES, 0
             if nxt is not None:
                 warnings.warn('wavernn_amd: cooperative launch refused (' + why + '); trying algo = ' + nxt)
                 self._ws = None
diff --git a/wavernn_amd/model.py b/wavernn_amd/model.py
--- a/wavernn_amd/model.py
+++ b/wavernn_amd/model.py
@@ -122,6 +122,7 @@
         self.pinned_output = True
         self.post_tables_early = True
         self.slab_prep_split = False
+        self.whole_call_tables = False
         self.mel_in_loop = None
         self.post_algo = 'native'
         self.noise_chunk_bytes = 2 << 30
@@ -305,15 +306,17 @@
         if self.progress_callback is not None:
             t_start, cb = time.perf_counter(), self.progress_callback
             prog = lambda done, T_, n_: cb(done, T_, n_, time.perf_counter() - t_start)
+        from .batch import whole_call_options
+        whole = whole_call_options(self, eng, B, T, algo, self.noise_source == 'library')
         if self.noise_source == 'library':
             from .batch import library_seg_ids
             return eng.run(mels_up, aux, B, T, stride, None, self.hop_length, algo=algo, progress=prog, sparse_groups=sparse_groups,
-                           noise_seed=self.noise_key, noise_seg_id=library_seg_ids(self.noise_seed, B))
+                           noise_seed=self.noise_key, noise_seg_id=library_seg_ids(self.noise_seed, B), **whole)
         for t0 in range(0, T, chunk):
             t1 = min(T, t0 + chunk)
             noise = draw_steps(self.mode, B, t1 - t0, self.n_classes, device, self.noise_source)
             out = eng.run(mels_up, aux, B, T, stride, noise, self.hop_length, algo=algo, out=out,
-                          t_range=None if (t0 == 0 and t1 == T) else (t0, t1), progress=prog, sparse_groups=sparse_groups)
+                          t_range=None if (t0 == 0 and t1 == T) else (t0, t1), progress=prog, sparse_groups=sparse_groups, **whole)
         return out
 
     def gen_display(self, i, seq_len, b_size, gen_rate):
```

Result: no change. 11.28 million (median of 3 runs) (+0.3%).
